# hegdepashupati/zero-inflated-gp

Hardware: AMD Instinct MI355X
Metric: elbo_steps_per_sec (higher is better)
Workload: dtype f64; 1 GPU; dense zero-inflated GP ELBO step (value+gradient), N=1000000 rows per GPU, D=3, M=1024 per latent, full batch; rows_this_rank=1000000, rows_total=1000000, M=1024, D=3, chunk_rows=32768, parallelism=row-shard x1, 1 all-reduce/step

## Files before the change

zero-inflated-gp_amd/csrc/zigp_ctx.h:

```cpp
#pragma once
#include <hip/hip_runtime.h>
#include <stdint.h>
#include <stdio.h>
#include <string.h>
#include <string>
#include <vector>
#include <map>
#include <memory>
#include "../../include/zigp.h"
#include "../../include/zigp_diag.h"
#include "zigp_gemm.h"

namespace zigp {

struct DevBuf {
  double* p = nullptr;
  size_t cap = 0;
  bool owned = true;
  DevBuf() = default;
  DevBuf(const DevBuf&) = delete;
  DevBuf& operator=(const DevBuf&) = delete;
  DevBuf(DevBuf&& o) noexcept : p(o.p), cap(o.cap), owned(o.owned) { o.p = nullptr; o.cap = 0; o.owned = true; }
  DevBuf& operator=(DevBuf&& o) noexcept {
    if (this != &o) { release(); p = o.p; cap = o.cap; owned = o.owned; o.p = nullptr; o.cap = 0; o.owned = true; }
    return *this;
  }
  ~DevBuf() { release(); }
  int ensure(size_t n) {
    if (!owned) { p = nullptr; cap = 0; owned = true; }
    if (n <= cap) return 0;
    if (p) (void)hipFree(p);
    p = nullptr; cap = 0;
    hipError_t e = hipMalloc((void**)&p, n * sizeof(double));
    if (e != hipSuccess) return -1;
    cap = n;
    return 0;
  }
  void alias(double* q, size_t n) { release(); p = q; cap = n; owned = false; }
  void release() { if (p && owned) (void)hipFree(p); p = nullptr; cap = 0; owned = true; }
};

enum ProfClass { PC_GEMM_A1 = 0, PC_GEMM_A2 = 1, PC_GEMM_H = 2, PC_GEMM_J = 3, PC_SYR2K = 4, PC_KUF = 5, PC_POINT = 6, PC_RED = 7, PC_MXM = 8, PC_OTHER = 9 };

struct TileList {
  GemmTile* d = nullptr;
  int n = 0;
  int per = 1;
};
struct HipFree { void operator()(void* q) const { (void)hipFree(q); } };
struct CachedTiles {
  std::unique_ptr<GemmTile, HipFree> d;
  int n = 0, per = 1;
  TileList view() const { return TileList{d.get(), n, per}; }
};

struct Latent {
  int M = 0, Mp = 0;
  DevBuf Z, ell, u, s, s2;
  double zc[64] = {0};
  bool kg_exact = false;
  DevBuf Zs;
  double var = 1.0;
  DevBuf Kuu, L, W;
  DevBuf K, A1, Jp;
  DevBuf Kd;
  DevBuf Wp, a1gm;
  DevBuf Wt;
  DevBuf P, Qt, Rt;
  bool P_ready = false;
  DevBuf part;
  DevBuf gm, gv;
  DevBuf du, dsq, krow;
  DevBuf xm, mom, ks0;
  DevBuf dLpart;
  DevBuf T1, T2, T3, G;
  DevBuf sk;
  DevBuf vec;
  DevBuf wh;
  DevBuf Lraw, Lq, lqssq, dLq;
};

struct KronState;
struct KfState;

struct PinnedArena {
  struct Block { char* p; size_t cap, used; };
  std::vector<Block> blocks;
  PinnedArena() = default;
  PinnedArena(const PinnedArena&) = delete;
  PinnedArena& operator=(const PinnedArena&) = delete;
  ~PinnedArena() { for (auto& b : blocks) (void)hipHostFree(b.p); }
  void reset() { for (auto& b : blocks) b.used = 0; }
  void* alloc(size_t bytes) {
    bytes = (bytes + 63) & ~(size_t)63;
    for (auto& b : blocks)
      if (b.cap - b.used >= bytes) { void* r = b.p + b.used; b.used += bytes; return r; }
    Block nb; nb.cap = bytes > ((size_t)1 << 20) ? bytes : ((size_t)1 << 20); nb.used = bytes; nb.p = nullptr;
    if (hipHostMalloc((void**)&nb.p, nb.cap, hipHostMallocDefault) != hipSuccess) return nullptr;
    blocks.push_back(nb);
    return nb.p;
  }
};

struct CtxHandles {
  hipStream_t stream = nullptr;
  hipStream_t stream_main = nullptr, stream2 = nullptr;
  hipStream_t stream3 = nullptr;
  hipEvent_t ev_fork = nullptr, ev_join = nullptr;
  hipEvent_t ev_prep_fork = nullptr, ev_prep = nullptr;
  int* d_info = nullptr;
  struct PendingEv { hipEvent_t a, b; int cls; };
  std::vector<PendingEv> pending;
  std::vector<hipEvent_t> ev_pool;
  CtxHandles() = default;
  CtxHandles(const CtxHandles&) = delete;
  CtxHandles& operator=(const CtxHandles&) = delete;
  ~CtxHandles() {
    if (d_info) (void)hipFree(d_info);
    for (auto& e : pending) { (void)hipEventDestroy(e.a); (void)hipEventDestroy(e.b); }
    for (auto e : ev_pool) (void)hipEventDestroy(e);
    for (hipEvent_t e : {ev_fork, ev_join, ev_prep_fork, ev_prep})
      if (e) (void)hipEventDestroy(e);
    for (hipStream_t s : {stream3, stream2, stream_main})
      if (s) (void)hipStreamDestroy(s);
  }
};

}

struct zigp_ctx : zigp::CtxHandles {
  ~zigp_ctx();
  int device = 0;
  std::string err;
  int info = 0;
  int64_t fit_steps_applied = 0;
  int64_t chunk = 32768;
  bool chunk_auto = true;
  const double* dX = nullptr; const double* dY = nullptr;
  zigp::DevBuf ownX, ownY;
  int64_t N = 0; int D = 0;
  const double* fullX = nullptr; const double* fullY = nullptr; int64_t fullN = 0;
  zigp::DevBuf selX, selY, selIdx;
  zigp::DevBuf fitX, fitY, fitIdx, fit;
  int64_t dense_fit_steps_applied = 0;
  zigp::Latent lat[2];
  zigp::DevBuf pw_part;
  bool fwd_kuf_side = true;
  bool trmm_tail = true;
  int overlap = 1;
  bool mean_on = false;
  bool whiten = false;
  int kern[2] = {0, 0};
  bool q_full = false;
  double mean_a[8] = {0}, mean_b = 0.0, mean_da[8] = {0}, mean_db = 0.0;
  zigp::DevBuf out9;
  zigp::DevBuf scratch, scratch2;
  zigp::DevBuf path_tab, path_out;
  zigp::PinnedArena pinned;
  std::unique_ptr<zigp::KronState> kron;
  std::unique_ptr<zigp::KfState> kronf;
  bool kron_panels = false;
  int kron_kern[2][2] = {{0, 0}, {0, 0}};
  bool kron_matern_fused = false;
  int kron_range_tiles = 1024;
  std::map<std::string, zigp::CachedTiles> tiles;
  void* comm = nullptr; int comm_rank = 0, comm_nranks = 1; int64_t comm_calls = 0;
  double comm_timeout_s = 120.0;
  zigp::DevBuf packed;
  zigp::DevBuf parm;
  double pivot_rtol = 8.0;
  bool prof_on = false;
  int prof_every = 8;
  bool prof_skip = false;
  int64_t prof_total[ZIGP_NCLASS] = {0};
  double prof_ms[ZIGP_NCLASS] = {0};
  int64_t prof_n[ZIGP_NCLASS] = {0};
  double prof_flops[ZIGP_NCLASS] = {0};
};

namespace zigp {

#define ZIGP_HIP(ctx, expr)                                                              \
  do {                                                                                   \
    hipError_t _e = (expr);                                                              \
    if (_e != hipSuccess) {                                                              \
      char _b[512];                                                                      \
      snprintf(_b, sizeof(_b), "HIP error '%s' at %s:%d (%s)", hipGetErrorString(_e), __FILE__, __LINE__, #expr); \
      (ctx)->err = _b;                                                                   \
      return ZIGP_EHIP;                                                                  \
    }                                                                                    \
  } while (0)

#define ZIGP_TRY(expr)            \
  do {                            \
    int _rc = (expr);             \
    if (_rc != 0) return _rc;     \
  } while (0)

#define ZIGP_ENSURE(ctx, buf, n)                                        \
  do {                                                                  \
    if ((buf).ensure((size_t)(n)) != 0) {                               \
      (ctx)->err = "hipMalloc failed for " #buf;                        \
      return ZIGP_EHIP;                                                 \
    }                                                                   \
  } while (0)

inline int fail_arg(zigp_ctx* c, const char* msg) { c->err = msg; return ZIGP_EARG; }

struct OnStream {
  zigp_ctx* c;
  hipStream_t saved;
  OnStream(zigp_ctx* c_, hipStream_t s) : c(c_), saved(c_->stream) { c->stream = s; }
  ~OnStream() { c->stream = saved; }
  OnStream(const OnStream&) = delete;
  OnStream& operator=(const OnStream&) = delete;
};

inline int fork_side(zigp_ctx* c, hipEvent_t ev, hipStream_t side) {
  ZIGP_HIP(c, hipEventRecord(ev, c->stream_main));
  ZIGP_HIP(c, hipStreamWaitEvent(side, ev, 0));
  return 0;
}
inline int join_side(zigp_ctx* c, hipEvent_t ev, hipStream_t side) {
  ZIGP_HIP(c, hipEventRecord(ev, side));
  ZIGP_HIP(c, hipStreamWaitEvent(c->stream_main, ev, 0));
  return 0;
}

struct ProfScope {
  zigp_ctx* c; hipEvent_t a = nullptr, b = nullptr; int cls; bool on;
  static hipEvent_t get_ev(zigp_ctx* c) {
    if (!c->ev_pool.empty()) { hipEvent_t e = c->ev_pool.back(); c->ev_pool.pop_back(); return e; }
    hipEvent_t e; if (hipEventCreate(&e) != hipSuccess) return nullptr; return e;
  }
  ProfScope(zigp_ctx* c_, int cls_, double flops = 0.0) : c(c_), cls(cls_), on(c_->prof_on) {
    if (!on) return;
    c->prof_total[cls] += 1;
    if (c->prof_skip) { on = false; return; }
    a = get_ev(c); b = get_ev(c);
    if (!a || !b) { on = false; return; }
    (void)hipEventRecord(a, c->stream);
    c->prof_flops[cls] += flops;
    c->prof_n[cls] += 1;
  }
  ~ProfScope() {
    if (!on) return;
    (void)hipEventRecord(b, c->stream);
    c->pending.push_back({a, b, cls});
  }
};

inline void prof_collect(zigp_ctx* c) {
  for (auto& p : c->pending) {
    float ms = 0.f;
    if (hipEventSynchronize(p.b) == hipSuccess && hipEventElapsedTime(&ms, p.a, p.b) == hipSuccess) c->prof_ms[p.cls] += ms;
    c->ev_pool.push_back(p.a); c->ev_pool.push_back(p.b);
  }
  c->pending.clear();
}

}
```

zero-inflated-gp_amd/csrc/zigp_dense.hip:

```cpp
#include "zigp_ctx.h"
#include "zigp_kernels.h"
#include "zigp_host.h"
#include "zigp_rows.h"
#include "zigp_comm.h"
#include <algorithm>
#include <cmath>
#include <functional>

using namespace zigp;

static_assert(WIDE_MAXD == ZIGP_MAX_D, "the wide kernels' hyperparameter structs hold ZIGP_MAX_D entries");
#define ZIGP_STR2(x) #x
#define ZIGP_STR(x) ZIGP_STR2(x)
#define ZIGP_MAX_D_STR ZIGP_STR(ZIGP_MAX_D)

namespace {

enum class Param : int { Diag = 0, White = 1, WhiteFull = 2 };
constexpr bool is_white(Param p) { return p != Param::Diag; }
constexpr bool is_full(Param p) { return p == Param::WhiteFull; }
static_assert((int)Param::Diag == ZIGP_FIT_DIAG && (int)Param::White == ZIGP_FIT_WHITE && (int)Param::WhiteFull == ZIGP_FIT_WHITE_FULL,
              "Param values are the ZIGP_FIT_* modes of include/zigp.h");
Param param_of(const zigp_ctx* c) { return !c->whiten ? Param::Diag : c->q_full ? Param::WhiteFull : Param::White; }

struct HostLatent {
  int M; const double *Z, *u, *s, *ell; double var;
  int kind = ZIGP_KERN_RBF;
};
static_assert(KERN_RBF == ZIGP_KERN_RBF && KERN_M32 == ZIGP_KERN_MATERN32 && KERN_M52 == ZIGP_KERN_MATERN52,
              "the kernels' kind values are the ZIGP_KERN_* constants of include/zigp.h");
constexpr bool is_matern(int kind) { return kind != ZIGP_KERN_RBF; }
const char* kern_name(int kind) { return kind == ZIGP_KERN_MATERN32 ? "Matern32" : kind == ZIGP_KERN_MATERN52 ? "Matern52" : "RBF"; }
const char* matern_latent(const zigp_ctx* c, std::string& who) {
  for (int h = 0; h < 2; ++h)
    if (is_matern(c->kern[h])) { who = std::string(kern_name(c->kern[h])) + " kernel on latent " + (h ? "g" : "f"); return who.c_str(); }
  return nullptr;
}

void kgrad_centre(Latent& lt, const double* Z, const double* ell, int M, int D) {
  double spread = 0.0;
  for (int d = 0; d < WIDE_MAXD; ++d) {
    double sum = 0.0;
    if (d < D) for (int m = 0; m < M; ++m) sum += Z[(size_t)m * D + d];
    lt.zc[d] = M > 0 ? sum / M : 0.0;
    if (d < D) for (int m = 0; m < M; ++m) spread = std::max(spread, std::fabs(Z[(size_t)m * D + d] - lt.zc[d]) / ell[d]);
  }
  lt.kg_exact = !(spread <= KG_EXACT_SPREAD);
}

int latents_layout(zigp_ctx* c, const int (&M)[2], int D, size_t (&off)[2][6], size_t& total) {
  total = 0;
  for (int h = 0; h < 2; ++h) {
    Latent& lt = c->lat[h];
    lt.M = M[h];
    lt.Mp = (int)round_up(M[h], BM);
    const size_t Mp = lt.Mp;
    off[h][0] = total; total += Mp * D;
    off[h][1] = total; total += std::max(D, MAXD);
    off[h][2] = total; total += Mp;
    off[h][3] = total; total += Mp;
    off[h][4] = total; total += Mp * D;
    off[h][5] = total;
  }
  ZIGP_ENSURE(c, c->parm, total);
  return 0;
}
int latents_views(zigp_ctx* c, const size_t (&off)[2][6], int D) {
  for (int h = 0; h < 2; ++h) {
    Latent& lt = c->lat[h];
    const size_t Mp = lt.Mp;
    lt.Z.alias(c->parm.p + off[h][0], Mp * D); lt.ell.alias(c->parm.p + off[h][1], std::max(D, MAXD));
    lt.u.alias(c->parm.p + off[h][2], Mp); lt.s.alias(c->parm.p + off[h][3], Mp); lt.Zs.alias(c->parm.p + off[h][4], Mp * D);
    ZIGP_ENSURE(c, lt.s2, Mp);
    ZIGP_ENSURE(c, lt.Kuu, Mp * Mp);
    ZIGP_ENSURE(c, lt.L, Mp * Mp);
    ZIGP_ENSURE(c, lt.W, Mp * Mp);
    ZIGP_ENSURE(c, lt.T1, Mp * Mp);
    ZIGP_ENSURE(c, lt.vec, 4 * Mp + 8);
    ZIGP_ENSURE(c, lt.wh, 4 * Mp + 8);
    ZIGP_ENSURE(c, lt.Wp, Mp * Mp);
    ZIGP_ENSURE(c, lt.Wt, Mp * Mp);
    ZIGP_ENSURE(c, lt.P, Mp * Mp); ZIGP_ENSURE(c, lt.Qt, Mp * Mp); ZIGP_ENSURE(c, lt.Rt, Mp * Mp);
  }
  return 0;
}
int latents_upload(zigp_ctx* c, const HostLatent (&hl)[2], int D, Param par) {
  size_t off[2][6], total = 0;
  const int M[2] = {hl[0].M, hl[1].M};
  ZIGP_TRY(latents_layout(c, M, D, off, total));
  for (int h = 0; h < 2; ++h) c->lat[h].var = hl[h].var;
  ZIGP_PINNED(c, img, total);
  memset(img, 0, sizeof(double) * total);
  for (int h = 0; h < 2; ++h) {
    const HostLatent& q = hl[h];
    memcpy(img + off[h][0], q.Z, sizeof(double) * q.M * D);
    memcpy(img + off[h][1], q.ell, sizeof(double) * D);
    memcpy(img + off[h][2], q.u, sizeof(double) * q.M);
    if (is_full(par)) for (int m = 0; m < q.M; ++m) img[off[h][3] + m] = q.s[(size_t)m * q.M + m];
    else memcpy(img + off[h][3], q.s, sizeof(double) * q.M);
    const KufHypWide kh = make_kuf_hyp_wide(q.ell, q.var, D);
    kgrad_centre(c->lat[h], q.Z, q.ell, q.M, D);
    for (int m = 0; m < q.M; ++m)
      for (int d = 0; d < D; ++d) img[off[h][4] + (size_t)m * D + d] = q.Z[(size_t)m * D + d] * kh.scale[d];
  }
  ZIGP_HIP(c, hipMemcpyAsync(c->parm.p, img, sizeof(double) * total, hipMemcpyHostToDevice, c->stream));
  if (is_full(par))
    for (int h = 0; h < 2; ++h) {
      Latent& lt = c->lat[h];
      const size_t mm = (size_t)hl[h].M * hl[h].M, mmp = (size_t)lt.Mp * lt.Mp;
      ZIGP_ENSURE(c, lt.Lraw, mm); ZIGP_ENSURE(c, lt.Lq, mmp); ZIGP_ENSURE(c, lt.lqssq, mmp / 256);
      ZIGP_PINNED(c, raw, mm);
      memcpy(raw, hl[h].s, sizeof(double) * mm);
      ZIGP_HIP(c, hipMemcpyAsync(lt.Lraw.p, raw, sizeof(double) * mm, hipMemcpyHostToDevice, c->stream));
    }
  return latents_views(c, off, D);
}

int latent_qfull_stage(zigp_ctx* c, Latent& lt) {
  const int Mp = lt.Mp, nblk = (int)((size_t)Mp * Mp / 256);
  hipLaunchKernelGGL(k_lq_stage, dim3(nblk), dim3(256), 0, c->stream, lt.Lraw.p, lt.M, (int64_t)Mp, lt.Lq.p, lt.lqssq.p);
  hipLaunchKernelGGL(k_kl_white_full, dim3(1), dim3(256), 0, c->stream, lt.u.p, lt.Lq.p, lt.lqssq.p, nblk, lt.M, (int64_t)Mp, lt.wh.p);
  ZIGP_HIP(c, hipGetLastError());
  return 0;
}
int latent_qfull_factors(zigp_ctx* c, Latent& lt) {
  const int Mp = lt.Mp, nb = Mp / BM;
  ZIGP_TRY((run_gemm_sk<LAY_KCONTIG, LAY_KCONTIG>(c, lt.sk, SkRule::TT, nb, lt.Lq.p, lt.Lq.p, lt.P.p, Mp, SK_STORE, 1.0)));
  hipLaunchKernelGGL(k_sub_eye, dim3(ceil_div(Mp, 256)), dim3(256), 0, c->stream, lt.P.p, lt.M, (int64_t)Mp);
  ZIGP_HIP(c, hipGetLastError());
  return run_gemm_sk<LAY_KCONTIG, LAY_MNCONTIG>(c, lt.sk, SkRule::Y, nb, lt.P.p, lt.W.p, lt.Rt.p, Mp, SK_STORE, 1.0);
}
int latent_qfull_dlq(zigp_ctx* c, Latent& lt, bool with_data, bool with_kl) {
  const int Mp = lt.Mp, nb = Mp / BM;
  const size_t mm = (size_t)Mp * Mp;
  ZIGP_ENSURE(c, lt.T3, mm); ZIGP_ENSURE(c, lt.dLq, mm);
  if (with_data)
    ZIGP_TRY((run_gemm_sk<LAY_KCONTIG, LAY_MNCONTIG>(c, lt.sk, SkRule::Y, nb, lt.T1.p, lt.Lq.p, lt.T3.p, Mp, SK_STORE, 1.0)));
  hipLaunchKernelGGL(k_dlq_assemble, dim3(ceil_div((int64_t)mm, 256)), dim3(256), 0, c->stream, lt.T3.p, lt.Lq.p, with_data ? 1 : 0, with_kl ? 1 : 0,
                     lt.M, (int64_t)Mp, lt.dLq.p);
  ZIGP_HIP(c, hipGetLastError());
  return 0;
}

int latents_forward(zigp_ctx* c, const HostLatent (&hl)[2], int D, double jitter, Param par, bool with_kl, bool need_grad, const double* d_hyp,
                    int* d_info2) {
  const hipStream_t st[2] = {c->stream_main, c->stream2};
  for (int h = 0; h < 2; ++h) {
    Latent& lt = c->lat[h];
    const int Mp = lt.Mp;
    OnStream on(c, st[h]);
    const dim3 grid(ceil_div((int64_t)Mp * Mp, 256));
    if (is_matern(hl[h].kind))
      hipLaunchKernelGGL(k_kuu_setup_matern, grid, dim3(256), 0, c->stream, lt.Z.p, (int64_t)hl[h].M, make_hyp(hl[h].ell, hl[h].var, D), hl[h].kind, jitter,
                         lt.Kuu.p, lt.L.p, lt.W.p, lt.s.p, lt.s2.p, (int64_t)Mp);
    else if (d_hyp)
      hipLaunchKernelGGL(k_kuu_setup<LatHypDev>, grid, dim3(256), 0, c->stream, lt.Z.p, (int64_t)hl[h].M, LatHypDev{d_hyp + h * DH_LAT, D}, jitter, lt.Kuu.p,
                         lt.L.p, lt.W.p, lt.s.p, lt.s2.p, (int64_t)Mp);
    else if (D > MAXD)
      hipLaunchKernelGGL(k_kuu_setup<KernHypWide>, grid, dim3(256), 0, c->stream, lt.Z.p, (int64_t)hl[h].M, make_hyp_wide(hl[h].ell, hl[h].var, D), jitter,
                         lt.Kuu.p, lt.L.p, lt.W.p, lt.s.p, lt.s2.p, (int64_t)Mp);
    else {
      KernHyp hyp = make_hyp(hl[h].ell, hl[h].var, D);
      hipLaunchKernelGGL(k_kuu_setup<KernHyp>, grid, dim3(256), 0, c->stream, lt.Z.p, (int64_t)hl[h].M, hyp, jitter, lt.Kuu.p,
                         lt.L.p, lt.W.p, lt.s.p, lt.s2.p, (int64_t)Mp);
    }
    ZIGP_HIP(c, hipGetLastError());
  }
  {
    PotrfJob jobs[2];
    for (int h = 0; h < 2; ++h) {
      Latent& lt = c->lat[h];
      jobs[h] = PotrfJob{lt.L.p, lt.W.p, lt.T1.p, lt.Mp, true, lt.M, d_hyp ? 0.0 : pivot_tol(hl[h].var, jitter, c->pivot_rtol), true, &lt.sk};
      if (d_hyp) { jobs[h].tol_dev = d_hyp + h * DH_LAT + DH_PIVTOL; jobs[h].info = d_info2 + h; }
    }
    ZIGP_TRY(potrf_trtri_jobs(c, 2, jobs, st));
  }
  for (int step = 0; step < 8; ++step)
    for (int h = 0; h < 2; ++h) {
      Latent& lt = c->lat[h];
      const int Mp = lt.Mp;
      OnStream on(c, st[h]);
      if (step == 0) lt.P_ready = false;
      double* v = lt.vec.p; double* alpha = v + Mp; double* dkinv = v + 2 * Mp; double* klv = v + 3 * Mp;
      if (is_white(par)) {
        switch (step) {
          case 0: hipLaunchKernelGGL(k_transpose, dim3(Mp / 32, Mp / 32), dim3(32, 8), 0, c->stream, lt.W.p, (int64_t)Mp, lt.Wt.p); break;
          case 1:
            if (is_full(par)) ZIGP_TRY(latent_qfull_stage(c, lt));
            else hipLaunchKernelGGL(k_kl_white, dim3(1), dim3(256), 0, c->stream, lt.u.p, lt.s.p, lt.M, (int64_t)Mp, lt.wh.p);
            break;
          case 2: if (need_grad) hipLaunchKernelGGL(k_gemv_cols, dim3(Mp / 64), dim3(64, COL_LANES), 0, c->stream, lt.W.p, lt.u.p, (int64_t)Mp, alpha); break;
          case 3:
            if (need_grad && is_full(par)) ZIGP_TRY(latent_qfull_factors(c, lt));
            else if (need_grad) hipLaunchKernelGGL(k_rowscale, dim3(ceil_div((int64_t)Mp * Mp, 256)), dim3(256), 0, c->stream, lt.W.p, lt.wh.p, (int64_t)Mp, lt.Wp.p);
            break;
          default: break;
        }
        ZIGP_HIP(c, hipGetLastError());
        continue;
      }
      switch (step) {
        case 0:
          hipLaunchKernelGGL(k_transpose, dim3(Mp / 32, Mp / 32), dim3(32, 8), 0, c->stream, lt.W.p, (int64_t)Mp, lt.Wt.p);
          break;
        case 1: if (with_kl) hipLaunchKernelGGL(k_gemv_rows, dim3(Mp), dim3(256), 0, c->stream, lt.W.p, lt.u.p, (int64_t)Mp, v); break;
        case 2: if (with_kl) hipLaunchKernelGGL(k_kl_cols, dim3(Mp / 64), dim3(64, COL_LANES), 0, c->stream, lt.W.p, v, (int64_t)Mp, alpha, dkinv); break;
        case 3: if (with_kl) hipLaunchKernelGGL(k_kl_value, dim3(1), dim3(256), 0, c->stream, v, lt.L.p, lt.s.p, dkinv, lt.M, (int64_t)Mp, klv); break;
        case 4:
          if (need_grad) hipLaunchKernelGGL(k_colscale, dim3(ceil_div((int64_t)Mp * Mp, 256)), dim3(256), 0, c->stream, lt.W.p, lt.s2.p, (int64_t)Mp, lt.Wp.p);
          break;
        case 5:
          if (need_grad) {
            ZIGP_TRY((run_gemm_sk<LAY_MNCONTIG, LAY_MNCONTIG>(c, lt.sk, SkRule::S, Mp / BM, lt.W.p, lt.W.p, lt.P.p, Mp, SK_STORE, 1.0)));
            lt.P_ready = true;
          }
          break;
        case 6:
          if (need_grad) hipLaunchKernelGGL(k_rowscale_minus_eye, dim3(ceil_div((int64_t)Mp * Mp, 256)), dim3(256), 0, c->stream, lt.P.p, lt.s2.p, (int64_t)Mp, lt.Qt.p);
          break;
        case 7:
          if (need_grad) ZIGP_TRY((run_gemm_sk<LAY_KCONTIG, LAY_MNCONTIG>(c, lt.sk, SkRule::RT, Mp / BM, lt.W.p, lt.Qt.p, lt.Rt.p, Mp, SK_STORE, 1.0)));
          break;
        default: break;
      }
      ZIGP_HIP(c, hipGetLastError());
    }
  return 0;
}

int latent_chunk_kuf_matern(zigp_ctx* c, Latent& lt, const double* dX, int64_t Nrows, int64_t n0, int64_t Nc, int D, const double* ell_host, int kind,
                            bool with_kd) {
  if (D < 1 || D > MAXD || !ell_host) return fail_arg(c, "a Matern Kuf panel needs 1 <= D <= 8 and host lengthscales");
  if (with_kd && lt.Kd.cap < (size_t)lt.Mp * Nc) return fail_arg(c, "a Matern gradient step's K' panel was not sized for this chunk");
  const KufHyp kh = make_kuf_hyp(ell_host, lt.var, D);
  ProfScope ps(c, PC_KUF);
  const dim3 grid((unsigned)(Nc / 512), lt.Mp / 16), block(256);
#define ZIGP_KUF_M(DD, KK, GG) \
  hipLaunchKernelGGL((k_kuf_build_matern<DD, KK, GG>), grid, block, 0, c->stream, dX, Nrows, n0, lt.Zs.p, lt.M, kh, lt.K.p, GG ? lt.Kd.p : nullptr, Nc)
#define ZIGP_KUF_MD(DD)                                                                    \
  case DD:                                                                                 \
    if (kind == ZIGP_KERN_MATERN32) { if (with_kd) ZIGP_KUF_M(DD, KERN_M32, true); else ZIGP_KUF_M(DD, KERN_M32, false); } \
    else { if (with_kd) ZIGP_KUF_M(DD, KERN_M52, true); else ZIGP_KUF_M(DD, KERN_M52, false); }                            \
    break;
  switch (D) { ZIGP_KUF_MD(1) ZIGP_KUF_MD(2) ZIGP_KUF_MD(3) ZIGP_KUF_MD(4) ZIGP_KUF_MD(5) ZIGP_KUF_MD(6) ZIGP_KUF_MD(7) ZIGP_KUF_MD(8) }
#undef ZIGP_KUF_MD
#undef ZIGP_KUF_M
  ZIGP_HIP(c, hipGetLastError());
  return 0;
}
int latent_chunk_kuf(zigp_ctx* c, Latent& lt, const double* dX, int64_t Nrows, int64_t n0, int64_t Nc, int D, const double* ell_host,
                     const double* R = nullptr, int kind = ZIGP_KERN_RBF, bool with_kd = false) {
  if (is_matern(kind)) return latent_chunk_kuf_matern(c, lt, dX, Nrows, n0, Nc, D, ell_host, kind, with_kd);
  const int Mp = lt.Mp;
  const KufHyp kh = (R || D > MAXD) ? KufHyp() : make_kuf_hyp(ell_host, lt.var, D);
  ProfScope ps(c, PC_KUF);
  const dim3 grid((unsigned)(Nc / 512), Mp / 16), block(256);
#define ZIGP_KUF(DD)                                                                                                                   \
  case DD:                                                                                                                             \
    if (R) hipLaunchKernelGGL((k_kuf_build<DD, LatHypDev>), grid, block, 0, c->stream, dX, Nrows, n0, lt.Zs.p, lt.M, LatHypDev{R, DD}, lt.K.p, Nc); \
    else hipLaunchKernelGGL((k_kuf_build<DD, KufHyp>), grid, block, 0, c->stream, dX, Nrows, n0, lt.Zs.p, lt.M, kh, lt.K.p, Nc);               \
    break;
  switch (D) {
    ZIGP_KUF(1) ZIGP_KUF(2) ZIGP_KUF(3) ZIGP_KUF(4) ZIGP_KUF(5) ZIGP_KUF(6) ZIGP_KUF(7) ZIGP_KUF(8)
    default:
      if (D < 1 || D > WIDE_MAXD || R) return fail_arg(c, "D out of range");
      hipLaunchKernelGGL(k_kuf_build_wide, grid, block, 0, c->stream, dX, Nrows, n0, lt.Zs.p, lt.M, D, make_kuf_hyp_wide(ell_host, lt.var, D), lt.K.p, Nc);
      break;
  }
#undef ZIGP_KUF
  ZIGP_HIP(c, hipGetLastError());
  return 0;
}

struct ChunkPlan {
  int64_t Nc = 0;
  bool paired = false;
  TrmmTail tail = {{0, 0}, {64, 64}};
  struct Lat { TileSpec a1_spec, a2j_spec, syr_spec, mom_spec; TileList a1, a2j, syr, mom; double fl = 0.0; } lat[2];
};
ChunkPlan chunk_plan(const int (&M)[2], int64_t Nc, Param par, bool need_grad, bool tail_on, bool wide) {
  ChunkPlan pl;
  const int nbm[2] = {ceil_div(M[0], BM), ceil_div(M[1], BM)}, nbn = (int)(Nc / BN);
  pl.Nc = Nc;
  pl.paired = trmm_paired_pays(nbn * ((nbm[0] + 1) / 2 + (nbm[1] + 1) / 2));
  if (pl.paired && tail_on)
    pl.tail = trmm_tail_plan((nbn + 7) / 8 * 8 * ((nbm[0] + 1) / 2), nbm[0], (nbn + 7) / 8 * 8 * ((nbm[1] + 1) / 2), nbm[1]);
  for (int h = 0; h < 2; ++h) {
    ChunkPlan::Lat& L = pl.lat[h];
    auto tri = [&](bool lower) { return trmm_tiles(lower, nbm[h], nbn, pl.paired, pl.tail.units[h], pl.tail.bins[h]); };
    auto full_product = [&] { return full_xcd_tiles(nbm[h], nbn, nbm[h] * (BM / BK)); };
    L.a1_spec = tri(true);
    switch (par) {
      case Param::Diag: L.a2j_spec = need_grad ? full_product() : tri(false); break;
      case Param::White: if (need_grad) L.a2j_spec = tri(false); break;
      case Param::WhiteFull: L.a2j_spec = need_grad ? full_product() : tri(false); break;
    }
    if (need_grad) L.syr_spec = syr2k_tiles(nbm[h], (int)(Nc / BK), syr_plan(nbm[h]));
    if (need_grad && wide) L.mom_spec = kgmom_tiles(nbm[h], Nc);
    L.fl = (double)M[h] * M[h] * (double)Nc;
  }
  return pl;
}
int upload_plan(zigp_ctx* c, ChunkPlan& pl) {
  for (ChunkPlan::Lat& L : pl.lat) {
    ZIGP_TRY(get_tiles(c, L.a1_spec, L.a1));
    if (L.a2j_spec.build) ZIGP_TRY(get_tiles(c, L.a2j_spec, L.a2j));
    if (L.syr_spec.build) ZIGP_TRY(get_tiles(c, L.syr_spec, L.syr));
    if (L.mom_spec.build) ZIGP_TRY(get_tiles(c, L.mom_spec, L.mom));
  }
  return 0;
}

int chunk_forward(zigp_ctx* c, const ChunkPlan& pl, Param par, bool need_grad, const std::function<int()>& after_a1 = nullptr) {
  const int64_t Nc = pl.Nc;
  struct Set { TileList t1, t2; double fl; GemmArgs a1, a2j; EpiStoreColsum e1; EpiColsum e2; EpiStorePanelKColsum ej; } q[3] = {};
  for (int h = 0; h < 2; ++h) {
    Latent& lt = c->lat[h];
    const int Mp = lt.Mp, np = Mp / 32;
    q[h].t1 = pl.lat[h].a1; q[h].t2 = pl.lat[h].a2j; q[h].fl = pl.lat[h].fl;
    q[h].a1 = mk_args(lt.Wt.p, Mp, lt.K.p, Nc, lt.A1.p, Nc);
    q[h].e1 = EpiStoreColsum{is_full(par) ? lt.wh.p + Mp : lt.vec.p, nullptr, lt.part.p, lt.part.p + (size_t)np * Nc};
    if (need_grad) {
      q[h].a2j = mk_args(lt.Rt.p, Mp, lt.A1.p, Nc, lt.Jp.p, Nc);
      q[h].ej = EpiStorePanelKColsum{lt.K.p, lt.part.p + (size_t)2 * np * Nc};
    } else {
      q[h].a2j = mk_args(is_full(par) ? lt.Lq.p : lt.W.p, Mp, lt.A1.p, Nc, nullptr, Nc);
      q[h].e2 = EpiColsum{nullptr, is_full(par) ? nullptr : lt.s2.p, nullptr, lt.part.p + (size_t)2 * np * Nc};
    }
  }
  const int groups = pl.paired ? 1 : 2;
  for (int gi = 0; gi < groups; ++gi) {
    const Set& x = q[gi];
    const Set& y = q[pl.paired ? 1 : 2];
    {
      ProfScope ps(c, PC_GEMM_A1, x.fl + y.fl);
      ZIGP_TRY((run_gemm<LAY_MNCONTIG, LAY_MNCONTIG, false, TRI_A_LOWER>(c, x.t1, x.a1, x.e1, y.t1, y.a1, y.e1)));
    }
    if (gi == groups - 1 && after_a1) ZIGP_TRY(after_a1());
    if (need_grad) {
      ProfScope ps(c, PC_GEMM_J, 2.0 * (x.fl + y.fl));
      ZIGP_TRY((run_gemm<LAY_MNCONTIG, LAY_MNCONTIG, false>(c, x.t2, x.a2j, x.ej, y.t2, y.a2j, y.ej)));
    } else {
      ProfScope ps(c, PC_GEMM_A2, x.fl + y.fl);
      ZIGP_TRY((run_gemm<LAY_MNCONTIG, LAY_MNCONTIG, false, TRI_A_UPPER>(c, x.t2, x.a2j, x.e2, y.t2, y.a2j, y.e2)));
    }
  }
  return 0;
}

int chunk_forward_white(zigp_ctx* c, const ChunkPlan& pl, bool need_grad, bool part_j, const std::function<int()>& after_a = nullptr) {
  const int64_t Nc = pl.Nc;
  struct Set { TileList t; double fl; GemmArgs g; EpiStoreColsum es; EpiColsum ec; } q[3] = {};
  for (int h = 0; h < 2; ++h) {
    Latent& lt = c->lat[h];
    const int Mp = lt.Mp, np = Mp / 32;
    double* p0 = lt.part.p; double* p2 = lt.part.p + (size_t)2 * np * Nc;
    q[h].fl = pl.lat[h].fl;
    if (part_j) { q[h].t = pl.lat[h].a2j; q[h].g = mk_args(lt.Wp.p, Mp, lt.A1.p, Nc, lt.Jp.p, Nc); continue; }
    q[h].t = pl.lat[h].a1;
    q[h].g = mk_args(lt.Wt.p, Mp, lt.K.p, Nc, need_grad ? lt.A1.p : nullptr, Nc);
    q[h].es = EpiStoreColsum{lt.wh.p + Mp, lt.wh.p, p0, p2};
    q[h].ec = EpiColsum{lt.wh.p + Mp, lt.wh.p, p0, p2};
  }
  const int groups = pl.paired ? 1 : 2;
  for (int gi = 0; gi < groups; ++gi) {
    const Set& x = q[gi];
    const Set& y = q[pl.paired ? 1 : 2];
    if (part_j) {
      ProfScope ps(c, PC_GEMM_J, x.fl + y.fl);
      ZIGP_TRY((run_gemm<LAY_MNCONTIG, LAY_MNCONTIG, false, TRI_A_UPPER>(c, x.t, x.g, EpiStore(), y.t, y.g, EpiStore())));
      continue;
    }
    {
      ProfScope ps(c, PC_GEMM_A1, x.fl + y.fl);
      if (need_grad) ZIGP_TRY((run_gemm<LAY_MNCONTIG, LAY_MNCONTIG, false, TRI_A_LOWER>(c, x.t, x.g, x.es, y.t, y.g, y.es)));
      else ZIGP_TRY((run_gemm<LAY_MNCONTIG, LAY_MNCONTIG, false, TRI_A_LOWER>(c, x.t, x.g, x.ec, y.t, y.g, y.ec)));
    }
    if (gi == groups - 1 && after_a) ZIGP_TRY(after_a());
  }
  return 0;
}

int latent_chunk_kgrad_wide(zigp_ctx* c, Latent& lt, const double* dX, int64_t Nrows, int64_t n0, int64_t Nc, int D, const TileList& mom) {
  const int Mp = lt.Mp, S = kgmom_slices(Mp / BM, Nc);
  if (mom.n != S * (Mp / BM)) return fail_arg(c, "wide Kuf gradient: the moments product's tile list was not planned for this chunk shape");
  KgCentreWide ctr;
  for (int d = 0; d < WIDE_MAXD; ++d) ctr.c[d] = lt.zc[d];
  hipLaunchKernelGGL(k_kgrad_wide_prep, dim3(Mp / KG_ROWS, KG_SPLIT), dim3(256), 0, c->stream, lt.Jp.p, lt.K.p, lt.vec.p + Mp, lt.gm.p, lt.gv.p, dX, Nrows,
                     n0, lt.M, Mp, D, Nc, (int64_t)Mp * (2 + 2 * D), ctr, lt.krow.p, lt.ks0.p, lt.xm.p);
  ZIGP_HIP(c, hipGetLastError());
  GemmArgs g = mk_args(lt.Jp.p, Nc, lt.xm.p, WIDE_MOM_COLS, lt.mom.p, WIDE_MOM_COLS);
  g.slice_stride = (int64_t)Mp * WIDE_MOM_COLS;
  ZIGP_TRY((run_gemm<LAY_KCONTIG, LAY_MNCONTIG, false>(c, mom, g, EpiStore())));
  hipLaunchKernelGGL(k_kgrad_wide_finish, dim3(Mp / 4), dim3(256), 0, c->stream, lt.mom.p, S, lt.ks0.p, lt.Z.p, lt.M, Mp, D, ctr, lt.krow.p);
  ZIGP_HIP(c, hipGetLastError());
  return 0;
}
int ensure_kgrad_wide(zigp_ctx* c, Latent& lt, int64_t Nc) {
  const int Mp = lt.Mp;
  ZIGP_ENSURE(c, lt.xm, (size_t)Nc * WIDE_MOM_COLS);
  ZIGP_ENSURE(c, lt.mom, (size_t)kgmom_slices(Mp / BM, Nc) * Mp * WIDE_MOM_COLS);
  ZIGP_ENSURE(c, lt.ks0, (size_t)KG_SPLIT * Mp);
  return 0;
}

int latent_chunk_kgrad_matern(zigp_ctx* c, Latent& lt, const double* dX, int64_t Nrows, int64_t n0, int64_t Nc, int D) {
  const int Mp = lt.Mp;
  if (D < 1 || D > MAXD) return fail_arg(c, "a Matern Kuf gradient needs 1 <= D <= 8");
  if (lt.Kd.cap < (size_t)Mp * Nc) return fail_arg(c, "a Matern gradient step's K' panel was not sized for this chunk");
  ProfScope ps(c, PC_RED);
  const dim3 gk((unsigned)ceil_div(lt.M, KG_ROWS), KG_SPLIT), bk(256);
  const int64_t slab = (int64_t)Mp * (2 + 2 * D);
#define ZIGP_KGRAD_M(DD)                                                                                                                         \
  case DD:                                                                                                                                       \
    hipLaunchKernelGGL((k_kgrad_matern<DD>), gk, bk, 0, c->stream, lt.Jp.p, lt.K.p, lt.Kd.p, lt.vec.p + Mp, lt.gm.p, lt.gv.p, dX, Nrows, n0, lt.Z.p, \
                       lt.M, Nc, slab, lt.krow.p);                                                                                               \
    break;
  switch (D) { ZIGP_KGRAD_M(1) ZIGP_KGRAD_M(2) ZIGP_KGRAD_M(3) ZIGP_KGRAD_M(4) ZIGP_KGRAD_M(5) ZIGP_KGRAD_M(6) ZIGP_KGRAD_M(7) ZIGP_KGRAD_M(8) }
#undef ZIGP_KGRAD_M
  ZIGP_HIP(c, hipGetLastError());
  return 0;
}
int latent_chunk_kgrad(zigp_ctx* c, Latent& lt, const double* dX, int64_t Nrows, int64_t n0, int64_t Nc, int D, const double* ell_host,
                       const TileList& mom = TileList(), int kind = ZIGP_KERN_RBF) {
  if (is_matern(kind)) return latent_chunk_kgrad_matern(c, lt, dX, Nrows, n0, Nc, D);
  const int Mp = lt.Mp;
  KgCentre hyp;
  for (int d = 0; d < MAXD; ++d) hyp.c[d] = lt.zc[d];
  double* alpha = lt.vec.p + Mp;
  {
    ProfScope ps(c, PC_RED);
    const dim3 gk((unsigned)ceil_div(lt.M, KG_ROWS), KG_SPLIT), bk(256);
    const int64_t slab = (int64_t)Mp * (2 + 2 * D);
#define ZIGP_KGRAD(DD)                                                                                                            \
  case DD:                                                                                                                        \
    if (lt.kg_exact)                                                                                                              \
      hipLaunchKernelGGL((k_kgrad<DD, true>), gk, bk, 0, c->stream, lt.Jp.p, lt.K.p, alpha, lt.gm.p, lt.gv.p, dX, Nrows, n0, lt.Z.p, lt.M, Nc, \
                         slab, hyp, lt.krow.p);                                                                                   \
    else                                                                                                                          \
      hipLaunchKernelGGL((k_kgrad<DD, false>), gk, bk, 0, c->stream, lt.Jp.p, lt.K.p, alpha, lt.gm.p, lt.gv.p, dX, Nrows, n0, lt.Z.p, lt.M, Nc, \
                         slab, hyp, lt.krow.p);                                                                                   \
    break;
    switch (D) {
      ZIGP_KGRAD(1) ZIGP_KGRAD(2) ZIGP_KGRAD(3) ZIGP_KGRAD(4) ZIGP_KGRAD(5) ZIGP_KGRAD(6) ZIGP_KGRAD(7) ZIGP_KGRAD(8)
      default:
        if (D < 1 || D > WIDE_MAXD) return fail_arg(c, "D out of range");
        if (!lt.kg_exact) { ZIGP_TRY(latent_chunk_kgrad_wide(c, lt, dX, Nrows, n0, Nc, D, mom)); break; }
        for (int d0 = 0; d0 < D; d0 += WIDE_SLICE)
          hipLaunchKernelGGL(k_kgrad_slice, gk, bk, 0, c->stream, lt.Jp.p, lt.K.p, alpha, lt.gm.p, lt.gv.p, dX, Nrows, n0, lt.Z.p, lt.M, D, d0, Nc,
                             slab, lt.krow.p);
        break;
    }
#undef ZIGP_KGRAD
    ZIGP_HIP(c, hipGetLastError());
  }
  return 0;
}

int latent_chunk_syrk(zigp_ctx* c, const ChunkPlan& pl, int h) {
  Latent& lt = c->lat[h];
  const int Mp = lt.Mp;
  const int64_t Nc = pl.Nc;
  ProfScope ps(c, PC_SYR2K, pl.lat[h].fl);
  GemmArgs g = mk_args(lt.A1.p, Nc, lt.A1.p, Nc, lt.dLpart.p, Mp);
  g.slice_stride = (int64_t)Mp * Mp; g.kscale = lt.gv.p;
  return run_gemm<LAY_KCONTIG, LAY_KCONTIG, true, TRI_C_LOWER>(c, pl.lat[h].syr, g, EpiAccum());
}

void latent_sym_from_planes(zigp_ctx* c, Latent& lt) {
  const int Mp = lt.Mp;
  const SyrPlan sp = syr_plan(Mp / BM);
  const int nt = Mp / 32;
  hipLaunchKernelGGL(k_sym_from_planes, dim3(nt * (nt + 1) / 2), dim3(256), 0, c->stream, lt.dLpart.p, sp.So, sp.Sd, (int64_t)Mp, lt.T1.p);
}

void launch_kuu_grad(zigp_ctx* c, Latent& lt, int D, double jitter, const HostLatent* hk = nullptr) {
  const int Mp = lt.Mp;
  if (hk && is_matern(hk->kind))
    hipLaunchKernelGGL(k_kuu_grad_matern, dim3(Mp), dim3(256), 0, c->stream, lt.T3.p, lt.Kuu.p, jitter, lt.Z.p, lt.M, make_hyp(hk->ell, hk->var, D), hk->kind,
                       (int64_t)Mp, lt.krow.p);
  else if (D > MAXD)
    hipLaunchKernelGGL(k_kuu_grad_wide, dim3(Mp, ceil_div(D, WIDE_SLICE)), dim3(256), 0, c->stream, lt.T3.p, lt.Kuu.p, jitter, lt.Z.p, lt.M, D, (int64_t)Mp,
                       lt.krow.p);
  else hipLaunchKernelGGL(k_kuu_grad, dim3(Mp), dim3(256), 0, c->stream, lt.T3.p, lt.Kuu.p, jitter, lt.Z.p, lt.M, D, (int64_t)Mp, lt.krow.p);
}

using MxmTap = std::function<int(int, const double*)>;
#define ZIGP_TAP(id, buf) do { if (tap) ZIGP_TRY(tap(id, buf)); } while (0)

int mxm_backward_head(zigp_ctx* c, Latent& lt, int D, Param par, const MxmTap& tap) {
  const int Mp = lt.Mp;
  double* kgm = lt.vec.p + 3 * Mp + 8;
  hipLaunchKernelGGL(k_gather, dim3(ceil_div(Mp, 256)), dim3(256), 0, c->stream, lt.krow.p, 2 + 2 * D, 1 + 2 * D, Mp, KG_SPLIT,
                     (int64_t)Mp * (2 + 2 * D), kgm);
  hipLaunchKernelGGL(k_gemv_rows, dim3(Mp), dim3(256), 0, c->stream, lt.W.p, kgm, (int64_t)Mp, lt.a1gm.p);
  if (!is_white(par)) hipLaunchKernelGGL(k_gemv_cols, dim3(Mp / 64), dim3(64, COL_LANES), 0, c->stream, lt.W.p, lt.a1gm.p, (int64_t)Mp, lt.du.p);
  latent_sym_from_planes(c, lt);
  ZIGP_TAP(ZIGP_MXM_TAP_C1, lt.T1.p);
  return 0;
}
int mxm_backward_r_diag(zigp_ctx* c, Latent& lt, const MxmTap& tap) {
  const int Mp = lt.Mp, nb = Mp / BM, gridmm = ceil_div((int64_t)Mp * Mp, 256);
  ZIGP_TRY((run_gemm_sk<LAY_KCONTIG, LAY_MNCONTIG>(c, lt.sk, SkRule::Y, nb, lt.T1.p, lt.W.p, lt.T3.p, Mp, SK_STORE, 1.0)));
  ZIGP_TAP(ZIGP_MXM_TAP_Y, lt.T3.p);
  hipLaunchKernelGGL(k_coldot, dim3(Mp / 64), dim3(64, COL_LANES), 0, c->stream, lt.W.p, lt.T3.p, (int64_t)Mp, lt.dsq.p);
  ZIGP_TRY((run_gemm_sk<LAY_KCONTIG, LAY_KCONTIG>(c, lt.sk, SkRule::TT, nb, lt.Wp.p, lt.W.p, lt.T2.p, Mp, SK_STORE, 1.0)));
  ZIGP_TAP(ZIGP_MXM_TAP_T, lt.T2.p);
  ZIGP_TRY((run_gemm_sk<LAY_KCONTIG, LAY_MNCONTIG>(c, lt.sk, SkRule::FULL, nb, lt.T2.p, lt.T1.p, lt.T3.p, Mp, SK_STORE, 1.0)));
  ZIGP_TAP(ZIGP_MXM_TAP_U, lt.T3.p);
  hipLaunchKernelGGL(k_uut_minus, dim3(gridmm), dim3(256), 0, c->stream, lt.T3.p, lt.T1.p, (int64_t)Mp, lt.G.p);
  ZIGP_TAP(ZIGP_MXM_TAP_V, lt.G.p);
  ZIGP_TRY((run_gemm_sk<LAY_MNCONTIG, LAY_MNCONTIG>(c, lt.sk, SkRule::R, nb, lt.W.p, lt.G.p, lt.T2.p, Mp, SK_STORE, 1.0)));
  ZIGP_TAP(ZIGP_MXM_TAP_R, lt.T2.p);
  return 0;
}
int mxm_backward_r_white(zigp_ctx* c, Latent& lt, Param par, bool with_kl, const MxmTap& tap) {
  const int Mp = lt.Mp, nb = Mp / BM;
  if (is_full(par)) {
    ZIGP_TRY(latent_qfull_dlq(c, lt, true, with_kl));
    ZIGP_TAP(ZIGP_MXM_TAP_Y, lt.T3.p);
    ZIGP_TRY((run_gemm_sk<LAY_MNCONTIG, LAY_MNCONTIG>(c, lt.sk, SkRule::RFULL, nb, lt.Rt.p, lt.T1.p, lt.T2.p, Mp, SK_STORE, 1.0)));
  } else {
    hipLaunchKernelGGL(k_diag, dim3(ceil_div(Mp, 256)), dim3(256), 0, c->stream, lt.T1.p, (int64_t)Mp, lt.dsq.p);
    ZIGP_TRY((run_gemm_sk<LAY_MNCONTIG, LAY_MNCONTIG>(c, lt.sk, SkRule::R, nb, lt.Wp.p, lt.T1.p, lt.T2.p, Mp, SK_STORE, 1.0)));
  }
  ZIGP_TAP(ZIGP_MXM_TAP_R, lt.T2.p);
  return 0;
}
int mxm_backward_tail(zigp_ctx* c, Latent& lt, const double* r1, const double* r2, const MxmTap& tap) {
  const int Mp = lt.Mp, nb = Mp / BM;
  hipLaunchKernelGGL(k_dl_assemble, dim3(ceil_div((int64_t)Mp * Mp, 256)), dim3(256), 0, c->stream, lt.T2.p, (int64_t)Mp, lt.vec.p + Mp, lt.a1gm.p, r1,
                     r2, lt.T1.p);
  ZIGP_TAP(ZIGP_MXM_TAP_DL, lt.T1.p);
  ZIGP_TRY((run_gemm_sk<LAY_MNCONTIG, LAY_MNCONTIG>(c, lt.sk, SkRule::R, nb, lt.L.p, lt.T1.p, lt.T2.p, Mp, SK_PHI, 1.0)));
  ZIGP_TAP(ZIGP_MXM_TAP_Q, lt.T2.p);
  ZIGP_TRY((run_gemm_sk<LAY_KCONTIG, LAY_MNCONTIG>(c, lt.sk, SkRule::T, nb, lt.T2.p, lt.W.p, lt.T3.p, Mp, SK_STORE, 1.0)));
  ZIGP_TAP(ZIGP_MXM_TAP_QW, lt.T3.p);
  ZIGP_TRY((run_gemm_sk<LAY_MNCONTIG, LAY_MNCONTIG>(c, lt.sk, SkRule::S, nb, lt.W.p, lt.T3.p, lt.T1.p, Mp, SK_STORE, 1.0)));
  ZIGP_TAP(ZIGP_MXM_TAP_S, lt.T1.p);
  return 0;
}
int latent_mxm_backward(zigp_ctx* c, Latent& lt, int D, double jitter, Param par, bool with_data, bool with_kl, const MxmTap& tap,
                        const HostLatent* hk = nullptr) {
  const int Mp = lt.Mp, nb = Mp / BM;
  const size_t mm = (size_t)Mp * Mp;
  ZIGP_ENSURE(c, lt.T1, mm); ZIGP_ENSURE(c, lt.T2, mm); ZIGP_ENSURE(c, lt.T3, mm);
  if (!is_white(par)) ZIGP_ENSURE(c, lt.G, mm);
  const int gridmm = ceil_div((int64_t)mm, 256);
  if (with_data) {
    ZIGP_TRY(mxm_backward_head(c, lt, D, par, tap));
    if (is_white(par)) ZIGP_TRY(mxm_backward_r_white(c, lt, par, with_kl, tap));
    else ZIGP_TRY(mxm_backward_r_diag(c, lt, tap));
    ZIGP_TRY(mxm_backward_tail(c, lt, lt.du.p, is_white(par) ? lt.du.p : lt.vec.p, tap));
  } else if (is_full(par)) ZIGP_TRY(latent_qfull_dlq(c, lt, false, with_kl));
  if (is_white(par)) {
    hipLaunchKernelGGL(k_sym_combine, dim3(gridmm), dim3(256), 0, c->stream, lt.T1.p, lt.T1.p, lt.T1.p, lt.vec.p + Mp, with_data ? 1 : 0, 0,
                       (int64_t)Mp, lt.T3.p);
  } else {
    double* P = lt.P_ready ? lt.P.p : lt.T2.p; double* PSP = lt.G.p;
    if (with_kl) {
      if (!lt.P_ready) {
        ZIGP_TRY((run_gemm_sk<LAY_MNCONTIG, LAY_MNCONTIG>(c, lt.sk, SkRule::S, nb, lt.W.p, lt.W.p, lt.T2.p, Mp, SK_STORE, 1.0)));
        ZIGP_TAP(ZIGP_MXM_TAP_P, lt.T2.p);
      }
      hipLaunchKernelGGL(k_rowscale, dim3(gridmm), dim3(256), 0, c->stream, P, lt.s2.p, (int64_t)Mp, lt.T3.p);
      ZIGP_TRY((run_gemm_sk<LAY_KCONTIG, LAY_MNCONTIG>(c, lt.sk, SkRule::FULL, nb, P, lt.T3.p, lt.G.p, Mp, SK_STORE, 1.0)));
      ZIGP_TAP(ZIGP_MXM_TAP_PSP, lt.G.p);
    }
    hipLaunchKernelGGL(k_sym_combine, dim3(gridmm), dim3(256), 0, c->stream, lt.T1.p, P, PSP, lt.vec.p + Mp, with_data ? 1 : 0, with_kl ? 1 : 0,
                       (int64_t)Mp, lt.T3.p);
  }
  launch_kuu_grad(c, lt, D, jitter, hk);
  ZIGP_HIP(c, hipGetLastError());
  return 0;
}

int validate_params(zigp_ctx* c, const zigp_params* p) {
  if (!p) return fail_arg(c, "params is NULL");
  if (p->Mf <= 0 || p->Mg <= 0) return fail_arg(c, "Mf and Mg must be positive");
  if (p->D <= 0 || p->D > ZIGP_MAX_D) return fail_arg(c, "D must be in [1, " ZIGP_MAX_D_STR "] (ZIGP_MAX_D)");
  if (p->D > MAXD) {
    std::string who;
    if (matern_latent(c, who))
      return fail_arg(c, ("a " + who + " (zigp_set_kernel) and D = " + std::to_string(p->D) + ": the Matern kernels cover D in [1, 8] (the wide kernels are RBF only)").c_str());
  }
  if (p->D > MAXD && c->mean_on)
    for (int d = 0; d < MAXD; ++d)
      if (c->mean_a[d] != 0.0) return fail_arg(c, "a Linear mean function is set and D > 8: Linear covers D in [1, 8] (Zero and Constant work at every D)");
  if (!p->Zf || !p->Zg || !p->u_fm || !p->u_gm || !p->u_fs_sqrt || !p->u_gs_sqrt || !p->ell_f || !p->ell_g)
    return fail_arg(c, "NULL pointer in params");
  if (!(p->var_f > 0) || !(p->var_g > 0) || !(p->noise > 0)) return fail_arg(c, "variances must be positive");
  for (int d = 0; d < p->D; ++d)
    if (!(p->ell_f[d] > 0) || !(p->ell_g[d] > 0)) return fail_arg(c, "lengthscales must be positive");
  if (c->q_full) {
    if (!c->whiten) return fail_arg(c, "zigp_set_q_full is on while whitening is off: the full-covariance q(u) exists for the whitened model only (zigp_set_whiten)");
    for (int m = 0; m < p->Mf; ++m)
      if (!(p->u_fs_sqrt[(size_t)m * p->Mf + m] != 0)) return fail_arg(c, "u_fs_sqrt has a zero (or NaN) diagonal entry (full q_sqrt, zigp_set_q_full)");
    for (int m = 0; m < p->Mg; ++m)
      if (!(p->u_gs_sqrt[(size_t)m * p->Mg + m] != 0)) return fail_arg(c, "u_gs_sqrt has a zero (or NaN) diagonal entry (full q_sqrt, zigp_set_q_full)");
    return 0;
  }
  for (int m = 0; m < p->Mf; ++m)
    if (!(p->u_fs_sqrt[m] > 0)) return fail_arg(c, "u_fs_sqrt must be positive (diagonal q_sqrt, transforms.positive)");
  for (int m = 0; m < p->Mg; ++m)
    if (!(p->u_gs_sqrt[m] > 0)) return fail_arg(c, "u_gs_sqrt must be positive (diagonal q_sqrt, transforms.positive)");
  return 0;
}

struct DenseCall {
  const zigp_params* p; const double* dX; const double* dY; int64_t Nrows; int D;
  double jitter, scale, g_offset; int64_t row_begin, row_end; int include_kl; bool predict; double* d_out9;
  bool need_grad, has_rows;
  Param par = Param::Diag;
  bool dlq_as_triangle = false;
  HostLatent hl[2]; const double* ell_h[2];
  int64_t Nc = 0;
  ChunkPlan plan[2];
  int pw_blocks = 0;
  int* hinfo = nullptr;
  bool prep_side = false;
  const double* d_hyp = nullptr; int* d_info2 = nullptr;
  int lik = 0;
  const double* hyp_rec(int h) const { return d_hyp ? d_hyp + h * DH_LAT : nullptr; }
};

int dense_prepare_buffers(zigp_ctx* c, DenseCall& k);
int64_t dense_first_chunk_rows(const DenseCall& k) { return std::min<int64_t>(k.Nc, round_up(k.row_end - k.row_begin, 1024)); }
int dense_mxm_forward(zigp_ctx* c, DenseCall& k) {
  if (k.d_hyp) ZIGP_HIP(c, hipMemsetAsync(k.d_info2, 0, 2 * sizeof(int), c->stream));
  else {
    ZIGP_TRY(begin_staged_call(c));
    ZIGP_HIP(c, hipMemsetAsync(c->d_info, 0, sizeof(int), c->stream));
    ZIGP_TRY(latents_upload(c, k.hl, k.D, k.par));
  }
  k.prep_side = c->overlap == 1 && !c->prof_on;
  if (k.prep_side) {
    ZIGP_TRY(fork_side(c, c->ev_prep_fork, c->stream3));
    OnStream on(c, c->stream3);
    ZIGP_TRY(dense_prepare_buffers(c, k));
    if (k.has_rows)
      for (int h = 0; h < 2; ++h)
        ZIGP_TRY(latent_chunk_kuf(c, c->lat[h], k.dX, k.Nrows, k.row_begin, dense_first_chunk_rows(k), k.D, k.ell_h[h], k.hyp_rec(h), k.hl[h].kind,
                                  k.need_grad));
    ZIGP_HIP(c, hipEventRecord(c->ev_prep, c->stream3));
  }
  {
    ProfScope ps(c, PC_MXM);
    ZIGP_TRY(fork_side(c, c->ev_fork, c->stream2));
    ZIGP_TRY(latents_forward(c, k.hl, k.D, k.jitter, k.par, true, k.need_grad, k.d_hyp, k.d_info2));
    ZIGP_TRY(join_side(c, c->ev_join, c->stream2));
  }
  return k.d_hyp ? 0 : request_info(c, &k.hinfo);
}

int64_t auto_chunk_for(bool chunk_auto, int64_t chunk_set, int64_t Mp) {
  if (!chunk_auto) return chunk_set;
  return std::min<int64_t>(131072, std::max<int64_t>(32768, round_up(32768 * 1024 / std::max<int64_t>(Mp, 128), 1024)));
}
int64_t chunk_rows_for(bool chunk_auto, int64_t chunk_set, int64_t Mp, int64_t span) {
  int64_t chunk = auto_chunk_for(chunk_auto, chunk_set, Mp);
  if (chunk_auto && span > 0 && span <= 131072 && 4 * 2 * 8 * Mp * round_up(span, 1024) <= ((int64_t)9 << 30)) chunk = 131072;
  if (span <= 0) return 1024;
  const int64_t nchunks = (span + chunk - 1) / chunk;
  return std::max<int64_t>(1024, round_up((span + nchunks - 1) / nchunks, 1024));
}
int dense_prepare_buffers(zigp_ctx* c, DenseCall& k) {
  const int64_t Nc = k.Nc;
  const int D = k.D;
  k.pw_blocks = (int)(Nc / PW_PTS);
  ZIGP_ENSURE(c, c->pw_part, (size_t)k.pw_blocks * PW_ACC);
  ZeroRanges zr;
  zr.count = 0;
  static_assert(1 + 2 * 4 <= ZERO_RANGES_MAX, "one launch zeroes every small accumulator of a call");
  auto zero = [&](double* ptr, int64_t n) { zr.p[zr.count] = ptr; zr.n[zr.count] = n; ++zr.count; };
  zero(c->pw_part.p, (int64_t)k.pw_blocks * PW_ACC);
  for (int h = 0; h < 2; ++h) {
    Latent& lt = c->lat[h];
    const int Mp = lt.Mp;
    ZIGP_ENSURE(c, lt.gm, Nc); ZIGP_ENSURE(c, lt.gv, Nc);
    if (k.has_rows) {
      ZIGP_ENSURE(c, lt.K, (size_t)Mp * Nc);
      if (k.par != Param::White || k.need_grad) ZIGP_ENSURE(c, lt.A1, (size_t)Mp * Nc);
      ZIGP_ENSURE(c, lt.part, (size_t)3 * (Mp / 32) * Nc);
      if (k.need_grad) ZIGP_ENSURE(c, lt.Jp, (size_t)Mp * Nc);
      if (k.need_grad && is_matern(k.hl[h].kind)) ZIGP_ENSURE(c, lt.Kd, (size_t)Mp * Nc);
      if (k.need_grad && D > MAXD && !lt.kg_exact) ZIGP_TRY(ensure_kgrad_wide(c, lt, Nc));
    }
    if (k.need_grad) {
      ZIGP_ENSURE(c, lt.du, Mp); ZIGP_ENSURE(c, lt.dsq, Mp); ZIGP_ENSURE(c, lt.krow, (size_t)KG_SPLIT * Mp * (2 + 2 * D));
      const int S = syr_plan(Mp / BM).planes();
      ZIGP_ENSURE(c, lt.dLpart, (size_t)S * Mp * Mp);
      ZIGP_ENSURE(c, lt.a1gm, Mp);
      zero(lt.a1gm.p, Mp); zero(lt.du.p, Mp); zero(lt.dsq.p, Mp); zero(lt.krow.p, (int64_t)KG_SPLIT * Mp * (2 + 2 * D));
      if (k.has_rows) ZIGP_HIP(c, hipMemsetAsync(lt.dLpart.p, 0, sizeof(double) * S * Mp * Mp, c->stream));
    }
  }
  hipLaunchKernelGGL(k_zero_ranges, dim3(64), dim3(256), 0, c->stream, zr);
  ZIGP_HIP(c, hipGetLastError());
  return 0;
}

PwArgs dense_pointwise_args(zigp_ctx* c, const DenseCall& k, int64_t n0, int64_t Nc) {
  PwArgs a;
  a.part_f = c->lat[0].part.p; a.part_g = c->lat[1].part.p; a.np_f = c->lat[0].Mp / 32; a.np_g = c->lat[1].Mp / 32;
  {
    constexpr int RW2 = Shape<WavesFor<LAY_MNCONTIG, LAY_MNCONTIG, false>::value>::RW, RW1 = RW2;
    static_assert(RW1 >= 32 && RW2 >= 32, "partial-row planes are allocated for 32-row wave tiles");
    a.np1_f = c->lat[0].Mp / RW1; a.np2_f = c->lat[0].Mp / RW2; a.np1_g = c->lat[1].Mp / RW1; a.np2_g = c->lat[1].Mp / RW2;
  }
  a.Y = k.dY; a.n0 = n0; a.row_end = k.row_end; a.Nc = Nc;
  a.var_f = k.p->var_f; a.var_g = k.p->var_g; a.noise = k.p->noise; a.g_offset = k.g_offset; a.scale = k.scale;
  a.gm_f = k.need_grad ? c->lat[0].gm.p : nullptr; a.gv_f = c->lat[0].gv.p; a.gm_g = c->lat[1].gm.p; a.gv_g = c->lat[1].gv.p;
  a.X = k.dX; a.D = k.D; a.mean_on = c->mean_on ? 1 : 0; a.mean_b = c->mean_b;
  for (int d = 0; d < MAXD; ++d) a.mean_a[d] = (d < k.D) ? c->mean_a[d] : 0.0;
  a.acc = c->pw_part.p; a.out9 = k.d_out9 ? k.d_out9 - k.row_begin : nullptr; a.ld9 = k.row_end - k.row_begin;
  return a;
}
static_assert(PWH_GAUSSIAN == ZIGP_LIK_GAUSSIAN && PWH_BERNOULLI == ZIGP_LIK_BERNOULLI, "the head kernel's LIK values are the ZIGP_LIK_* constants");
template <int LIK>
void pointwise_head_launch(zigp_ctx* c, const dim3& grid, const dim3& block, bool predict, bool plane2, const PwArgs& a) {
  if (predict && plane2) hipLaunchKernelGGL((k_pointwise_head<LIK, true, true>), grid, block, 0, c->stream, a);
  else if (predict) hipLaunchKernelGGL((k_pointwise_head<LIK, true, false>), grid, block, 0, c->stream, a);
  else if (plane2) hipLaunchKernelGGL((k_pointwise_head<LIK, false, true>), grid, block, 0, c->stream, a);
  else hipLaunchKernelGGL((k_pointwise_head<LIK, false, false>), grid, block, 0, c->stream, a);
}
int dense_pointwise_launch(zigp_ctx* c, Param par, bool predict, bool need_grad, const PwArgs& a, const double* d_hyp, int lik = 0) {
  ProfScope ps(c, PC_POINT);
  const dim3 grid((unsigned)(a.Nc / PW_PTS)), block(PW_THREADS);
  const bool plane2 = need_grad || d_hyp || par == Param::White;
  if (lik == ZIGP_LIK_GAUSSIAN) pointwise_head_launch<PWH_GAUSSIAN>(c, grid, block, predict, plane2, a);
  else if (lik == ZIGP_LIK_BERNOULLI) pointwise_head_launch<PWH_BERNOULLI>(c, grid, block, predict, plane2, a);
  else if (d_hyp) hipLaunchKernelGGL((k_pointwise<false, true>), grid, block, 0, c->stream, a, d_hyp);
  else if (predict && plane2) hipLaunchKernelGGL((k_pointwise<true, true>), grid, block, 0, c->stream, a);
  else if (predict) hipLaunchKernelGGL((k_pointwise<true, false>), grid, block, 0, c->stream, a);
  else if (plane2) hipLaunchKernelGGL((k_pointwise<false, true>), grid, block, 0, c->stream, a);
  else hipLaunchKernelGGL((k_pointwise<false, false>), grid, block, 0, c->stream, a);
  ZIGP_HIP(c, hipGetLastError());
  return 0;
}
int dense_pointwise(zigp_ctx* c, const DenseCall& k, int64_t n0, int64_t Nc) {
  return dense_pointwise_launch(c, k.par, k.predict, k.need_grad, dense_pointwise_args(c, k, n0, Nc), k.d_hyp, k.lik);
}

int dense_chunk_loop(zigp_ctx* c, const DenseCall& k) {
  if (!k.has_rows) return 0;
  const int64_t Nc_full = k.Nc, row_begin = k.row_begin, row_end = k.row_end;
  const int D = k.D;
  auto chunk_rows = [&](int64_t n0) { return std::min<int64_t>(Nc_full, round_up(row_end - n0, 1024)); };
  auto sampled = [&](int64_t n0) {
    if (!c->prof_on) return false;
    if (c->prof_every <= 1 || row_end - row_begin <= Nc_full) return true;
    return chunk_rows(n0) == Nc_full && (((n0 - row_begin) / Nc_full) % c->prof_every) == 0;
  };
  auto kuf = [&](int64_t n0) -> int {
    for (int h = 0; h < 2; ++h)
      ZIGP_TRY(latent_chunk_kuf(c, c->lat[h], k.dX, k.Nrows, n0, chunk_rows(n0), D, k.ell_h[h], k.hyp_rec(h), k.hl[h].kind, k.need_grad));
    return 0;
  };
  auto kgrad = [&](int64_t n0, int64_t Nc) -> int {
    const ChunkPlan& pl = k.plan[Nc == k.plan[0].Nc ? 0 : 1];
    for (int h = 0; h < 2; ++h) ZIGP_TRY(latent_chunk_kgrad(c, c->lat[h], k.dX, k.Nrows, n0, Nc, D, k.ell_h[h], pl.lat[h].mom, k.hl[h].kind));
    return 0;
  };
  bool side_busy = false;
  auto on_side = [&](auto work) -> int {
    ZIGP_TRY(fork_side(c, c->ev_fork, c->stream2));
    OnStream on(c, c->stream2);
    ZIGP_TRY(work());
    ZIGP_HIP(c, hipEventRecord(c->ev_join, c->stream2));
    side_busy = true;
    return 0;
  };
  auto wait_side = [&]() -> int {
    if (side_busy) ZIGP_HIP(c, hipStreamWaitEvent(c->stream_main, c->ev_join, 0));
    side_busy = false;
    return 0;
  };
  c->prof_skip = c->prof_on && !sampled(row_begin);
  if (!k.prep_side) ZIGP_TRY(kuf(row_begin));
  for (int64_t n0 = row_begin; n0 < row_end; n0 += Nc_full) {
    const int64_t Nc = chunk_rows(n0);
    const int64_t n1 = n0 + Nc_full;
    const bool has_next = n1 < row_end;
    const bool timed = sampled(n0), timed_next = has_next && sampled(n1);
    c->prof_skip = c->prof_on && !timed;
    ZIGP_TRY(wait_side());
    const bool kuf_fwd_side = c->overlap == 1 && c->fwd_kuf_side && !k.need_grad && has_next && !timed && !timed_next;
    std::function<int()> after_a1;
    if (kuf_fwd_side) after_a1 = [&] { return on_side([&] { return kuf(n1); }); };
    const ChunkPlan& pl = k.plan[Nc == k.plan[0].Nc ? 0 : 1];
    if (k.par == Param::White) {
      ZIGP_TRY(chunk_forward_white(c, pl, k.need_grad, false, after_a1));
      ZIGP_TRY(dense_pointwise(c, k, n0, Nc));
      if (k.need_grad) ZIGP_TRY(chunk_forward_white(c, pl, true, true));
    } else {
      ZIGP_TRY(chunk_forward(c, pl, k.par, k.need_grad, after_a1));
      ZIGP_TRY(dense_pointwise(c, k, n0, Nc));
    }
    const bool kgrad_side = c->overlap == 1 && k.need_grad && !timed;
    const bool kuf_side = kgrad_side && has_next && !timed_next;
    if (kgrad_side)
      ZIGP_TRY(on_side([&]() -> int {
        ZIGP_TRY(kgrad(n0, Nc));
        return kuf_side ? kuf(n1) : 0;
      }));
    if (k.need_grad) {
      if (!kgrad_side) ZIGP_TRY(kgrad(n0, Nc));
      for (int h = 0; h < 2; ++h) ZIGP_TRY(latent_chunk_syrk(c, pl, h));
    }
    if (has_next && !kuf_side && !kuf_fwd_side) {
      ZIGP_TRY(wait_side());
      c->prof_skip = c->prof_on && !timed_next;
      ZIGP_TRY(kuf(n1));
    }
  }
  return wait_side();
}

int dense_pack(zigp_ctx* c, const DenseCall& k, DensePackArgs& a, size_t& n) {
  const int D = k.D;
  n = DP_HDR;
  memset(&a, 0, sizeof(a));
  for (int h = 0; h < 2; ++h) {
    Latent& lt = c->lat[h];
    DensePackLat& L = a.lat[h];
    L.krow = lt.krow.p; L.du = lt.du.p; L.dsq = lt.dsq.p; L.vec = lt.vec.p; L.s = lt.s.p; L.ell = lt.ell.p;
    if (is_white(k.par)) { L.du = lt.a1gm.p; L.vec = lt.wh.p; }
    L.M = lt.M; L.Mp = lt.Mp; L.var = lt.var; L.out_off = (int64_t)n; L.q_full = is_full(k.par) ? 1 : 0;
    L.ns = !is_full(k.par) ? (int64_t)lt.M : k.dlq_as_triangle ? (int64_t)lt.M * (lt.M + 1) / 2 : (int64_t)lt.M * lt.M;
    if (k.need_grad) n += (size_t)lt.M * D + (size_t)lt.M + (size_t)L.ns + D;
  }
  a.pw = c->pw_part.p; a.pw_blocks = k.pw_blocks; a.D = D; a.need_grad = k.need_grad ? 1 : 0; a.include_kl = k.include_kl ? 1 : 0;
  a.mean_on = c->mean_on ? 1 : 0;
  ZIGP_ENSURE(c, c->packed, n);
  a.out = c->packed.p;
  if (k.d_hyp) hipLaunchKernelGGL(k_dense_pack<const double*>, dim3(2), dim3(256), 0, c->stream, a, k.d_hyp);
  else hipLaunchKernelGGL(k_dense_pack<>, dim3(2), dim3(256), 0, c->stream, a);
  if (k.need_grad && is_full(k.par))
    for (int h = 0; h < 2; ++h) {
      const Latent& lt = c->lat[h];
      double* os = a.out + a.lat[h].out_off + (int64_t)lt.M * D + lt.M;
      const dim3 grid(ceil_div((int64_t)lt.M * lt.M, 256));
      if (k.dlq_as_triangle) hipLaunchKernelGGL(k_pack_tril, grid, dim3(256), 0, c->stream, lt.dLq.p, lt.M, (int64_t)lt.Mp, os);
      else hipLaunchKernelGGL(k_pack_square, grid, dim3(256), 0, c->stream, lt.dLq.p, lt.M, (int64_t)lt.Mp, os);
    }
  ZIGP_HIP(c, hipGetLastError());
  return 0;
}
int dense_gather(zigp_ctx* c, DenseCall& k, double* elbo_data, double* kl, zigp_grads* grads) {
  const int D = k.D;
  size_t n = 0;
  DensePackArgs a;
  ZIGP_TRY(dense_pack(c, k, a, n));
  ZIGP_TRY(comm_allreduce(c, c->packed.p, n));
  double* hv = nullptr;
  ZIGP_TRY(download(c, c->packed.p, n, &hv));
  double* hkl_f = nullptr;
  if (k.lik) ZIGP_TRY(download(c, (is_white(k.par) ? c->lat[0].wh.p : c->lat[0].vec.p) + 3 * c->lat[0].Mp, 1, &hkl_f));
  ZIGP_HIP(c, hipStreamSynchronize(c->stream));
  prof_collect(c);
  ZIGP_TRY(info_result(c, k.hinfo, "Kuu"));
  if (elbo_data) *elbo_data = hv[0];
  if (kl) *kl = !k.lik ? hv[1] : k.include_kl ? *hkl_f : 0.0;
  c->mean_db = hv[5];
  for (int d = 0; d < MAXD; ++d) c->mean_da[d] = hv[6 + d];
  if (k.need_grad) {
    double* gZ[2] = {grads->Zf, grads->Zg};
    double* gu[2] = {grads->u_fm, grads->u_gm};
    double* gs[2] = {grads->u_fs_sqrt, grads->u_gs_sqrt};
    double* gl[2] = {grads->ell_f, grads->ell_g};
    for (int h = 0; h < (k.lik ? 1 : 2); ++h) {
      const size_t M = (size_t)c->lat[h].M;
      const double* o = hv + a.lat[h].out_off;
      if (gZ[h]) memcpy(gZ[h], o, sizeof(double) * M * D);
      if (gu[h]) memcpy(gu[h], o + M * D, sizeof(double) * M);
      const size_t ns = is_full(k.par) ? M * M : M;
      if (gs[h]) memcpy(gs[h], o + M * D + M, sizeof(double) * ns);
      if (gl[h]) memcpy(gl[h], o + M * D + M + ns, sizeof(double) * D);
    }
    grads->var_f = hv[2]; grads->noise = hv[4];
    if (!k.lik) grads->var_g = hv[3];
  }
  return 0;
}

int dense_plan(zigp_ctx* c, DenseCall& k) {
  const int M[2] = {k.hl[0].M, k.hl[1].M};
  const int64_t span = k.has_rows ? k.row_end - k.row_begin : 0;
  k.Nc = chunk_rows_for(c->chunk_auto, c->chunk, round_up(std::max(M[0], M[1]), BM), span);
  if (k.has_rows) {
    const int64_t last = std::min<int64_t>(k.Nc, round_up(span - (span - 1) / k.Nc * k.Nc, 1024));
    k.plan[0] = chunk_plan(M, k.Nc, k.par, k.need_grad, c->trmm_tail, k.D > MAXD);
    ZIGP_TRY(upload_plan(c, k.plan[0]));
    if (last != k.Nc) { k.plan[1] = chunk_plan(M, last, k.par, k.need_grad, c->trmm_tail, k.D > MAXD); ZIGP_TRY(upload_plan(c, k.plan[1])); }
  }
  return 0;
}
int dense_step(zigp_ctx* c, DenseCall& k) {
  ZIGP_TRY(dense_mxm_forward(c, k));
  if (k.prep_side) ZIGP_HIP(c, hipStreamWaitEvent(c->stream_main, c->ev_prep, 0));
  else ZIGP_TRY(dense_prepare_buffers(c, k));
  const int rc = dense_chunk_loop(c, k);
  c->prof_skip = false;
  ZIGP_TRY(rc);
  if (k.need_grad) {
    ProfScope ps(c, PC_MXM);
    ZIGP_TRY(fork_side(c, c->ev_fork, c->stream2));
    for (int h = 0; h < 2; ++h) {
      OnStream on(c, h == 0 ? c->stream_main : c->stream2);
      ZIGP_TRY(latent_mxm_backward(c, c->lat[h], k.D, k.jitter, k.par, k.has_rows, k.include_kl != 0, nullptr, &k.hl[h]));
    }
    ZIGP_TRY(join_side(c, c->ev_join, c->stream2));
  }
  return 0;
}

struct HeadPlaceholder {
  double Z[ZIGP_MAX_D], ell[ZIGP_MAX_D], u[1], s[1];
  HeadPlaceholder() { for (int d = 0; d < ZIGP_MAX_D; ++d) { Z[d] = 0.0; ell[d] = 1.0; } u[0] = 0.0; s[0] = 1.0; }
};
const HeadPlaceholder& head_placeholder() { static const HeadPlaceholder h; return h; }

int run_dense_lik(zigp_ctx* c, const zigp_params* p, int lik, const double* dX, const double* dY, int64_t Nrows, int D, double jitter,
                  double scale, double g_offset, int64_t row_begin, int64_t row_end, int include_kl, bool predict, double* d_out9,
                  double* elbo_data, double* kl, zigp_grads* grads);
int run_dense(zigp_ctx* c, const zigp_params* p, const double* dX, const double* dY, int64_t Nrows, int D, double jitter,
              double scale, double g_offset, int64_t row_begin, int64_t row_end, int include_kl, bool predict, double* d_out9,
              double* elbo_data, double* kl, zigp_grads* grads) {
  return run_dense_lik(c, p, 0, dX, dY, Nrows, D, jitter, scale, g_offset, row_begin, row_end, include_kl, predict, d_out9, elbo_data, kl, grads);
}
int run_dense_lik(zigp_ctx* c, const zigp_params* p, int lik, const double* dX, const double* dY, int64_t Nrows, int D, double jitter,
                  double scale, double g_offset, int64_t row_begin, int64_t row_end, int include_kl, bool predict, double* d_out9,
                  double* elbo_data, double* kl, zigp_grads* grads) {
  DenseCall k;
  k.lik = lik;
  k.p = p; k.dX = dX; k.dY = dY; k.Nrows = Nrows; k.D = D; k.jitter = jitter; k.scale = scale; k.g_offset = g_offset;
  k.row_begin = row_begin; k.row_end = row_end; k.include_kl = include_kl; k.predict = predict; k.d_out9 = d_out9;
  k.need_grad = (grads != nullptr) && !predict;
  k.has_rows = row_end > row_begin;
  k.par = param_of(c);
  k.hl[0] = HostLatent{p->Mf, p->Zf, p->u_fm, p->u_fs_sqrt, p->ell_f, p->var_f, c->kern[0]};
  k.hl[1] = HostLatent{p->Mg, p->Zg, p->u_gm, p->u_gs_sqrt, p->ell_g, p->var_g, lik ? (int)ZIGP_KERN_RBF : c->kern[1]};
  k.ell_h[0] = p->ell_f; k.ell_h[1] = p->ell_g;
  ZIGP_TRY(dense_plan(c, k));
  ZIGP_TRY(dense_step(c, k));
  if (predict) { ZIGP_HIP(c, hipStreamSynchronize(c->stream)); prof_collect(c); return info_result(c, k.hinfo, "Kuu"); }
  return dense_gather(c, k, elbo_data, kl, grads);
}

}

extern "C" {

int zigp_create(zigp_ctx** out, int device_id) {
  if (!out) return ZIGP_EARG;
  *out = nullptr;
  int ndev = 0;
  if (hipGetDeviceCount(&ndev) != hipSuccess || ndev <= 0) return ZIGP_EHIP;
  if (device_id < 0 || device_id >= ndev) return ZIGP_EARG;
  if (hipSetDevice(device_id) != hipSuccess) return ZIGP_EHIP;
  zigp_ctx* c = new (std::nothrow) zigp_ctx();
  if (!c) return ZIGP_EHIP;
  c->device = device_id;
  if (hipStreamCreateWithFlags(&c->stream, hipStreamNonBlocking) != hipSuccess) { delete c; return ZIGP_EHIP; }
  c->stream_main = c->stream;
  if (hipStreamCreateWithFlags(&c->stream2, hipStreamNonBlocking) != hipSuccess) { delete c; return ZIGP_EHIP; }
  if (hipStreamCreateWithFlags(&c->stream3, hipStreamNonBlocking) != hipSuccess) { delete c; return ZIGP_EHIP; }
  if (hipEventCreateWithFlags(&c->ev_fork, hipEventDisableTiming) != hipSuccess ||
      hipEventCreateWithFlags(&c->ev_join, hipEventDisableTiming) != hipSuccess ||
      hipEventCreateWithFlags(&c->ev_prep_fork, hipEventDisableTiming) != hipSuccess ||
      hipEventCreateWithFlags(&c->ev_prep, hipEventDisableTiming) != hipSuccess) { delete c; return ZIGP_EHIP; }
  if (hipMalloc((void**)&c->d_info, sizeof(int)) != hipSuccess) { delete c; return ZIGP_EHIP; }
  if (hipFuncSetAttribute(reinterpret_cast<const void*>(&k_potrf_diag<double>), hipFuncAttributeMaxDynamicSharedMemorySize,
                          (int)(sizeof(double) * PB * PBLD)) != hipSuccess ||
      hipFuncSetAttribute(reinterpret_cast<const void*>(&k_potrf_diag<const double*>), hipFuncAttributeMaxDynamicSharedMemorySize,
                          (int)(sizeof(double) * PB * PBLD)) != hipSuccess) { delete c; return ZIGP_EHIP; }
  if (const char* e = getenv("ZIGP_FWD_KUF_SIDE")) c->fwd_kuf_side = atoi(e) != 0;
  if (const char* e = getenv("ZIGP_TRMM_TAIL")) c->trmm_tail = atoi(e) != 0;
  if (const char* e = getenv("ZIGP_COMM_TIMEOUT_S")) { const double v = atof(e); if (v > 0) c->comm_timeout_s = v; }
  *out = c;
  return ZIGP_OK;
}

int zigp_destroy(zigp_ctx* c) {
  if (!c) return ZIGP_EARG;
  (void)hipSetDevice(c->device);
  (void)hipStreamSynchronize(c->stream_main);
  (void)hipStreamSynchronize(c->stream2);
  if (c->stream3) (void)hipStreamSynchronize(c->stream3);
  if (c->comm) { RcclApi* api = rccl_api(nullptr); if (api) (void)api->CommDestroy(static_cast<ncclComm_t>(c->comm)); c->comm = nullptr; }
  delete c;
  return ZIGP_OK;
}

const char* zigp_last_error(zigp_ctx* c) { return c ? c->err.c_str() : "null context"; }
int zigp_last_info(zigp_ctx* c) { return c ? c->info : 0; }

int zigp_set_overlap(zigp_ctx* c, int32_t on) {
  if (!c) return ZIGP_EARG;
  if (on < 0 || on > 1) return fail_arg(c, "zigp_set_overlap: mode must be 0 or 1");
  c->overlap = on;
  return ZIGP_OK;
}

int zigp_set_chunk(zigp_ctx* c, int64_t chunk_rows) {
  if (!c) return ZIGP_EARG;
  if (chunk_rows == 0) { c->chunk_auto = true; c->chunk = 32768; return ZIGP_OK; }
  if (chunk_rows < 1024 || chunk_rows % 1024 != 0) return fail_arg(c, "chunk must be a positive multiple of 1024 (or 0: automatic)");
  if (chunk_rows > (1 << 20)) return fail_arg(c, "chunk must be <= 1048576 rows (32-bit staging offsets; 3 panels (K, A1, J') of 8*M*chunk bytes per latent)");
  c->chunk = chunk_rows;
  c->chunk_auto = false;
  return ZIGP_OK;
}

int zigp_set_pivot_rtol(zigp_ctx* c, double rtol) {
  if (!c) return ZIGP_EARG;
  if (!(rtol >= 0) || !std::isfinite(rtol)) return fail_arg(c, "zigp_set_pivot_rtol: rtol must be finite and >= 0");
  c->pivot_rtol = rtol;
  return ZIGP_OK;
}

int64_t zigp_get_chunk(zigp_ctx* c, int32_t M) {
  if (!c || M <= 0) return ZIGP_EARG;
  return auto_chunk_for(c->chunk_auto, c->chunk, round_up(M, BM));
}

int64_t zigp_get_chunk_rows(zigp_ctx* c, int32_t M, int64_t span) {
  if (!c || M <= 0 || span < 0) return ZIGP_EARG;
  return chunk_rows_for(c->chunk_auto, c->chunk, round_up(M, BM), span);
}

static_assert(MAXD == 8, "zigp_ctx::mean_a / mean_da hold MAXD entries");

int zigp_set_mean_function(zigp_ctx* c, const double* a, int32_t D, double b) {
  if (!c) return ZIGP_EARG;
  if (D < -1 || D > MAXD || (D > 0 && !a)) return fail_arg(c, "zigp_set_mean_function: need -1 <= D <= 8 and a[D] (a Linear mean function covers D in [1, 8]; Zero and Constant work at every D)");
  if (D < 0) {
    for (int d = 0; d < MAXD; ++d) c->mean_a[d] = 0.0;
    c->mean_b = 0.0; c->mean_on = false;
    return ZIGP_OK;
  }
  if (!std::isfinite(b)) return fail_arg(c, "zigp_set_mean_function: b must be finite");
  for (int d = 0; d < D; ++d)
    if (!std::isfinite(a[d])) return fail_arg(c, "zigp_set_mean_function: a must be finite");
  for (int d = 0; d < MAXD; ++d) c->mean_a[d] = (d < D) ? a[d] : 0.0;
  c->mean_b = b;
  c->mean_on = true;
  return ZIGP_OK;
}

int zigp_set_whiten(zigp_ctx* c, int32_t on) {
  if (!c) return ZIGP_EARG;
  if (on < 0 || on > 1) return fail_arg(c, "zigp_set_whiten: on must be 0 or 1");
  c->whiten = on != 0;
  return ZIGP_OK;
}
int zigp_get_whiten(zigp_ctx* c) { return c ? (c->whiten ? 1 : 0) : (int)ZIGP_EARG; }

int zigp_set_q_full(zigp_ctx* c, int32_t on) {
  if (!c) return ZIGP_EARG;
  if (on < 0 || on > 1) return fail_arg(c, "zigp_set_q_full: on must be 0 or 1");
  c->q_full = on != 0;
  return ZIGP_OK;
}
int zigp_get_q_full(zigp_ctx* c) { return c ? (c->q_full ? 1 : 0) : (int)ZIGP_EARG; }

int zigp_set_kernel(zigp_ctx* c, int32_t latent, int32_t kind) {
  if (!c) return ZIGP_EARG;
  if (latent < 0 || latent > 1) return fail_arg(c, "zigp_set_kernel: latent must be 0 (f) or 1 (g)");
  if (kind != ZIGP_KERN_RBF && kind != ZIGP_KERN_MATERN32 && kind != ZIGP_KERN_MATERN52)
    return fail_arg(c, "zigp_set_kernel: unknown kernel kind (ZIGP_KERN_RBF, ZIGP_KERN_MATERN32, ZIGP_KERN_MATERN52)");
  c->kern[latent] = kind;
  if (!is_matern(kind)) {
    (void)hipSetDevice(c->device);
    c->lat[latent].Kd.release();
  }
  return ZIGP_OK;
}
int zigp_get_kernel(zigp_ctx* c, int32_t latent) { return (c && latent >= 0 && latent <= 1) ? c->kern[latent] : (int)ZIGP_EARG; }

int zigp_get_mean_function_grad(zigp_ctx* c, double* da, int32_t D, double* db) {
  if (!c) return ZIGP_EARG;
  if (D < 0 || D > MAXD || (D > 0 && !da)) return fail_arg(c, "zigp_get_mean_function_grad: need 0 <= D <= 8 and da[D]");
  for (int d = 0; d < D; ++d) da[d] = c->mean_da[d];
  if (db) *db = c->mean_db;
  return ZIGP_OK;
}

int zigp_set_data(zigp_ctx* c, const double* X, const double* Y, int64_t N, int32_t D) {
  if (!c) return ZIGP_EARG;
  if (!X || !Y || N <= 0 || D <= 0 || D > ZIGP_MAX_D) return fail_arg(c, "zigp_set_data: bad arguments (need X, Y, N>0, 1<=D<=" ZIGP_MAX_D_STR ")");
  ZIGP_HIP(c, hipSetDevice(c->device));
  ZIGP_ENSURE(c, c->ownX, (size_t)N * D);
  ZIGP_ENSURE(c, c->ownY, (size_t)N);
  ZIGP_HIP(c, hipMemcpyAsync(c->ownX.p, X, sizeof(double) * N * D, hipMemcpyHostToDevice, c->stream));
  ZIGP_HIP(c, hipMemcpyAsync(c->ownY.p, Y, sizeof(double) * N, hipMemcpyHostToDevice, c->stream));
  ZIGP_HIP(c, hipStreamSynchronize(c->stream));
  c->dX = c->ownX.p; c->dY = c->ownY.p; c->N = N; c->D = D;
  c->fullX = c->dX; c->fullY = c->dY; c->fullN = N;
  return ZIGP_OK;
}

int zigp_set_data_device(zigp_ctx* c, const double* dX, const double* dY, int64_t N, int32_t D) {
  if (!c) return ZIGP_EARG;
  if (!dX || !dY || N <= 0 || D <= 0 || D > ZIGP_MAX_D) return fail_arg(c, "zigp_set_data_device: bad arguments (need dX, dY, N>0, 1<=D<=" ZIGP_MAX_D_STR ")");
  c->dX = dX; c->dY = dY; c->N = N; c->D = D;
  c->fullX = dX; c->fullY = dY; c->fullN = N;
  return ZIGP_OK;
}

int zigp_select_rows(zigp_ctx* c, const int64_t* rows, int64_t n) {
  if (!c) return ZIGP_EARG;
  if (!c->fullX) return fail_arg(c, "zigp_select_rows: no data set (call zigp_set_data first)");
  if (n < 0 || (n > 0 && !rows)) return fail_arg(c, "zigp_select_rows: bad arguments");
  if (n == 0) { c->dX = c->fullX; c->dY = c->fullY; c->N = c->fullN; return ZIGP_OK; }
  for (int64_t i = 0; i < n; ++i)
    if (rows[i] < 0 || rows[i] >= c->fullN) return fail_arg(c, "zigp_select_rows: row index out of range");
  ZIGP_HIP(c, hipSetDevice(c->device));
  ZIGP_TRY(begin_staged_call(c));
  const int D = c->D;
  ZIGP_ENSURE(c, c->selX, (size_t)n * D); ZIGP_ENSURE(c, c->selY, (size_t)n); ZIGP_ENSURE(c, c->selIdx, (size_t)n);
  int64_t* h = (int64_t*)c->pinned.alloc(sizeof(int64_t) * n);
  if (!h) { c->err = "hipHostMalloc failed for the staging arena"; return ZIGP_EHIP; }
  memcpy(h, rows, sizeof(int64_t) * n);
// ... 1239 lines not shown
```

zero-inflated-gp_amd/csrc/zigp_host.h:

```cpp
#pragma once
#include "zigp_ctx.h"
#include "zigp_kernels.h"
#include <algorithm>
#include <cmath>
#include <functional>
#include <initializer_list>

namespace zigp {

static inline int ceil_div(int64_t a, int64_t b) { return (int)((a + b - 1) / b); }
static inline int64_t round_up(int64_t a, int64_t b) { return (a + b - 1) / b * b; }

struct TileSpec { std::string key; std::function<int(std::vector<GemmTile>&)> build; };
static int get_tiles(zigp_ctx* c, const TileSpec& s, TileList& out) {
  auto it = c->tiles.find(s.key);
  if (it != c->tiles.end()) { out = it->second.view(); return 0; }
  std::vector<GemmTile> v;
  CachedTiles t;
  t.per = s.build(v); t.n = (int)v.size();
  if (t.n > 0) {
    GemmTile* d = nullptr;
    ZIGP_HIP(c, hipMalloc((void**)&d, sizeof(GemmTile) * v.size()));
    t.d.reset(d);
    ZIGP_HIP(c, hipMemcpy(d, v.data(), sizeof(GemmTile) * v.size(), hipMemcpyHostToDevice));
  }
  out = c->tiles.emplace(s.key, std::move(t)).first->second.view();
  return 0;
}
template <class F>
static int get_tiles(zigp_ctx* c, const std::string& key, F build, TileList& out) {
  return get_tiles(c, TileSpec{key, [&](std::vector<GemmTile>& v) { build(v); return 1; }}, out);
}

static inline GemmTile mk_tile(int bi, int bj, int kbeg, int kend, int slice = 0) {
  GemmTile t; t.bi = bi; t.bj = bj; t.kbeg = kbeg; t.kend = kend; t.slice = slice; t.kdir = 1; t.pad1 = t.pad2 = 0; return t;
}

constexpr int NST = 2;

template <int AL, int BL, bool KS> struct WavesFor { static constexpr int value = 4; };
template <> struct WavesFor<LAY_MNCONTIG, LAY_MNCONTIG, false> { static constexpr int value = 8; };

template <int AL, int BL, bool KS, int TRI = TRI_NONE, class EP>
static int run_gemm(zigp_ctx* c, TileList tl0, GemmArgs g0, EP ep0, TileList tl1 = {}, GemmArgs g1 = {}, EP ep1 = {}) {
  if (tl0.n == 0) { tl0 = tl1; g0 = g1; ep0 = ep1; tl1 = TileList(); }
  if (tl0.n == 0) return 0;
  if (EP::writes_c && (!g0.C || (tl1.n > 0 && !g1.C))) return fail_arg(c, "run_gemm: the epilogue stores C, and C is NULL");
  constexpr int WV = WavesFor<AL, BL, KS>::value;
  constexpr size_t shm = sizeof(double) * NST * STAGE_DOUBLES;
  static bool attr_set = false;
  if (!attr_set) {
    ZIGP_HIP(c, hipFuncSetAttribute(reinterpret_cast<const void*>(&gemm_f64_kernel<AL, BL, NST, KS, TRI, WV, EP>),
                                    hipFuncAttributeMaxDynamicSharedMemorySize, (int)shm));
    attr_set = true;
  }
  g0.tiles = tl0.d; g0.per = tl0.per;
  const int n0 = tl0.n / tl0.per;
  int64_t nwg = n0;
  if (tl1.n > 0) { g1.tiles = tl1.d; g1.per = tl1.per; nwg = round_up(n0, 8) + tl1.n / tl1.per; }
  else { g1 = g0; ep1 = ep0; }
  hipLaunchKernelGGL((gemm_f64_kernel<AL, BL, NST, KS, TRI, WV, EP>), dim3((unsigned)nwg), dim3(64 * WV), shm, c->stream, g0, ep0, g1, ep1, n0);
  ZIGP_HIP(c, hipGetLastError());
  return 0;
}

static inline GemmArgs mk_args(const double* A, int64_t lda, const double* B, int64_t ldb, double* C, int64_t ldc, double alpha = 1.0) {
  GemmArgs g;
  g.seg[0].A = A; g.seg[0].B = B; g.seg[0].lda = lda; g.seg[0].ldb = ldb;
  g.tiles = nullptr; g.per = 1; g.C = C; g.ldc = ldc; g.slice_stride = 0; g.alpha = alpha; g.kscale = nullptr;
  return g;
}

static inline int trmm_tail_makespan(int nbm, int tail_units_per_xcd, int bins) {
  std::vector<int> len;
  const int U = (nbm + 1) / 2;
  for (int i = 0; i < tail_units_per_xcd; ++i) {
    const int u = i % U, lo = u + 1, hi = nbm - u;
    len.push_back(hi);
    if (lo != hi) len.push_back(lo);
  }
  std::sort(len.begin(), len.end(), [](int a, int b) { return a > b; });
  std::vector<int> load(bins, 0);
  for (int l : len) *std::min_element(load.begin(), load.end()) += l;
  return *std::max_element(load.begin(), load.end());
}
static int build_trmm_list(bool lower, int nbm, int nbn, bool paired, int tail_units, int tail_bins, std::vector<GemmTile>& v) {
  const int kb = BM / BK;
  if (!paired) {
    if (lower) { for (int bi = nbm - 1; bi >= 0; --bi) for (int bj = 0; bj < nbn; ++bj) v.push_back(mk_tile(bi, bj, 0, (bi + 1) * kb)); }
    else { for (int bi = 0; bi < nbm; ++bi) for (int bj = 0; bj < nbn; ++bj) v.push_back(mk_tile(bi, bj, bi * kb, nbm * kb)); }
    return 1;
  }
  const int U = (nbm + 1) / 2;
  auto tile = [&](int bi, int bj, int dir) {
    GemmTile t = lower ? mk_tile(bi, bj, 0, (bi + 1) * kb) : mk_tile(bi, bj, bi * kb, nbm * kb);
    t.kdir = dir;
    return t;
  };
  std::vector<GemmTile> q[8];
  for (int bj = 0; bj < nbn; ++bj)
    for (int u = 0; u < U; ++u) {
      const int lo = u, hi = nbm - 1 - u;
      std::vector<GemmTile>& dst = q[bj % 8];
      if (lo == hi) { dst.push_back(tile(lo, bj, lower ? -1 : 1)); dst.push_back(mk_tile(0, 0, 0, 0)); continue; }
      if (lower) { dst.push_back(tile(lo, bj, 1)); dst.push_back(tile(hi, bj, -1)); }
      else { dst.push_back(tile(hi, bj, -1)); dst.push_back(tile(lo, bj, 1)); }
    }
  size_t longest = 0;
  for (int x = 0; x < 8; ++x) longest = std::max(longest, q[x].size());
  int per = 2;
  std::vector<std::vector<GemmTile>> bins[8];
  const int tu = std::min<int>(tail_units / 8, (int)(longest / 2));
  if (tu > 0) {
    const int BINS = std::max(1, std::min(64, tail_bins));
    for (int x = 0; x < 8; ++x) {
      const size_t first = std::min(q[x].size(), (longest / 2 - (size_t)tu) * 2);
      std::vector<GemmTile> t(q[x].begin() + first, q[x].end());
      q[x].resize(first);
      t.erase(std::remove_if(t.begin(), t.end(), [](const GemmTile& a) { return a.kend <= a.kbeg; }), t.end());
      std::stable_sort(t.begin(), t.end(), [](const GemmTile& a, const GemmTile& b) { return a.kend - a.kbeg > b.kend - b.kbeg; });
      bins[x].assign(std::min<size_t>((size_t)BINS, t.size()), std::vector<GemmTile>());
      std::vector<int> load(bins[x].size(), 0);
      for (const GemmTile& a : t) {
        const size_t b = std::min_element(load.begin(), load.end()) - load.begin();
        bins[x][b].push_back(a);
        load[b] += a.kend - a.kbeg;
      }
      std::vector<size_t> order(bins[x].size());
      for (size_t i = 0; i < order.size(); ++i) order[i] = i;
      std::stable_sort(order.begin(), order.end(), [&](size_t a, size_t b) { return load[a] > load[b]; });
      std::vector<std::vector<GemmTile>> sorted;
      for (size_t i : order) sorted.push_back(bins[x][i]);
      bins[x] = sorted;
      for (const auto& b : bins[x]) per = std::max(per, (int)b.size());
    }
  }
  {
    size_t reg = 0, nb = 0;
    for (int x = 0; x < 8; ++x) { reg = std::max(reg, q[x].size() / 2); nb = std::max(nb, bins[x].size()); }
    for (size_t i = 0; i < reg; ++i)
      for (int x = 0; x < 8; ++x)
        for (int e = 0; e < per; ++e) v.push_back(e < 2 && 2 * i + e < q[x].size() ? q[x][2 * i + e] : mk_tile(0, 0, 0, 0));
    for (size_t i = 0; i < nb; ++i)
      for (int x = 0; x < 8; ++x)
        for (int e = 0; e < per; ++e) v.push_back(i < bins[x].size() && e < (int)bins[x][i].size() ? bins[x][i][e] : mk_tile(0, 0, 0, 0));
  }
  return per;
}
static TileSpec trmm_tiles(bool lower, int nbm, int nbn, bool paired, int tail_units, int tail_bins) {
  return {std::string(lower ? "trl:" : "tru:") + std::to_string(nbm) + ":" + std::to_string(nbn) + (paired ? ":p" : ":l") +
              (tail_units > 0 ? ":t" + std::to_string(tail_units) + ":" + std::to_string(tail_bins) : std::string()),
          [=](std::vector<GemmTile>& v) { return build_trmm_list(lower, nbm, nbn, paired, tail_units, tail_bins, v); }};
}
static inline bool trmm_paired_pays(int units_both_latents) {
  const int slots = 512, waves = (units_both_latents + slots - 1) / slots;
  return units_both_latents >= slots && (double)units_both_latents / ((double)waves * slots) >= 0.85;
}
struct TrmmTail { int units[2], bins[2]; };
static inline TrmmTail trmm_tail_plan(int units0, int nbm0, int units1, int nbm1) {
// ... 93 lines not shown
  int h = 0;
  ZIGP_HIP(c, hipMemcpyAsync(&h, c->d_info, sizeof(int), hipMemcpyDeviceToHost, c->stream));
  ZIGP_HIP(c, hipStreamSynchronize(c->stream));
  if (h != 0) {
    c->info = h;
    char b[256];
    snprintf(b, sizeof(b), "Cholesky decomposition was not successful for %s: the input might not be positive definite (pivot %d)", what, h);
    c->err = b;
    return ZIGP_ENOTPD;
  }
  return 0;
}

static inline double pivot_tol(double var, double jitter, double rtol = 8.0) { return rtol * 2.220446049250313e-16 * (var + jitter); }

__global__ void __launch_bounds__(256)
k_sk_finish_tiles(const double* __restrict__ planes, const GemmTile* __restrict__ tiles, int S, int64_t Mp, double alpha, int accum, double* __restrict__ out) {
  const GemmTile tl = tiles[blockIdx.x >> 6];
  const int e = ((blockIdx.x & 63) << 8) + threadIdx.x;
  const int64_t idx = ((int64_t)tl.bi * BM + (e >> 7)) * Mp + (int64_t)tl.bj * BN + (e & 127);
  double v = 0.0;
  for (int s = 0; s < S; ++s) v += planes[(int64_t)s * Mp * Mp + idx];
  out[idx] = accum ? fma(alpha, v, out[idx]) : alpha * v;
}
template <int AL, int BL, class Gen>
static int run_gemm_sk_tiles(zigp_ctx* c, DevBuf& planes, const std::string& key, Gen gen, const double* A, const double* B, double* C, int64_t Mp, double alpha,
                             bool accum = false) {
  std::vector<GemmTile> base;
  gen(base);
  if (base.empty()) return 0;
  int minlen = 1 << 30;
  for (const GemmTile& t : base) minlen = std::min(minlen, t.kend - t.kbeg);
  const int count = (int)base.size(), S = std::max(1, std::min(std::min(8, minlen), 512 / count));
  TileList tl;
  ZIGP_TRY(get_tiles(c, "skt:" + key + ":" + std::to_string(S), [&](std::vector<GemmTile>& v) {
    for (int s = 0; s < S; ++s)
      for (const GemmTile& t : base) {
        const int len = t.kend - t.kbeg;
        v.push_back(mk_tile(t.bi, t.bj, t.kbeg + (int)((int64_t)len * s / S), t.kbeg + (int)((int64_t)len * (s + 1) / S), s));
      }
  }, tl));
  ZIGP_ENSURE(c, planes, (size_t)S * Mp * Mp);
  GemmArgs g = mk_args(A, Mp, B, Mp, planes.p, Mp);
  g.slice_stride = Mp * Mp;
  ZIGP_TRY((run_gemm<AL, BL, false>(c, tl, g, EpiStore())));
  hipLaunchKernelGGL(k_sk_finish_tiles, dim3(64 * count), dim3(256), 0, c->stream, planes.p, tl.d, S, Mp, alpha, accum ? 1 : 0, C);
  ZIGP_HIP(c, hipGetLastError());
  return 0;
}

struct PotrfJob { double* L; double* W; double* T; int Mp; bool want_W; int Mreal; double piv_tol; bool prepared; DevBuf* planes;
                  const double* tol_dev = nullptr; int* info = nullptr; };
static int potrf_trtri_jobs(zigp_ctx* c, int njobs, const PotrfJob* jobs, const hipStream_t* streams) {
  const int kb = BM / BK;
  const size_t shm = sizeof(double) * PB * PBLD;
  int nbmax = 0;
  for (int q = 0; q < njobs; ++q) nbmax = std::max(nbmax, jobs[q].Mp / BM);
  for (int q = 0; q < njobs; ++q) {
    if (jobs[q].prepared) continue;
    OnStream on(c, streams[q]);
    ZIGP_HIP(c, hipMemsetAsync(jobs[q].W, 0, sizeof(double) * jobs[q].Mp * jobs[q].Mp, c->stream));
  }
  for (int j = 0; j < nbmax; ++j) {
    for (int step = 0; step < 3; ++step)
      for (int q = 0; q < njobs; ++q) {
        const PotrfJob& J = jobs[q];
        const int Mp = J.Mp, nb = Mp / BM, Mreal = (J.Mreal < 0 || J.Mreal > Mp) ? Mp : J.Mreal;
        if (j >= nb) continue;
        OnStream on(c, streams[q]);
        double* Lb = J.L; double* Wb = J.W;
        if (step == 0) {
          double* Ajj = Lb + (int64_t)j * BM * Mp + (int64_t)j * BM;
          double* Wjj = Wb + (int64_t)j * BM * Mp + (int64_t)j * BM;
          const int nreal_j = std::max(0, std::min(BM, Mreal - j * BM));
          int* info = J.info ? J.info : c->d_info;
          if (J.tol_dev) hipLaunchKernelGGL(k_potrf_diag<const double*>, dim3(1), dim3(1024), shm, c->stream, Ajj, Ajj, Wjj, (int64_t)Mp, j * BM, info, (nreal_j + PNB - 1) / PNB, J.tol_dev);
          else hipLaunchKernelGGL(k_potrf_diag<double>, dim3(1), dim3(1024), shm, c->stream, Ajj, Ajj, Wjj, (int64_t)Mp, j * BM, info, (nreal_j + PNB - 1) / PNB, J.piv_tol);
          ZIGP_HIP(c, hipGetLastError());
        } else if (j + 1 < nb && step == 1) {
          auto genp = [&](std::vector<GemmTile>& v) {
            for (int bi = j + 1; bi < nb; ++bi) v.push_back(mk_tile(bi, j, j * kb, (j + 1) * kb));
          };
          const std::string tag = "po_p:" + std::to_string(nb) + ":" + std::to_string(j);
          if (J.planes) { ZIGP_TRY((run_gemm_sk_tiles<LAY_KCONTIG, LAY_KCONTIG>(c, *J.planes, tag, genp, Lb, Wb, Lb, Mp, 1.0))); continue; }
          TileList tp;
          ZIGP_TRY(get_tiles(c, tag, genp, tp));
          ZIGP_TRY((run_gemm<LAY_KCONTIG, LAY_KCONTIG, false>(c, tp, mk_args(Lb, Mp, Wb, Mp, Lb, Mp), EpiStore())));
        } else if (j + 1 < nb && step == 2) {
          auto gens = [&](std::vector<GemmTile>& v) {
            for (int bi = j + 1; bi < nb; ++bi)
              for (int bj = j + 1; bj <= bi; ++bj) v.push_back(mk_tile(bi, bj, j * kb, (j + 1) * kb));
          };
          const std::string tag = "po_s:" + std::to_string(nb) + ":" + std::to_string(j);
          if (J.planes) { ZIGP_TRY((run_gemm_sk_tiles<LAY_KCONTIG, LAY_KCONTIG>(c, *J.planes, tag, gens, Lb, Lb, Lb, Mp, -1.0, true))); continue; }
          TileList ts;
          ZIGP_TRY(get_tiles(c, tag, gens, ts));
          ZIGP_TRY((run_gemm<LAY_KCONTIG, LAY_KCONTIG, false>(c, ts, mk_args(Lb, Mp, Lb, Mp, Lb, Mp, -1.0), EpiAccum())));
        }
      }
  }
  for (int bi = 0; bi + 1 < nbmax; ++bi)
    for (int q = 0; q < njobs; ++q) {
      const int Mp = jobs[q].Mp, nb = Mp / BM;
      if (bi + 1 >= nb || jobs[q].prepared) continue;
      OnStream on(c, streams[q]);
      ZIGP_HIP(c, hipMemset2DAsync(jobs[q].L + (int64_t)bi * BM * Mp + (int64_t)(bi + 1) * BM, sizeof(double) * Mp, 0,
                                   sizeof(double) * (size_t)(Mp - (bi + 1) * BM), BM, c->stream));
    }
  for (int b = 1; b < nbmax; b *= 2)
    for (int step = 0; step < 2; ++step)
      for (int q = 0; q < njobs; ++q) {
        const PotrfJob& J = jobs[q];
        const int Mp = J.Mp, nb = Mp / BM;
        if (!J.want_W || b >= nb) continue;
        OnStream on(c, streams[q]);
        auto gen1 = [&](std::vector<GemmTile>& v) {
          for (int lo = 0; lo < nb; lo += 2 * b) {
            const int mid = lo + b, hi = std::min(lo + 2 * b, nb);
            if (mid >= nb) continue;
            for (int bi = mid; bi < hi; ++bi)
              for (int bj = lo; bj < mid; ++bj) v.push_back(mk_tile(bi, bj, bj * kb, mid * kb));
          }
        };
        auto gen2 = [&](std::vector<GemmTile>& v) {
          for (int lo = 0; lo < nb; lo += 2 * b) {
            const int mid = lo + b, hi = std::min(lo + 2 * b, nb);
            if (mid >= nb) continue;
            for (int bi = mid; bi < hi; ++bi)
              for (int bj = lo; bj < mid; ++bj) v.push_back(mk_tile(bi, bj, mid * kb, (bi + 1) * kb));
          }
        };
        const std::string tag = std::to_string(nb) + ":" + std::to_string(b);
        if (step == 0) {
          if (J.planes) { ZIGP_TRY((run_gemm_sk_tiles<LAY_KCONTIG, LAY_MNCONTIG>(c, *J.planes, "tri1:" + tag, gen1, J.L, J.W, J.T, Mp, 1.0))); continue; }
          TileList t1;
          ZIGP_TRY(get_tiles(c, "tri1:" + tag, gen1, t1));
          ZIGP_TRY((run_gemm<LAY_KCONTIG, LAY_MNCONTIG, false>(c, t1, mk_args(J.L, Mp, J.W, Mp, J.T, Mp), EpiStore())));
        } else {
          if (J.planes) { ZIGP_TRY((run_gemm_sk_tiles<LAY_KCONTIG, LAY_MNCONTIG>(c, *J.planes, "tri2:" + tag, gen2, J.W, J.T, J.W, Mp, -1.0))); continue; }
          TileList t2;
          ZIGP_TRY(get_tiles(c, "tri2:" + tag, gen2, t2));
          ZIGP_TRY((run_gemm<LAY_KCONTIG, LAY_MNCONTIG, false>(c, t2, mk_args(J.W, Mp, J.T, Mp, J.W, Mp, -1.0), EpiStore())));
        }
      }
  return 0;
}
static int potrf_trtri(zigp_ctx* c, double* Lb, double* Wb, double* Tb, int Mp, bool want_W, int Mreal = -1, double piv_tol = 0.0) {
  const PotrfJob job = {Lb, Wb, Tb, Mp, want_W, Mreal, piv_tol, false, nullptr};
  const hipStream_t st = c->stream;
  return potrf_trtri_jobs(c, 1, &job, &st);
}

enum { SK_STORE = 0, SK_ACCUM = 1, SK_PHI = 2 };
template <int POST>
__global__ void __launch_bounds__(256)
k_sk_finish(const double* __restrict__ planes, int S, int64_t Mp, double alpha, int lower_only, double* __restrict__ out) {
  const int64_t idx = (int64_t)blockIdx.x * 256 + threadIdx.x;
  if (idx >= Mp * Mp) return;
  const int64_t i = idx / Mp, j = idx - i * Mp;
  if (lower_only && (j / BN > i / BM)) {
    if (POST != SK_ACCUM) out[idx] = 0.0;
    return;
  }
  double v = 0.0;
  for (int s = 0; s < S; ++s) v += planes[(int64_t)s * Mp * Mp + idx];
  v *= alpha;
  if (POST == SK_STORE) out[idx] = v;
  else if (POST == SK_ACCUM) out[idx] += v;
  else out[idx] = (j < i) ? v : ((j == i) ? 0.5 * v : 0.0);
}

enum class SkRule : int { S = 0, Y, R, TT, FULL, T, RT, RFULL, COUNT };
struct SkRuleInfo { const char* key; bool lower_only; };
constexpr SkRuleInfo SK_RULES[(int)SkRule::COUNT] = {
    {"s", false},
    {"y", false},
    {"r", true},
    {"tt", false},
    {"full", false},
    {"t", true},
    {"rt", false},
    {"rfull", true},
};
static inline void sk_range(SkRule r, int bi, int bj, int nb, int kb, int& k0, int& k1) {
  const bool lower = bj <= bi;
  k0 = 0; k1 = 0;
  switch (r) {
    case SkRule::S: k0 = std::max(bi, bj) * kb; k1 = nb * kb; break;
    case SkRule::Y: k0 = bj * kb; k1 = nb * kb; break;
    case SkRule::R: if (lower) { k0 = bi * kb; k1 = nb * kb; } break;
    case SkRule::TT: k1 = (std::min(bi, bj) + 1) * kb; break;
    case SkRule::FULL: k1 = nb * kb; break;
    case SkRule::T: if (lower) { k0 = bj * kb; k1 = (bi + 1) * kb; } break;
    case SkRule::RT: k1 = (bi + 1) * kb; break;
    case SkRule::RFULL: if (lower) k1 = nb * kb; break;
    case SkRule::COUNT: break;
  }
}
static inline int sk_slices(SkRule r, int nb) {
  int count = 0, minlen = 1 << 30;
  for (int bi = 0; bi < nb; ++bi)
    for (int bj = 0; bj < nb; ++bj) {
      int k0, k1; sk_range(r, bi, bj, nb, BM / BK, k0, k1);
      if (k1 > k0) { ++count; minlen = std::min(minlen, k1 - k0); }
    }
  return count == 0 ? 0 : std::max(1, std::min(std::min(8, minlen), 512 / count));
}
static inline void build_sk_list(SkRule r, int nb, std::vector<GemmTile>& v) {
  const int S = sk_slices(r, nb);
  for (int s = 0; s < S; ++s)
    for (int bi = 0; bi < nb; ++bi)
      for (int bj = 0; bj < nb; ++bj) {
        int k0, k1; sk_range(r, bi, bj, nb, BM / BK, k0, k1);
        if (k1 <= k0) continue;
        const int len = k1 - k0;
        v.push_back(mk_tile(bi, bj, k0 + (int)((int64_t)len * s / S), k0 + (int)((int64_t)len * (s + 1) / S), s));
      }
}
template <int AL, int BL>
static int run_gemm_sk(zigp_ctx* c, DevBuf& planes, SkRule r, int nb, const double* A, const double* B, double* C, int64_t Mp, int post, double alpha) {
  const SkRuleInfo& info = SK_RULES[(int)r];
  const int S = sk_slices(r, nb), lower_only = info.lower_only ? 1 : 0;
  if (S == 0) return 0;
  TileList tl;
  ZIGP_TRY(get_tiles(c, std::string("sk:") + info.key + ":" + std::to_string(nb) + ":" + std::to_string(S),
                     [&](std::vector<GemmTile>& v) { build_sk_list(r, nb, v); }, tl));
  ZIGP_ENSURE(c, planes, (size_t)S * Mp * Mp);
  GemmArgs g = mk_args(A, Mp, B, Mp, planes.p, Mp);
  g.slice_stride = Mp * Mp;
  ZIGP_TRY((run_gemm<AL, BL, false>(c, tl, g, EpiStore())));
  const dim3 grid((unsigned)((Mp * Mp + 255) / 256));
  if (post == SK_STORE) hipLaunchKernelGGL(k_sk_finish<SK_STORE>, grid, dim3(256), 0, c->stream, planes.p, S, Mp, alpha, lower_only, C);
  else if (post == SK_ACCUM) hipLaunchKernelGGL(k_sk_finish<SK_ACCUM>, grid, dim3(256), 0, c->stream, planes.p, S, Mp, alpha, lower_only, C);
  else hipLaunchKernelGGL(k_sk_finish<SK_PHI>, grid, dim3(256), 0, c->stream, planes.p, S, Mp, alpha, lower_only, C);
  ZIGP_HIP(c, hipGetLastError());
  return 0;
}

static inline KernHyp make_hyp(const double* ell, double var, int D) {
  KernHyp h;
  for (int d = 0; d < MAXD; ++d) h.inv_ell[d] = (d < D) ? 1.0 / ell[d] : 0.0;
  h.var = var; h.D = D;
  return h;
}

static inline KufHyp make_kuf_hyp(const double* ell, double var, int D) {
  KufHyp h;
  for (int d = 0; d < MAXD; ++d) h.scale[d] = (d < D) ? KUF_C * (1.0 / ell[d]) : 0.0;
  h.var = var;
  return h;
}

static inline int kgmom_slices(int nbm, int64_t Nc) {
  const int64_t ks = Nc / BK;
  return (int)std::max<int64_t>(1, std::min<int64_t>(std::min<int64_t>(64, ks / 16), 512 / std::max(nbm, 1)));
}
static inline int build_kgmom_list(int nbm, int64_t Nc, std::vector<GemmTile>& v) {
  const int S = kgmom_slices(nbm, Nc);
  const int64_t ks = Nc / BK;
  for (int s = 0; s < S; ++s)
    for (int bi = 0; bi < nbm; ++bi) v.push_back(mk_tile(bi, 0, (int)(ks * s / S), (int)(ks * (s + 1) / S), s));
  return 1;
}
static inline TileSpec kgmom_tiles(int nbm, int64_t Nc) {
  return TileSpec{"kgmom:" + std::to_string(nbm) + ":" + std::to_string(Nc), [=](std::vector<GemmTile>& v) { return build_kgmom_list(nbm, Nc, v); }};
}

static inline KernHypWide make_hyp_wide(const double* ell, double var, int D) {
  KernHypWide h;
  for (int d = 0; d < WIDE_MAXD; ++d) h.inv_ell[d] = (d < D) ? 1.0 / ell[d] : 0.0;
  h.var = var; h.D = D;
  return h;
}
static inline KufHypWide make_kuf_hyp_wide(const double* ell, double var, int D) {
  KufHypWide h;
  for (int d = 0; d < WIDE_MAXD; ++d) h.scale[d] = (d < D) ? KUF_C * (1.0 / ell[d]) : 0.0;
  h.var = var;
  return h;
}

static int begin_staged_call(zigp_ctx* c) {
  ZIGP_HIP(c, hipStreamSynchronize(c->stream_main));
  ZIGP_HIP(c, hipStreamSynchronize(c->stream2));
  ZIGP_HIP(c, hipStreamSynchronize(c->stream3));
  c->pinned.reset();
  return 0;
}
static inline double* pinned_doubles(zigp_ctx* c, size_t n) { return (double*)c->pinned.alloc(sizeof(double) * (n ? n : 1)); }
#define ZIGP_PINNED(ctx, ptr, n)                                                         \
  double* ptr = pinned_doubles((ctx), (n));                                              \
  if (!ptr) { (ctx)->err = "hipHostMalloc failed for the staging arena"; return ZIGP_EHIP; }
static int upload_padded(zigp_ctx* c, DevBuf& b, const double* src, size_t n, size_t npad) {
  ZIGP_ENSURE(c, b, npad);
  ZIGP_PINNED(c, h, npad);
  if (n) memcpy(h, src, sizeof(double) * n);
  if (npad > n) memset(h + n, 0, sizeof(double) * (npad - n));
  ZIGP_HIP(c, hipMemcpyAsync(b.p, h, sizeof(double) * npad, hipMemcpyHostToDevice, c->stream));
  return 0;
}
static int download(zigp_ctx* c, const double* dev, size_t n, double** out) {
  ZIGP_PINNED(c, h, n);
  ZIGP_HIP(c, hipMemcpyAsync(h, dev, sizeof(double) * n, hipMemcpyDeviceToHost, c->stream));
  *out = h;
  return 0;
}

static int require_device_ptrs(zigp_ctx* c, std::initializer_list<const void*> ptrs, const char* message) {
  for (const void* q : ptrs) {
    hipPointerAttribute_t at;
    if (!q) continue;
    if (hipPointerGetAttributes(&at, q) != hipSuccess || at.type != hipMemoryTypeDevice || at.device != c->device) {
      (void)hipGetLastError();
      return fail_arg(c, message);
    }
  }
  return 0;
}

}
```

zero-inflated-gp_amd/csrc/zigp_kernels.h:

```cpp
#pragma once
#include <hip/hip_runtime.h>
#include <stdint.h>
#include <math.h>

namespace zigp {

constexpr int MAXD = 8;

constexpr int KH_INV = 0, KH_ZC = MAXD, KH_ELL = 2 * MAXD, KH_VAR = 3 * MAXD, KH_FAC = 3 * MAXD + 2;
constexpr int KH_NOISE = 4 * KH_FAC, KH_FMU = KH_NOISE + 1, KH_SIZE = KH_NOISE + 4;
#define KF_CONST(p) ((const __attribute__((address_space(4))) double*)(p))
constexpr int PW_THREADS = 256;

struct KernHyp { double inv_ell[MAXD]; double var; int D; };

constexpr int DH_INV = 0, DH_ELL = MAXD, DH_SCALE = 2 * MAXD, DH_VAR = 3 * MAXD, DH_PIVTOL = 3 * MAXD + 1, DH_LAT = 3 * MAXD + 2;
constexpr int DH_NOISE = 2 * DH_LAT, DH_SIZE = DH_NOISE + 2;
struct LatHypDev { const double* R; int D; };
__device__ __forceinline__ int hyp_dim(const KernHyp& h) { return h.D; }
__device__ __forceinline__ double hyp_inv_ell(const KernHyp& h, int d) { return h.inv_ell[d]; }
__device__ __forceinline__ double hyp_var(const KernHyp& h) { return h.var; }
__device__ __forceinline__ int hyp_dim(const LatHypDev& h) { return h.D; }
__device__ __forceinline__ double hyp_inv_ell(const LatHypDev& h, int d) { return KF_CONST(h.R)[DH_INV + d]; }
__device__ __forceinline__ double hyp_scale(const LatHypDev& h, int d) { return KF_CONST(h.R)[DH_SCALE + d]; }
// ... 814 lines not shown
  g = fma(g, r, g);
  h = fma(h, r, h);
  return fma(fma(-g, g, s), h, g);
}
template <int KIND, bool GRAD>
__device__ __forceinline__ void kuf_matern(double w, const double* T, double& k, double& kd) {
  const double g = kuf_sqrt(fmin(fma(-w, KufMatern<KIND>::A, KufMatern<KIND>::B), 0x1p+996));
  const double t = g * (KUF_LN2 / 32.0);
  const double e = kuf_exp2_32(-g, T);
  if (KIND == KERN_M32) {
    k = fma(e, t, e);
    if (GRAD) kd = 3.0 * e;
  } else {
    k = e * fma(t, fma(t, 1.0 / 3.0, 1.0), 1.0);
    if (GRAD) kd = (5.0 / 3.0) * fma(e, t, e);
  }
}
template <int D, int KIND, bool GRAD>
__global__ void __launch_bounds__(256)
k_kuf_build_matern(const double* __restrict__ X, int64_t N, int64_t n0, const double* __restrict__ Zs, int M, KufHyp h,
                   double* __restrict__ K, double* __restrict__ Kd, int64_t Nc) {
  __shared__ double T[32];
  if (threadIdx.x < 32) T[threadIdx.x] = hyp_var(h) * KUF_T[threadIdx.x];
  const int64_t n = ((int64_t)blockIdx.x * 256 + threadIdx.x) * 2;
  const int m0 = blockIdx.y * 16;
  double xs[2][D];
#pragma unroll
  for (int e = 0; e < 2; ++e) {
    const bool valid = (n0 + n + e) < N;
#pragma unroll
    for (int d = 0; d < D; ++d) xs[e][d] = valid ? X[(n0 + n + e) * D + d] * hyp_scale(h, d) : 0.0;
  }
  __syncthreads();
#pragma unroll 4
  for (int mm = 0; mm < 16; ++mm) {
    const int m = m0 + mm;
    double2* out = reinterpret_cast<double2*>(K + (int64_t)m * Nc + n);
    double2* outd = GRAD ? reinterpret_cast<double2*>(Kd + (int64_t)m * Nc + n) : nullptr;
    if (m >= M) {
      *out = make_double2(0.0, 0.0);
      if (GRAD) *outd = make_double2(0.0, 0.0);
      continue;
    }
    double w0, w1;
#pragma unroll
    for (int d = 0; d < D; ++d) {
      const double zs = Zs[m * D + d];
      const double t0 = zs - xs[0][d], t1 = zs - xs[1][d];
      w0 = d == 0 ? -t0 * t0 : fma(-t0, t0, w0); w1 = d == 0 ? -t1 * t1 : fma(-t1, t1, w1);
    }
    double k0, k1, kd0 = 0.0, kd1 = 0.0;
    kuf_matern<KIND, GRAD>(w0, T, k0, kd0);
    kuf_matern<KIND, GRAD>(w1, T, k1, kd1);
    *out = make_double2(k0, k1);
    if (GRAD) *outd = make_double2(kd0, kd1);
  }
}

template <int D>
__global__ void __launch_bounds__(256)
k_kgrad_matern(const double* __restrict__ Jp, const double* __restrict__ K, const double* __restrict__ Kd, const double* __restrict__ alpha,
               const double* __restrict__ gm, const double* __restrict__ gv, const double* __restrict__ X, int64_t N, int64_t n0,
               const double* __restrict__ Z, int M, int64_t Nc, int64_t slab, double* __restrict__ krow) {
  constexpr int W = 2 + 2 * D;
  __shared__ double sh[4][KG_ROWS * W];
  krow += (int64_t)blockIdx.y * slab;
  const int m0 = blockIdx.x * KG_ROWS;
  if (m0 >= M) return;
  double am[KG_ROWS], acc[KG_ROWS][W], zr[KG_ROWS][D];
#pragma unroll
  for (int r = 0; r < KG_ROWS; ++r) {
    am[r] = alpha[min(m0 + r, M - 1)];
#pragma unroll
    for (int d = 0; d < D; ++d) zr[r][d] = Z[min(m0 + r, M - 1) * D + d];
#pragma unroll
    for (int q = 0; q < W; ++q) acc[r][q] = 0.0;
  }
  const int64_t nspan = Nc / KG_SPLIT, nbeg = (int64_t)blockIdx.y * nspan;
  const int64_t nmax = min(nbeg + nspan, N - n0);
  for (int64_t n = nbeg + threadIdx.x; n < nmax; n += 256) {
    const double gmn = gm[n], gv2 = 2.0 * gv[n];
    double xc[D];
#pragma unroll
    for (int d = 0; d < D; ++d) xc[d] = X[(n0 + n) * D + d];
#pragma unroll
    for (int r = 0; r < KG_ROWS; ++r) {
      const int64_t o = (int64_t)(m0 + r) * Nc + n;
      const double kk = K[o];
      const double f = fma(gv2, Jp[o], am[r] * gmn);
      const double t = f * Kd[o];
      acc[r][0] = fma(f, kk, acc[r][0]);
      acc[r][1 + 2 * D] = fma(kk, gmn, acc[r][1 + 2 * D]);
#pragma unroll
      for (int d = 0; d < D; ++d) {
        const double df = xc[d] - zr[r][d], td = t * df;
        acc[r][1 + d] += td;
        acc[r][1 + D + d] = fma(td, df, acc[r][1 + D + d]);
      }
    }
  }
#pragma unroll
  for (int r = 0; r < KG_ROWS; ++r)
#pragma unroll
    for (int q = 0; q < W; ++q) {
      const double v = wave_sum(acc[r][q]);
      if ((threadIdx.x & 63) == 0) sh[threadIdx.x >> 6][r * W + q] = v;
    }
  __syncthreads();
  if (threadIdx.x < KG_ROWS * W) {
    const int r = threadIdx.x / W, q = threadIdx.x - r * W;
    if (m0 + r < M)
      krow[(int64_t)(m0 + r) * W + q] += (sh[0][threadIdx.x] + sh[1][threadIdx.x]) + (sh[2][threadIdx.x] + sh[3][threadIdx.x]);
  }
}

__global__ void __launch_bounds__(256)
k_sym_from_planes(const double* __restrict__ part, int So, int Sd, int64_t Mp, double* __restrict__ out) {
  __shared__ double sh[32][33];
  const int t = blockIdx.x;
  int tr = (int)((sqrt(8.0 * t + 1.0) - 1.0) * 0.5);
  while (tr * (tr + 1) / 2 > t) --tr;
  while ((tr + 1) * (tr + 2) / 2 <= t) ++tr;
  const int tc = t - tr * (tr + 1) / 2;
  const int S = (tr * 32 / BM == tc * 32 / BM) ? Sd : So;
  const int tx = threadIdx.x & 31, ty = threadIdx.x >> 5;
  const int64_t plane = Mp * Mp;
  const double* __restrict__ src = part + (int64_t)(32 * tr + ty) * Mp + 32 * tc + tx;
  double a[4] = {0.0, 0.0, 0.0, 0.0};
  for (int s = 0; s < S; ++s) {
#pragma unroll
    for (int k = 0; k < 4; ++k) a[k] += src[(int64_t)s * plane + (int64_t)(8 * k) * Mp];
  }
#pragma unroll
  for (int k = 0; k < 4; ++k) sh[ty + 8 * k][tx] = a[k];
  __syncthreads();
#pragma unroll
  for (int k = 0; k < 4; ++k) {
    const int r = ty + 8 * k;
    if (tr != tc) {
      out[(int64_t)(32 * tr + r) * Mp + 32 * tc + tx] = sh[r][tx];
      out[(int64_t)(32 * tc + r) * Mp + 32 * tr + tx] = sh[tx][r];
    } else {
      out[(int64_t)(32 * tr + r) * Mp + 32 * tc + tx] = (tx <= r) ? sh[r][tx] : sh[tx][r];
    }
  }
}
constexpr int ZERO_RANGES_MAX = 12;
struct ZeroRanges { double* p[ZERO_RANGES_MAX]; int64_t n[ZERO_RANGES_MAX]; int count; };
__global__ void __launch_bounds__(256)
k_zero_ranges(ZeroRanges z) {
  for (int q = 0; q < z.count; ++q)
    for (int64_t i = (int64_t)blockIdx.x * 256 + threadIdx.x; i < z.n[q]; i += (int64_t)gridDim.x * 256) z.p[q][i] = 0.0;
}
__global__ void k_uut_minus(const double* __restrict__ U, const double* __restrict__ C, int64_t Mp, double* __restrict__ V) {
  int64_t idx = (int64_t)blockIdx.x * blockDim.x + threadIdx.x;
  if (idx >= Mp * Mp) return;
  int64_t i = idx / Mp, j = idx - i * Mp;
  V[idx] = U[idx] + U[j * Mp + i] - C[idx];
}
__global__ void k_dl_assemble(const double* __restrict__ R, int64_t Mp, const double* __restrict__ alpha,
                              const double* __restrict__ a1gm, const double* __restrict__ a2gm, const double* __restrict__ v,
                              double* __restrict__ out) {
  int64_t idx = (int64_t)blockIdx.x * blockDim.x + threadIdx.x;
  if (idx >= Mp * Mp) return;
  int64_t i = idx / Mp, j = idx - i * Mp;
  out[idx] = (j <= i) ? -(2.0 * R[idx] + alpha[i] * a1gm[j] + a2gm[i] * v[j]) : 0.0;
}

__global__ void k_sym_combine(const double* __restrict__ S, const double* __restrict__ P, const double* __restrict__ PSP,
                              const double* __restrict__ alpha, int with_data, int with_kl, int64_t Mp, double* __restrict__ G) {
  int64_t idx = (int64_t)blockIdx.x * blockDim.x + threadIdx.x;
  if (idx >= Mp * Mp) return;
  int64_t i = idx / Mp, j = idx - i * Mp;
  double v = 0.0;
  if (with_data) v = 0.5 * (S[i * Mp + j] + S[j * Mp + i]);
  if (with_kl) v -= 0.5 * (0.5 * (P[i * Mp + j] + P[j * Mp + i]) - alpha[i] * alpha[j] - 0.5 * (PSP[i * Mp + j] + PSP[j * Mp + i]));
  G[idx] = v;
}

__global__ void __launch_bounds__(256)
k_gemv_rows(const double* __restrict__ W, const double* __restrict__ u, int64_t Mp, double* __restrict__ v) {
  __shared__ double sh[4];
  const int i = blockIdx.x;
  double a = 0.0;
  for (int k = threadIdx.x; k <= i; k += 256) a = fma(W[(int64_t)i * Mp + k], u[k], a);
  a = block_sum<4>(a, sh);
  if (threadIdx.x == 0) v[i] = a;
}
__global__ void k_gather(const double* __restrict__ src, int stride, int off, int n, int nslab, int64_t slab, double* __restrict__ x) {
  int i = blockIdx.x * blockDim.x + threadIdx.x;
  if (i >= n) return;
  double a = 0.0;
  for (int sp = 0; sp < nslab; ++sp) a += src[(int64_t)sp * slab + (int64_t)i * stride + off];
  x[i] = a;
}
constexpr int COL_LANES = 16;
template <int NV>
__device__ __forceinline__ void col_lanes_reduce(double (&a)[NV], double (*sh)[COL_LANES][64]) {
#pragma unroll
  for (int q = 0; q < NV; ++q) sh[q][threadIdx.y][threadIdx.x] = a[q];
  __syncthreads();
  if (threadIdx.y == 0) {
#pragma unroll
    for (int q = 0; q < NV; ++q) {
      double t = 0.0;
      for (int l = 0; l < COL_LANES; ++l) t += sh[q][l][threadIdx.x];
      a[q] = t;
    }
  }
}
__global__ void __launch_bounds__(64 * COL_LANES)
k_gemv_cols(const double* __restrict__ W, const double* __restrict__ x, int64_t Mp, double* __restrict__ y) {
  __shared__ double sh[1][COL_LANES][64];
  const int i = blockIdx.x * 64 + threadIdx.x;
  double a[1] = {0.0};
  for (int k = blockIdx.x * 64 + threadIdx.y; k < Mp; k += COL_LANES)
    if (k >= i) a[0] = fma(W[(int64_t)k * Mp + i], x[k], a[0]);
  col_lanes_reduce<1>(a, sh);
  if (threadIdx.y == 0) y[i] = a[0];
}
__global__ void __launch_bounds__(64 * COL_LANES)
k_coldot(const double* __restrict__ W, const double* __restrict__ Y, int64_t Mp, double* __restrict__ d) {
  __shared__ double sh[1][COL_LANES][64];
  const int i = blockIdx.x * 64 + threadIdx.x;
  double a[1] = {0.0};
  for (int k = blockIdx.x * 64 + threadIdx.y; k < Mp; k += COL_LANES)
    if (k >= i) a[0] = fma(W[(int64_t)k * Mp + i], Y[(int64_t)k * Mp + i], a[0]);
  col_lanes_reduce<1>(a, sh);
  if (threadIdx.y == 0) d[i] = a[0];
}
__global__ void __launch_bounds__(64 * COL_LANES)
k_kl_cols(const double* __restrict__ W, const double* __restrict__ v, int64_t Mp,
          double* __restrict__ alpha, double* __restrict__ dkinv) {
  __shared__ double sh[2][COL_LANES][64];
  const int i = blockIdx.x * 64 + threadIdx.x;
  double a[2] = {0.0, 0.0};
  for (int k = blockIdx.x * 64 + threadIdx.y; k < Mp; k += COL_LANES)
    if (k >= i) {
      const double w = W[(int64_t)k * Mp + i];
      a[0] = fma(w, v[k], a[0]);
      a[1] = fma(w, w, a[1]);
    }
  col_lanes_reduce<2>(a, sh);
  if (threadIdx.y == 0) { alpha[i] = a[0]; dkinv[i] = a[1]; }
}
__global__ void __launch_bounds__(256)
k_kl_value(const double* __restrict__ v, const double* __restrict__ L, const double* __restrict__ s, const double* __restrict__ dkinv,
           int M, int64_t Mp, double* __restrict__ out) {
  __shared__ double sh[4];
  double mah = 0.0, lq = 0.0, tr = 0.0, lp = 0.0;
  for (int i = threadIdx.x; i < M; i += 256) {
    mah = fma(v[i], v[i], mah);
    const double si = s[i], li = L[(int64_t)i * Mp + i];
    lq += log(si * si);
    tr = fma(dkinv[i], si * si, tr);
    lp += log(li * li);
  }
  mah = block_sum<4>(mah, sh); lq = block_sum<4>(lq, sh); tr = block_sum<4>(tr, sh); lp = block_sum<4>(lp, sh);
  if (threadIdx.x == 0) out[0] = 0.5 * (mah - (double)M - lq + tr + lp);
}
__global__ void __launch_bounds__(256)
k_kl_white(const double* __restrict__ u, const double* __restrict__ s, int M, int64_t Mp, double* __restrict__ wh) {
  __shared__ double sh[4];
  double mah = 0.0, lq = 0.0, tr = 0.0;
  for (int i = threadIdx.x; i < Mp; i += 256) {
    const bool real = i < M;
    const double ui = real ? u[i] : 0.0, s2 = real ? s[i] * s[i] : 1.0;
    wh[i] = s2 - 1.0; wh[Mp + i] = ui; wh[2 * Mp + i] = 1.0;
    if (real) { mah = fma(ui, ui, mah); tr += s2; lq += log(s2); }
  }
  mah = block_sum<4>(mah, sh); lq = block_sum<4>(lq, sh); tr = block_sum<4>(tr, sh);
  if (threadIdx.x == 0) wh[3 * Mp] = 0.5 * (mah - (double)M - lq + tr);
}
__global__ void k_diag(const double* __restrict__ A, int64_t Mp, double* __restrict__ d) {
  const int64_t i = (int64_t)blockIdx.x * blockDim.x + threadIdx.x;
  if (i < Mp) d[i] = A[i * Mp + i];
}

__global__ void __launch_bounds__(256)
k_lq_stage(const double* __restrict__ raw, int M, int64_t Mp, double* __restrict__ Lq, double* __restrict__ ssq) {
  __shared__ double sh[4];
  const int64_t idx = (int64_t)blockIdx.x * 256 + threadIdx.x;
  const int64_t i = idx / Mp, j = idx - i * Mp;
  const double v = (i < M && j <= i) ? raw[i * M + j] : 0.0;
  Lq[idx] = v;
  const double s = block_sum<4>(v * v, sh);
  if (threadIdx.x == 0) ssq[blockIdx.x] = s;
}
__global__ void k_sub_eye(double* __restrict__ A, int M, int64_t Mp) {
  const int64_t i = (int64_t)blockIdx.x * blockDim.x + threadIdx.x;
  if (i < M) A[i * Mp + i] -= 1.0;
}
__global__ void __launch_bounds__(256)
k_kl_white_full(const double* __restrict__ u, const double* __restrict__ Lq, const double* __restrict__ ssq, int nssq, int M, int64_t Mp,
                double* __restrict__ wh) {
  __shared__ double sh[4];
  double mah = 0.0, lq = 0.0, tr = 0.0;
  for (int i = threadIdx.x; i < Mp; i += 256) {
    const bool real = i < M;
    const double ui = real ? u[i] : 0.0;
    wh[i] = 0.0; wh[Mp + i] = ui; wh[2 * Mp + i] = 0.0;
    if (real) { const double d = Lq[(int64_t)i * Mp + i]; mah = fma(ui, ui, mah); lq += log(d * d); }
  }
  for (int b = threadIdx.x; b < nssq; b += 256) tr += ssq[b];
  mah = block_sum<4>(mah, sh); lq = block_sum<4>(lq, sh); tr = block_sum<4>(tr, sh);
  if (threadIdx.x == 0) wh[3 * Mp] = 0.5 * (mah - (double)M - lq + tr);
}
__global__ void k_dlq_assemble(const double* __restrict__ Y, const double* __restrict__ Lq, int with_data, int with_kl, int M, int64_t Mp,
                               double* __restrict__ out) {
  const int64_t idx = (int64_t)blockIdx.x * blockDim.x + threadIdx.x;
  if (idx >= Mp * Mp) return;
  const int64_t i = idx / Mp, j = idx - i * Mp;
  double v = 0.0;
  if (i < M && j <= i) {
    if (with_data) v = 2.0 * Y[idx];
    if (with_kl) { const double l = Lq[idx]; v -= (i == j) ? l - 1.0 / l : l; }
  }
  out[idx] = v;
}
__global__ void k_pack_square(const double* __restrict__ src, int M, int64_t Mp, double* __restrict__ out) {
  const int64_t idx = (int64_t)blockIdx.x * blockDim.x + threadIdx.x;
// ... 78 lines not shown
  for (int m = t; m < M; m += 256) dv += ksum(m, 0);
  dv = block_sum<4>(dv, sh);
  for (int d = 0; d < D; ++d) {
    double v = 0.0;
    for (int m = t; m < M; m += 256) v += ksum(m, 1 + D + d);
    v = block_sum<4>(v, sh);
    if (t == 0) { const double e = L.ell[d]; ol[d] = v / (e * e * e); }
  }
  if (t == 0) a.out[2 + h] = dv / pack_var(a, h, hv...) + pws[2 + h];
}
__global__ void k_gather_rows(const double* __restrict__ X, const double* __restrict__ Y, const int64_t* __restrict__ idx, int64_t n, int D,
                              double* __restrict__ Xb, double* __restrict__ Yb) {
  const int64_t t = (int64_t)blockIdx.x * blockDim.x + threadIdx.x;
  if (t >= n * (D + 1)) return;
  const int64_t i = t / (D + 1); const int d = (int)(t - i * (D + 1));
  const int64_t r = idx[i];
  if (d < D) Xb[i * D + d] = X[r * D + d]; else Yb[i] = Y[r];
}

__device__ __forceinline__ double kfit_softplus(double x) {
#pragma clang fp contract(off)
  const double sp = x < 0.0 ? log1p(exp(x)) : (x == 0.0 ? 0.6931471805599453 : x + log1p(exp(-x)));
  return sp + 1e-6;
}
struct KfitAdam { double beta1, beta2, eps, lr_sq, lr_den; };
__device__ __forceinline__ void kfit_adam(double gc, bool positive, double lr, const KfitAdam& o, double& x, double& m, double& v) {
#pragma clang fp contract(off)
  const double g = -(positive ? gc * (0.5 * (1.0 + tanh(0.5 * x))) : gc);
  const double mnew = o.beta1 * m + (1.0 - o.beta1) * g;
  const double vnew = o.beta2 * v + (1.0 - o.beta2) * g * g;
  const double lr_t = lr * o.lr_sq / o.lr_den;
  x = x - lr_t * mnew / (sqrt(vnew) + o.eps);
  m = mnew; v = vnew;
}

constexpr int DFIT_BLOCKS = 11, DFIT_THREADS = 256;
struct DenseFitDesc {
  int off[DFIT_BLOCKS + 1], n[DFIT_BLOCKS], goff[DFIT_BLOCKS], gn[DFIT_BLOCKS], positive[DFIT_BLOCKS], trainable[DFIT_BLOCKS];
  double lr[DFIT_BLOCKS];
  int D, M[2];
  int tri;
  int img_Z[2], img_ell[2], img_u[2], img_s[2], img_Zs[2];
  double beta1, beta2, eps, jitter, rtol_eps;
};
__device__ __forceinline__ int dfit_block(const DenseFitDesc& d, int e) {
  int b = 0;
#pragma unroll
  for (int q = 1; q < DFIT_BLOCKS; ++q) b += (e >= d.off[q]) ? 1 : 0;
  return b;
}
__device__ __forceinline__ double dfit_value(const DenseFitDesc& d, int b, double x) { return d.positive[b] ? kfit_softplus(x) : x; }

__global__ void __launch_bounds__(DFIT_THREADS)
k_dense_fit_image(DenseFitDesc d, const double* __restrict__ x, double* __restrict__ img, double* __restrict__ H) {
#pragma clang fp contract(off)
  const int e = blockIdx.x * DFIT_THREADS + threadIdx.x;
  if (e >= d.off[DFIT_BLOCKS]) return;
  const int b = dfit_block(d, e), i = e - d.off[b];
  const double val = dfit_value(d, b, x[e]);
  const int h = b & 1, D = d.D;
  if (b <= 1) {
    const int dd = i % D, eb = 6 + h;
    const double ell = dfit_value(d, eb, x[d.off[eb] + (d.n[eb] == 1 ? 0 : dd)]);
    img[d.img_Z[h] + i] = val;
    img[d.img_Zs[h] + i] = val * (KUF_C * (1.0 / ell));
  } else if (b <= 3) img[d.img_u[h] + i] = val;
  else if (b <= 5) { if (!d.tri) img[d.img_s[h] + i] = val; }
  else if (b <= 7) {
    double* R = H + h * DH_LAT;
    for (int dd = (d.n[b] == 1 ? 0 : i); dd < (d.n[b] == 1 ? D : i + 1); ++dd) {
      img[d.img_ell[h] + dd] = val;
      R[DH_ELL + dd] = val; R[DH_INV + dd] = 1.0 / val; R[DH_SCALE + dd] = KUF_C * (1.0 / val);
    }
  } else if (b <= 9) {
    double* R = H + h * DH_LAT;
    R[DH_VAR] = val; R[DH_PIVTOL] = d.rtol_eps * (val + d.jitter);
  } else H[DH_NOISE] = val;
}

__global__ void __launch_bounds__(DFIT_THREADS)
k_dense_fit_image_tri(DenseFitDesc d, const double* __restrict__ x, double* __restrict__ img, double* __restrict__ Lraw_f,
                      double* __restrict__ Lraw_g) {
  const int h = blockIdx.y;
  const int64_t M = d.M[h], idx = (int64_t)blockIdx.x * DFIT_THREADS + threadIdx.x;
  if (idx >= M * M) return;
  const int64_t i = idx / M, j = idx - i * M;
  const double val = j <= i ? x[d.off[4 + h] + i * (i + 1) / 2 + j] : 0.0;
  (h == 0 ? Lraw_f : Lraw_g)[idx] = val;
  if (i == j) img[d.img_s[h] + i] = val;
}

struct DenseFitArgs {
  DenseFitDesc d;
  double *x, *m, *v;
  const double* packed;
  const int* info;
  double* hist;
  int* fail;
  int step;
  double lr_sq, lr_den;
};
__global__ void __launch_bounds__(DFIT_THREADS)
k_dense_fit_update(DenseFitArgs a) {
  const DenseFitDesc& d = a.d;
  __shared__ int s_fail;
  if (threadIdx.x == 0) {
    int f = a.fail[0];
    if (f == 0) {
      const int i0 = a.info[0], i1 = a.info[1];
      const int bad = i0 != 0 ? 0 : (i1 != 0 ? 1 : -1);
      if (bad >= 0) { f = 1 + a.step; if (blockIdx.x == 0) { a.fail[1] = bad; a.fail[2] = bad == 0 ? i0 : i1; a.fail[0] = f; } }
    }
    s_fail = f;
  }
  const int e = blockIdx.x * DFIT_THREADS + threadIdx.x;
  const bool live = e < d.off[DFIT_BLOCKS];
  const int b = live ? dfit_block(d, e) : 0, i = live ? e - d.off[b] : 0;
  double x = 0.0, m = 0.0, v = 0.0, gc = 0.0;
  if (live && d.trainable[b]) {
    x = a.x[e]; m = a.m[e]; v = a.v[e];
    const double* g = a.packed + d.goff[b] + i * d.gn[b];
    gc = g[0];
    for (int j = 1; j < d.gn[b]; ++j) gc += g[j];
  }
  __syncthreads();
  if (s_fail) return;
  if (e == 0) { a.hist[2 * a.step] = a.packed[0]; a.hist[2 * a.step + 1] = a.packed[1]; }
  if (!live || !d.trainable[b]) return;
  kfit_adam(gc, d.positive[b] != 0, d.lr[b], KfitAdam{d.beta1, d.beta2, d.eps, a.lr_sq, a.lr_den}, x, m, v);
  a.x[e] = x; a.m[e] = m; a.v[e] = v;
}

__global__ void k_square(const double* s, double* s2, int n) {
  int i = blockIdx.x * blockDim.x + threadIdx.x;
  if (i < n) s2[i] = s[i] * s[i];
}
__global__ void k_colscale(const double* __restrict__ W, const double* __restrict__ s2, int64_t Mp, double* __restrict__ out) {
  int64_t idx = (int64_t)blockIdx.x * blockDim.x + threadIdx.x;
  if (idx >= Mp * Mp) return;
  out[idx] = s2[idx % Mp] * W[idx];
}
__global__ void __launch_bounds__(256)
k_transpose(const double* __restrict__ W, int64_t Mp, double* __restrict__ Wt) {
  __shared__ double tile[32][33];
  const int bx = blockIdx.x * 32, by = blockIdx.y * 32;
  for (int j = threadIdx.y; j < 32; j += 8) tile[j][threadIdx.x] = W[(int64_t)(by + j) * Mp + bx + threadIdx.x];
  __syncthreads();
  for (int j = threadIdx.y; j < 32; j += 8) {
    const double v = tile[threadIdx.x][j];
    const int64_t o = (int64_t)(bx + j) * Mp + by + threadIdx.x;
    Wt[o] = v;
  }
}
__global__ void k_rowscale_minus_eye(const double* __restrict__ P, const double* __restrict__ s2, int64_t Mp, double* __restrict__ out) {
  int64_t idx = (int64_t)blockIdx.x * blockDim.x + threadIdx.x;
  if (idx >= Mp * Mp) return;
  const int64_t k = idx / Mp;
  out[idx] = fma(s2[k], P[idx], (idx - k * Mp == k) ? -1.0 : 0.0);
}
__global__ void k_rowscale(const double* __restrict__ P, const double* __restrict__ s2, int64_t Mp, double* __restrict__ out) {
  int64_t idx = (int64_t)blockIdx.x * blockDim.x + threadIdx.x;
  if (idx >= Mp * Mp) return;
  out[idx] = s2[idx / Mp] * P[idx];
}

constexpr int PB = 128, PBLD = 129, PNB = 32;
constexpr int PHB = 16;
__device__ __forceinline__ double readlane_f64(double v, int lane) {
  const int lo = __builtin_amdgcn_readlane(__double2loint(v), lane);
  const int hi = __builtin_amdgcn_readlane(__double2hiint(v), lane);
  return __hiloint2double(hi, lo);
}
struct PotrfShared { double dinv[PB]; double T[3][PNB][PNB + 1]; int fail; };
__device__ __forceinline__ double potrf_wget(const double* S, const double* dinv, int x, int y) {
  return x > y ? S[y * PBLD + x] : (x == y ? dinv[x] : 0.0);
}
typedef double potrf_d4 __attribute__((ext_vector_type(4)));
__device__ __forceinline__ void potrf_mfma16(double (&c)[4], double a, double b) {
  potrf_d4 v = {c[0], c[1], c[2], c[3]};
  v = __builtin_amdgcn_mfma_f64_16x16x4f64(a, b, v, 0, 0, 0);
  c[0] = v[0]; c[1] = v[1]; c[2] = v[2]; c[3] = v[3];
}
__device__ __forceinline__ double potrf_rsqrt(double d) {
  double y = __builtin_amdgcn_rsq(d);
  double e = fma(-d * y, y, 1.0);
  y = fma(0.5 * y, e, y);
  e = fma(-d * y, y, 1.0);
  y = fma(0.5 * y, e, y);
  return y;
}
__device__ __forceinline__ void potrf_tile_update(double* S, int i0, int k0, int c0) {
  const int lane = threadIdx.x & 63, g = lane >> 4, n = lane & 15;
  double acc[4] = {0.0, 0.0, 0.0, 0.0};
#pragma unroll
  for (int ks = 0; ks < PNB / 4; ++ks) {
    const int c = c0 + 4 * ks + g;
    potrf_mfma16(acc, S[(i0 + n) * PBLD + c], S[(k0 + n) * PBLD + c]);
  }
#pragma unroll
  for (int r = 0; r < 4; ++r) S[(i0 + 4 * r + g) * PBLD + k0 + n] -= acc[r];
}
__device__ __forceinline__ void potrf_tri_decode(int idx, int& ti, int& tk) {
  int r = 0;
  while (idx >= r + 1) { idx -= r + 1; ++r; }
  ti = r; tk = idx;
}
template <int J0, int J1>
__device__ __forceinline__ void potrf_factor_cols(double (&a)[PNB], int r, double tol, int& bad, double& rdv) {
#pragma unroll
  for (int j = J0; j < J1; ++j) {
    int rr = r;
    asm volatile("" : "+v"(rr));
    const double d = readlane_f64(a[j], j);
    if (!(d > tol)) { if (!bad) bad = j + 1; }
    const double rd = potrf_rsqrt(d);
    double sq = d * rd;
    sq = fma(0.5 * rd, fma(-sq, sq, d), sq);
    const double l = (rr == j) ? sq : a[j] * rd;
    rdv = (rr == j) ? rd : rdv;
    asm volatile("" : "+v"(rdv));
    a[j] = l;
#pragma unroll
    for (int k = j + 1; k < J1; ++k) {
      a[k] = fma(-l, readlane_f64(l, k), a[k]);
      asm volatile("" : "+v"(a[k]));
    }
    __builtin_amdgcn_sched_barrier(0);
  }
}
__device__ __forceinline__ void potrf_wave_sync() {
  __builtin_amdgcn_fence(__ATOMIC_RELEASE, "wavefront");
  __builtin_amdgcn_wave_barrier();
  __builtin_amdgcn_fence(__ATOMIC_ACQUIRE, "wavefront");
}
__device__ __forceinline__ int potrf_factor32(const double* S, PotrfShared& psh, int jb, double tol) {
  const int lane = threadIdx.x & 63, r = lane & 31;
  const int g = lane >> 4, n = lane & 15;
  double a[PNB];
#pragma unroll
  for (int k = 0; k < PNB; ++k) a[k] = S[(jb + r) * PBLD + jb + k];
  int bad = 0;
  double rdv = 1.0;
  potrf_factor_cols<0, PHB>(a, r, tol, bad, rdv);
  if (lane < 32) {
#pragma unroll
    for (int k = 0; k < PHB; ++k) psh.T[0][r][k] = a[k];
  }
  potrf_wave_sync();
  {
    double acc[4] = {0.0, 0.0, 0.0, 0.0};
#pragma unroll
    for (int ks = 0; ks < PHB / 4; ++ks) {
      const double bv = psh.T[0][PHB + n][4 * ks + g];
      potrf_mfma16(acc, bv, bv);
    }
#pragma unroll
    for (int q = 0; q < 4; ++q) psh.T[1][PHB + 4 * q + g][n] = acc[q];
  }
  potrf_wave_sync();
#pragma unroll
  for (int c = 0; c < PHB; ++c) a[PHB + c] -= psh.T[1][PHB + (r & 15)][c];
  potrf_factor_cols<PHB, PNB>(a, r, tol, bad, rdv);
  if (!bad && lane < 32) {
#pragma unroll
    for (int k = PHB; k < PNB; ++k) psh.T[0][r][k] = a[k];
    psh.T[1][0][r] = rdv;
    psh.dinv[jb + r] = rdv;
  }
  return bad;
}
__device__ __forceinline__ void potrf_invert16(double* S, PotrfShared& psh, int pb, int h) {
  const int lane = threadIdx.x & 63, r = lane & 15, p0 = pb + PHB * h;
  double a[PHB];
#pragma unroll
  for (int k = 0; k < PHB; ++k) a[k] = S[(p0 + r) * PBLD + p0 + k];
  {
    int rr = r;
    asm volatile("" : "+v"(rr));
#pragma unroll
    for (int k = 1; k < PHB; ++k) a[k] = (k <= rr) ? a[k] : 0.0;
  }
  const double dv = psh.dinv[p0 + r];
#pragma unroll
  for (int j = PHB - 1; j >= 0; --j) {
    int rr = r;
    asm volatile("" : "+v"(rr));
    const double wjj = readlane_f64(dv, j);
    double sum = 0.0;
#pragma unroll
    for (int k = j + 1; k < PHB; ++k) sum = fma(a[k], readlane_f64(a[j], k), sum);
    a[j] = (rr == j) ? wjj : ((rr > j) ? -wjj * sum : 0.0);
    asm volatile("" : "+v"(a[j]));
    __builtin_amdgcn_sched_barrier(0);
  }
  if (lane < PHB) {
#pragma unroll
    for (int k = 0; k < PHB; ++k) psh.T[2][PHB * h + r][k] = a[k];
  }
  __builtin_amdgcn_fence(__ATOMIC_RELEASE, "wavefront");
  __builtin_amdgcn_wave_barrier();
  __builtin_amdgcn_fence(__ATOMIC_ACQUIRE, "wavefront");
  for (int idx = lane; idx < PHB * PHB; idx += 64) {
    const int rr = idx >> 4, k = idx & 15;
    if (k < rr) S[(p0 + k) * PBLD + p0 + rr] = psh.T[2][PHB * h + rr][k];
  }
}
__device__ __forceinline__ void potrf_invert_couple(double* S, PotrfShared& psh, int pb) {
  const int lane = threadIdx.x & 63, g = lane >> 4, n = lane & 15;
  double x[4] = {0.0, 0.0, 0.0, 0.0}, w[4] = {0.0, 0.0, 0.0, 0.0};
  const double dn = psh.dinv[pb + n];
#pragma unroll
// ... 171 lines not shown
```

Baseline: 7.408 ELBO steps/s (value+gradient, 1e6-row steps, fp64).

## Fuse elementwise M×M passes into GEMM epilogues and overlap latent tail on side stream

```diff
diff --git a/zero-inflated-gp_amd/csrc/zigp_ctx.h b/zero-inflated-gp_amd/csrc/zigp_ctx.h
--- a/zero-inflated-gp_amd/csrc/zigp_ctx.h
+++ b/zero-inflated-gp_amd/csrc/zigp_ctx.h
@@ -108,6 +108,7 @@
   hipStream_t stream3 = nullptr;
   hipEvent_t ev_fork = nullptr, ev_join = nullptr;
   hipEvent_t ev_prep_fork = nullptr, ev_prep = nullptr;
+  hipEvent_t ev_tail_fork[2] = {nullptr, nullptr}, ev_tail = nullptr, ev_rev = nullptr;
   int* d_info = nullptr;
   struct PendingEv { hipEvent_t a, b; int cls; };
   std::vector<PendingEv> pending;
@@ -119,7 +120,7 @@
     if (d_info) (void)hipFree(d_info);
     for (auto& e : pending) { (void)hipEventDestroy(e.a); (void)hipEventDestroy(e.b); }
     for (auto e : ev_pool) (void)hipEventDestroy(e);
-    for (hipEvent_t e : {ev_fork, ev_join, ev_prep_fork, ev_prep})
+    for (hipEvent_t e : {ev_fork, ev_join, ev_prep_fork, ev_prep, ev_tail_fork[0], ev_tail_fork[1], ev_tail, ev_rev})
       if (e) (void)hipEventDestroy(e);
     for (hipStream_t s : {stream3, stream2, stream_main})
       if (s) (void)hipStreamDestroy(s);
diff --git a/zero-inflated-gp_amd/csrc/zigp_dense.hip b/zero-inflated-gp_amd/csrc/zigp_dense.hip
--- a/zero-inflated-gp_amd/csrc/zigp_dense.hip
+++ b/zero-inflated-gp_amd/csrc/zigp_dense.hip
@@ -143,7 +143,7 @@
 }
 
 int latents_forward(zigp_ctx* c, const HostLatent (&hl)[2], int D, double jitter, Param par, bool with_kl, bool need_grad, const double* d_hyp,
-                    int* d_info2) {
+                    int* d_info2, bool tail_side = false) {
   const hipStream_t st[2] = {c->stream_main, c->stream2};
   for (int h = 0; h < 2; ++h) {
     Latent& lt = c->lat[h];
@@ -175,11 +175,16 @@
     }
     ZIGP_TRY(potrf_trtri_jobs(c, 2, jobs, st));
   }
-  for (int step = 0; step < 8; ++step)
+  const bool diag_tail_side = tail_side && !is_white(par);
+  for (int step = 0; step < 6; ++step)
     for (int h = 0; h < 2; ++h) {
       Latent& lt = c->lat[h];
       const int Mp = lt.Mp;
-      OnStream on(c, st[h]);
+      if (diag_tail_side && step == 2) {
+        ZIGP_HIP(c, hipEventRecord(c->ev_tail_fork[h], st[h]));
+        ZIGP_HIP(c, hipStreamWaitEvent(c->stream3, c->ev_tail_fork[h], 0));
+      }
+      OnStream on(c, diag_tail_side && step >= 2 ? c->stream3 : st[h]);
       if (step == 0) lt.P_ready = false;
       double* v = lt.vec.p; double* alpha = v + Mp; double* dkinv = v + 2 * Mp; double* klv = v + 3 * Mp;
       if (is_white(par)) {
@@ -201,30 +206,28 @@
       }
       switch (step) {
         case 0:
-          hipLaunchKernelGGL(k_transpose, dim3(Mp / 32, Mp / 32), dim3(32, 8), 0, c->stream, lt.W.p, (int64_t)Mp, lt.Wt.p);
+          if (need_grad)
+            hipLaunchKernelGGL(k_transpose_colscale, dim3(Mp / 32, Mp / 32), dim3(32, 8), 0, c->stream, lt.W.p, lt.s2.p, (int64_t)Mp, lt.Wt.p, lt.Wp.p);
+          else hipLaunchKernelGGL(k_transpose, dim3(Mp / 32, Mp / 32), dim3(32, 8), 0, c->stream, lt.W.p, (int64_t)Mp, lt.Wt.p);
           break;
         case 1: if (with_kl) hipLaunchKernelGGL(k_gemv_rows, dim3(Mp), dim3(256), 0, c->stream, lt.W.p, lt.u.p, (int64_t)Mp, v); break;
         case 2: if (with_kl) hipLaunchKernelGGL(k_kl_cols, dim3(Mp / 64), dim3(64, COL_LANES), 0, c->stream, lt.W.p, v, (int64_t)Mp, alpha, dkinv); break;
         case 3: if (with_kl) hipLaunchKernelGGL(k_kl_value, dim3(1), dim3(256), 0, c->stream, v, lt.L.p, lt.s.p, dkinv, lt.M, (int64_t)Mp, klv); break;
         case 4:
-          if (need_grad) hipLaunchKernelGGL(k_colscale, dim3(ceil_div((int64_t)Mp * Mp, 256)), dim3(256), 0, c->stream, lt.W.p, lt.s2.p, (int64_t)Mp, lt.Wp.p);
-          break;
-        case 5:
           if (need_grad) {
-            ZIGP_TRY((run_gemm_sk<LAY_MNCONTIG, LAY_MNCONTIG>(c, lt.sk, SkRule::S, Mp / BM, lt.W.p, lt.W.p, lt.P.p, Mp, SK_STORE, 1.0)));
+            ZIGP_TRY((run_gemm_sk<LAY_MNCONTIG, LAY_MNCONTIG>(c, lt.sk, SkRule::S, Mp / BM, lt.W.p, lt.W.p, lt.P.p, Mp, SK_STORE, 1.0,
+                                                               FinQt{lt.s2.p, lt.Qt.p})));
             lt.P_ready = true;
           }
           break;
-        case 6:
-          if (need_grad) hipLaunchKernelGGL(k_rowscale_minus_eye, dim3(ceil_div((int64_t)Mp * Mp, 256)), dim3(256), 0, c->stream, lt.P.p, lt.s2.p, (int64_t)Mp, lt.Qt.p);
-          break;
-        case 7:
+        case 5:
           if (need_grad) ZIGP_TRY((run_gemm_sk<LAY_KCONTIG, LAY_MNCONTIG>(c, lt.sk, SkRule::RT, Mp / BM, lt.W.p, lt.Qt.p, lt.Rt.p, Mp, SK_STORE, 1.0)));
           break;
         default: break;
       }
       ZIGP_HIP(c, hipGetLastError());
     }
+  if (diag_tail_side) ZIGP_HIP(c, hipEventRecord(c->ev_tail, c->stream3));
   return 0;
 }
 
@@ -311,7 +314,8 @@
   return 0;
 }
 
-int chunk_forward(zigp_ctx* c, const ChunkPlan& pl, Param par, bool need_grad, const std::function<int()>& after_a1 = nullptr) {
+int chunk_forward(zigp_ctx* c, const ChunkPlan& pl, Param par, bool need_grad, const std::function<int()>& after_a1 = nullptr,
+                  const std::function<int()>& before_j = nullptr) {
   const int64_t Nc = pl.Nc;
   struct Set { TileList t1, t2; double fl; GemmArgs a1, a2j; EpiStoreColsum e1; EpiColsum e2; EpiStorePanelKColsum ej; } q[3] = {};
   for (int h = 0; h < 2; ++h) {
@@ -337,6 +341,7 @@
       ZIGP_TRY((run_gemm<LAY_MNCONTIG, LAY_MNCONTIG, false, TRI_A_LOWER>(c, x.t1, x.a1, x.e1, y.t1, y.a1, y.e1)));
     }
     if (gi == groups - 1 && after_a1) ZIGP_TRY(after_a1());
+    if (need_grad && gi == 0 && before_j) ZIGP_TRY(before_j());
     if (need_grad) {
       ProfScope ps(c, PC_GEMM_J, 2.0 * (x.fl + y.fl));
       ZIGP_TRY((run_gemm<LAY_MNCONTIG, LAY_MNCONTIG, false>(c, x.t2, x.a2j, x.ej, y.t2, y.a2j, y.ej)));
@@ -488,87 +493,94 @@
 using MxmTap = std::function<int(int, const double*)>;
 #define ZIGP_TAP(id, buf) do { if (tap) ZIGP_TRY(tap(id, buf)); } while (0)
 
-int mxm_backward_head(zigp_ctx* c, Latent& lt, int D, Param par, const MxmTap& tap) {
+int mxm_backward_seeds(zigp_ctx* c, Latent& lt, int D, Param par) {
   const int Mp = lt.Mp;
   double* kgm = lt.vec.p + 3 * Mp + 8;
   hipLaunchKernelGGL(k_gather, dim3(ceil_div(Mp, 256)), dim3(256), 0, c->stream, lt.krow.p, 2 + 2 * D, 1 + 2 * D, Mp, KG_SPLIT,
                      (int64_t)Mp * (2 + 2 * D), kgm);
   hipLaunchKernelGGL(k_gemv_rows, dim3(Mp), dim3(256), 0, c->stream, lt.W.p, kgm, (int64_t)Mp, lt.a1gm.p);
   if (!is_white(par)) hipLaunchKernelGGL(k_gemv_cols, dim3(Mp / 64), dim3(64, COL_LANES), 0, c->stream, lt.W.p, lt.a1gm.p, (int64_t)Mp, lt.du.p);
+  ZIGP_HIP(c, hipGetLastError());
+  return 0;
+}
+int mxm_backward_head(zigp_ctx* c, Latent& lt, int D, Param par, bool seeds_done, const MxmTap& tap) {
+  if (!seeds_done) ZIGP_TRY(mxm_backward_seeds(c, lt, D, par));
   latent_sym_from_planes(c, lt);
   ZIGP_TAP(ZIGP_MXM_TAP_C1, lt.T1.p);
   return 0;
 }
-int mxm_backward_r_diag(zigp_ctx* c, Latent& lt, const MxmTap& tap) {
-  const int Mp = lt.Mp, nb = Mp / BM, gridmm = ceil_div((int64_t)Mp * Mp, 256);
+int mxm_backward_r_diag(zigp_ctx* c, Latent& lt, const FinDl& dl, const MxmTap& tap) {
+  const int Mp = lt.Mp, nb = Mp / BM;
   ZIGP_TRY((run_gemm_sk<LAY_KCONTIG, LAY_MNCONTIG>(c, lt.sk, SkRule::Y, nb, lt.T1.p, lt.W.p, lt.T3.p, Mp, SK_STORE, 1.0)));
   ZIGP_TAP(ZIGP_MXM_TAP_Y, lt.T3.p);
   hipLaunchKernelGGL(k_coldot, dim3(Mp / 64), dim3(64, COL_LANES), 0, c->stream, lt.W.p, lt.T3.p, (int64_t)Mp, lt.dsq.p);
   ZIGP_TRY((run_gemm_sk<LAY_KCONTIG, LAY_KCONTIG>(c, lt.sk, SkRule::TT, nb, lt.Wp.p, lt.W.p, lt.T2.p, Mp, SK_STORE, 1.0)));
   ZIGP_TAP(ZIGP_MXM_TAP_T, lt.T2.p);
-  ZIGP_TRY((run_gemm_sk<LAY_KCONTIG, LAY_MNCONTIG>(c, lt.sk, SkRule::FULL, nb, lt.T2.p, lt.T1.p, lt.T3.p, Mp, SK_STORE, 1.0)));
+  ZIGP_TRY((run_gemm_sk_pair<LAY_KCONTIG, LAY_MNCONTIG>(c, lt.sk, SkRule::FULL, nb, lt.T2.p, lt.T1.p, lt.T3.p, Mp, 1.0, FinV{lt.T1.p, lt.G.p})));
   ZIGP_TAP(ZIGP_MXM_TAP_U, lt.T3.p);
-  hipLaunchKernelGGL(k_uut_minus, dim3(gridmm), dim3(256), 0, c->stream, lt.T3.p, lt.T1.p, (int64_t)Mp, lt.G.p);
   ZIGP_TAP(ZIGP_MXM_TAP_V, lt.G.p);
-  ZIGP_TRY((run_gemm_sk<LAY_MNCONTIG, LAY_MNCONTIG>(c, lt.sk, SkRule::R, nb, lt.W.p, lt.G.p, lt.T2.p, Mp, SK_STORE, 1.0)));
+  ZIGP_TRY((run_gemm_sk<LAY_MNCONTIG, LAY_MNCONTIG>(c, lt.sk, SkRule::R, nb, lt.W.p, lt.G.p, lt.T2.p, Mp, SK_STORE, 1.0, dl)));
   ZIGP_TAP(ZIGP_MXM_TAP_R, lt.T2.p);
   return 0;
 }
-int mxm_backward_r_white(zigp_ctx* c, Latent& lt, Param par, bool with_kl, const MxmTap& tap) {
+int mxm_backward_r_white(zigp_ctx* c, Latent& lt, Param par, bool with_kl, const FinDl& dl, const MxmTap& tap) {
   const int Mp = lt.Mp, nb = Mp / BM;
   if (is_full(par)) {
     ZIGP_TRY(latent_qfull_dlq(c, lt, true, with_kl));
     ZIGP_TAP(ZIGP_MXM_TAP_Y, lt.T3.p);
-    ZIGP_TRY((run_gemm_sk<LAY_MNCONTIG, LAY_MNCONTIG>(c, lt.sk, SkRule::RFULL, nb, lt.Rt.p, lt.T1.p, lt.T2.p, Mp, SK_STORE, 1.0)));
+    ZIGP_TRY((run_gemm_sk<LAY_MNCONTIG, LAY_MNCONTIG>(c, lt.sk, SkRule::RFULL, nb, lt.Rt.p, lt.T1.p, lt.T2.p, Mp, SK_STORE, 1.0, dl)));
   } else {
     hipLaunchKernelGGL(k_diag, dim3(ceil_div(Mp, 256)), dim3(256), 0, c->stream, lt.T1.p, (int64_t)Mp, lt.dsq.p);
-    ZIGP_TRY((run_gemm_sk<LAY_MNCONTIG, LAY_MNCONTIG>(c, lt.sk, SkRule::R, nb, lt.Wp.p, lt.T1.p, lt.T2.p, Mp, SK_STORE, 1.0)));
+    ZIGP_TRY((run_gemm_sk<LAY_MNCONTIG, LAY_MNCONTIG>(c, lt.sk, SkRule::R, nb, lt.Wp.p, lt.T1.p, lt.T2.p, Mp, SK_STORE, 1.0, dl)));
   }
   ZIGP_TAP(ZIGP_MXM_TAP_R, lt.T2.p);
   return 0;
 }
-int mxm_backward_tail(zigp_ctx* c, Latent& lt, const double* r1, const double* r2, const MxmTap& tap) {
+int mxm_backward_tail(zigp_ctx* c, Latent& lt, const FinG& fin, const MxmTap& tap) {
   const int Mp = lt.Mp, nb = Mp / BM;
-  hipLaunchKernelGGL(k_dl_assemble, dim3(ceil_div((int64_t)Mp * Mp, 256)), dim3(256), 0, c->stream, lt.T2.p, (int64_t)Mp, lt.vec.p + Mp, lt.a1gm.p, r1,
-                     r2, lt.T1.p);
   ZIGP_TAP(ZIGP_MXM_TAP_DL, lt.T1.p);
   ZIGP_TRY((run_gemm_sk<LAY_MNCONTIG, LAY_MNCONTIG>(c, lt.sk, SkRule::R, nb, lt.L.p, lt.T1.p, lt.T2.p, Mp, SK_PHI, 1.0)));
   ZIGP_TAP(ZIGP_MXM_TAP_Q, lt.T2.p);
   ZIGP_TRY((run_gemm_sk<LAY_KCONTIG, LAY_MNCONTIG>(c, lt.sk, SkRule::T, nb, lt.T2.p, lt.W.p, lt.T3.p, Mp, SK_STORE, 1.0)));
   ZIGP_TAP(ZIGP_MXM_TAP_QW, lt.T3.p);
-  ZIGP_TRY((run_gemm_sk<LAY_MNCONTIG, LAY_MNCONTIG>(c, lt.sk, SkRule::S, nb, lt.W.p, lt.T3.p, lt.T1.p, Mp, SK_STORE, 1.0)));
+  ZIGP_TRY((run_gemm_sk_pair<LAY_MNCONTIG, LAY_MNCONTIG>(c, lt.sk, SkRule::S, nb, lt.W.p, lt.T3.p, lt.T1.p, Mp, 1.0, fin)));
   ZIGP_TAP(ZIGP_MXM_TAP_S, lt.T1.p);
   return 0;
 }
 int latent_mxm_backward(zigp_ctx* c, Latent& lt, int D, double jitter, Param par, bool with_data, bool with_kl, const MxmTap& tap,
-                        const HostLatent* hk = nullptr) {
+                        const HostLatent* hk = nullptr, bool early_done = false) {
   const int Mp = lt.Mp, nb = Mp / BM;
   const size_t mm = (size_t)Mp * Mp;
   ZIGP_ENSURE(c, lt.T1, mm); ZIGP_ENSURE(c, lt.T2, mm); ZIGP_ENSURE(c, lt.T3, mm);
   if (!is_white(par)) ZIGP_ENSURE(c, lt.G, mm);
   const int gridmm = ceil_div((int64_t)mm, 256);
+  const bool kl_part = !is_white(par) && with_kl;
+  double* alpha = lt.vec.p + Mp;
+  auto kl_products = [&]() -> int {
+    if (!lt.P_ready) {
+      ZIGP_ENSURE(c, lt.P, mm);
+      ZIGP_TRY((run_gemm_sk<LAY_MNCONTIG, LAY_MNCONTIG>(c, lt.sk, SkRule::S, nb, lt.W.p, lt.W.p, lt.P.p, Mp, SK_STORE, 1.0)));
+      ZIGP_TAP(ZIGP_MXM_TAP_P, lt.P.p);
+    }
+    const double* Ps = lt.T3.p;
+    if (early_done && lt.P_ready) Ps = lt.Qt.p;
+    else hipLaunchKernelGGL(k_rowscale, dim3(gridmm), dim3(256), 0, c->stream, lt.P.p, lt.s2.p, (int64_t)Mp, lt.T3.p);
+    ZIGP_TRY((run_gemm_sk<LAY_KCONTIG, LAY_MNCONTIG>(c, lt.sk, SkRule::FULL, nb, lt.P.p, Ps, lt.G.p, Mp, SK_STORE, 1.0)));
+    ZIGP_TAP(ZIGP_MXM_TAP_PSP, lt.G.p);
+    return 0;
+  };
   if (with_data) {
-    ZIGP_TRY(mxm_backward_head(c, lt, D, par, tap));
-    if (is_white(par)) ZIGP_TRY(mxm_backward_r_white(c, lt, par, with_kl, tap));
-    else ZIGP_TRY(mxm_backward_r_diag(c, lt, tap));
-    ZIGP_TRY(mxm_backward_tail(c, lt, lt.du.p, is_white(par) ? lt.du.p : lt.vec.p, tap));
-  } else if (is_full(par)) ZIGP_TRY(latent_qfull_dlq(c, lt, false, with_kl));
-  if (is_white(par)) {
-    hipLaunchKernelGGL(k_sym_combine, dim3(gridmm), dim3(256), 0, c->stream, lt.T1.p, lt.T1.p, lt.T1.p, lt.vec.p + Mp, with_data ? 1 : 0, 0,
-                       (int64_t)Mp, lt.T3.p);
+    const FinDl dl{alpha, lt.a1gm.p, lt.du.p, is_white(par) ? lt.du.p : lt.vec.p, lt.T1.p};
+    ZIGP_TRY(mxm_backward_head(c, lt, D, par, early_done, tap));
+    if (is_white(par)) ZIGP_TRY(mxm_backward_r_white(c, lt, par, with_kl, dl, tap));
+    else ZIGP_TRY(mxm_backward_r_diag(c, lt, dl, tap));
+    if (kl_part) ZIGP_TRY(kl_products());
+    ZIGP_TRY(mxm_backward_tail(c, lt, FinG{lt.P.p, lt.G.p, alpha, kl_part ? 1 : 0, (int64_t)Mp, lt.T3.p}, tap));
   } else {
-    double* P = lt.P_ready ? lt.P.p : lt.T2.p; double* PSP = lt.G.p;
-    if (with_kl) {
-      if (!lt.P_ready) {
-        ZIGP_TRY((run_gemm_sk<LAY_MNCONTIG, LAY_MNCONTIG>(c, lt.sk, SkRule::S, nb, lt.W.p, lt.W.p, lt.T2.p, Mp, SK_STORE, 1.0)));
-        ZIGP_TAP(ZIGP_MXM_TAP_P, lt.T2.p);
-      }
-      hipLaunchKernelGGL(k_rowscale, dim3(gridmm), dim3(256), 0, c->stream, P, lt.s2.p, (int64_t)Mp, lt.T3.p);
-      ZIGP_TRY((run_gemm_sk<LAY_KCONTIG, LAY_MNCONTIG>(c, lt.sk, SkRule::FULL, nb, P, lt.T3.p, lt.G.p, Mp, SK_STORE, 1.0)));
-      ZIGP_TAP(ZIGP_MXM_TAP_PSP, lt.G.p);
-    }
-    hipLaunchKernelGGL(k_sym_combine, dim3(gridmm), dim3(256), 0, c->stream, lt.T1.p, P, PSP, lt.vec.p + Mp, with_data ? 1 : 0, with_kl ? 1 : 0,
-                       (int64_t)Mp, lt.T3.p);
+    if (is_full(par)) ZIGP_TRY(latent_qfull_dlq(c, lt, false, with_kl));
+    if (kl_part) ZIGP_TRY(kl_products());
+    hipLaunchKernelGGL(k_sym_combine, dim3(gridmm), dim3(256), 0, c->stream, lt.T1.p, kl_part ? lt.P.p : lt.T1.p, kl_part ? lt.G.p : lt.T1.p, alpha, 0,
+                       kl_part ? 1 : 0, (int64_t)Mp, lt.T3.p);
   }
   launch_kuu_grad(c, lt, D, jitter, hk);
   ZIGP_HIP(c, hipGetLastError());
@@ -619,6 +631,8 @@
   int pw_blocks = 0;
   int* hinfo = nullptr;
   bool prep_side = false;
+  bool tail_side = false;
+  bool rev_side = false;
   const double* d_hyp = nullptr; int* d_info2 = nullptr;
   int lik = 0;
   const double* hyp_rec(int h) const { return d_hyp ? d_hyp + h * DH_LAT : nullptr; }
@@ -627,6 +641,7 @@
 int dense_prepare_buffers(zigp_ctx* c, DenseCall& k);
 int64_t dense_first_chunk_rows(const DenseCall& k) { return std::min<int64_t>(k.Nc, round_up(k.row_end - k.row_begin, 1024)); }
 int dense_mxm_forward(zigp_ctx* c, DenseCall& k) {
+  k.tail_side = k.rev_side = false;
   if (k.d_hyp) ZIGP_HIP(c, hipMemsetAsync(k.d_info2, 0, 2 * sizeof(int), c->stream));
   else {
     ZIGP_TRY(begin_staged_call(c));
@@ -647,7 +662,8 @@
   {
     ProfScope ps(c, PC_MXM);
     ZIGP_TRY(fork_side(c, c->ev_fork, c->stream2));
-    ZIGP_TRY(latents_forward(c, k.hl, k.D, k.jitter, k.par, true, k.need_grad, k.d_hyp, k.d_info2));
+    k.tail_side = k.prep_side && k.need_grad && k.par == Param::Diag;
+    ZIGP_TRY(latents_forward(c, k.hl, k.D, k.jitter, k.par, true, k.need_grad, k.d_hyp, k.d_info2, k.tail_side));
     ZIGP_TRY(join_side(c, c->ev_join, c->stream2));
   }
   return k.d_hyp ? 0 : request_info(c, &k.hinfo);
@@ -742,7 +758,7 @@
   return dense_pointwise_launch(c, k.par, k.predict, k.need_grad, dense_pointwise_args(c, k, n0, Nc), k.d_hyp, k.lik);
 }
 
-int dense_chunk_loop(zigp_ctx* c, const DenseCall& k) {
+int dense_chunk_loop(zigp_ctx* c, DenseCall& k) {
   if (!k.has_rows) return 0;
   const int64_t Nc_full = k.Nc, row_begin = k.row_begin, row_end = k.row_end;
   const int D = k.D;
@@ -794,7 +810,9 @@
       ZIGP_TRY(dense_pointwise(c, k, n0, Nc));
       if (k.need_grad) ZIGP_TRY(chunk_forward_white(c, pl, true, true));
     } else {
-      ZIGP_TRY(chunk_forward(c, pl, k.par, k.need_grad, after_a1));
+      std::function<int()> before_j;
+      if (k.tail_side && n0 == row_begin) before_j = [&]() -> int { ZIGP_HIP(c, hipStreamWaitEvent(c->stream_main, c->ev_tail, 0)); return 0; };
+      ZIGP_TRY(chunk_forward(c, pl, k.par, k.need_grad, after_a1, before_j));
       ZIGP_TRY(dense_pointwise(c, k, n0, Nc));
     }
     const bool kgrad_side = c->overlap == 1 && k.need_grad && !timed;
@@ -804,6 +822,19 @@
         ZIGP_TRY(kgrad(n0, Nc));
         return kuf_side ? kuf(n1) : 0;
       }));
+    if (k.tail_side && kgrad_side && !has_next) {
+      ZIGP_HIP(c, hipStreamWaitEvent(c->stream3, c->ev_join, 0));
+      OnStream on(c, c->stream3);
+      for (int h = 0; h < 2; ++h) {
+        Latent& lt = c->lat[h];
+        ZIGP_TRY(mxm_backward_seeds(c, lt, D, k.par));
+        if (k.include_kl && lt.P_ready)
+          hipLaunchKernelGGL(k_rowscale, dim3(ceil_div((int64_t)lt.Mp * lt.Mp, 256)), dim3(256), 0, c->stream, lt.P.p, lt.s2.p, (int64_t)lt.Mp, lt.Qt.p);
+      }
+      ZIGP_HIP(c, hipGetLastError());
+      ZIGP_HIP(c, hipEventRecord(c->ev_rev, c->stream3));
+      k.rev_side = true;
+    }
     if (k.need_grad) {
       if (!kgrad_side) ZIGP_TRY(kgrad(n0, Nc));
       for (int h = 0; h < 2; ++h) ZIGP_TRY(latent_chunk_syrk(c, pl, h));
@@ -903,12 +934,14 @@
   const int rc = dense_chunk_loop(c, k);
   c->prof_skip = false;
   ZIGP_TRY(rc);
+  if (k.tail_side && !k.has_rows) ZIGP_HIP(c, hipStreamWaitEvent(c->stream_main, c->ev_tail, 0));
+  if (k.rev_side) ZIGP_HIP(c, hipStreamWaitEvent(c->stream_main, c->ev_rev, 0));
   if (k.need_grad) {
     ProfScope ps(c, PC_MXM);
     ZIGP_TRY(fork_side(c, c->ev_fork, c->stream2));
     for (int h = 0; h < 2; ++h) {
       OnStream on(c, h == 0 ? c->stream_main : c->stream2);
-      ZIGP_TRY(latent_mxm_backward(c, c->lat[h], k.D, k.jitter, k.par, k.has_rows, k.include_kl != 0, nullptr, &k.hl[h]));
+      ZIGP_TRY(latent_mxm_backward(c, c->lat[h], k.D, k.jitter, k.par, k.has_rows, k.include_kl != 0, nullptr, &k.hl[h], k.rev_side));
     }
     ZIGP_TRY(join_side(c, c->ev_join, c->stream2));
   }
@@ -969,7 +1002,11 @@
   if (hipEventCreateWithFlags(&c->ev_fork, hipEventDisableTiming) != hipSuccess ||
       hipEventCreateWithFlags(&c->ev_join, hipEventDisableTiming) != hipSuccess ||
       hipEventCreateWithFlags(&c->ev_prep_fork, hipEventDisableTiming) != hipSuccess ||
-      hipEventCreateWithFlags(&c->ev_prep, hipEventDisableTiming) != hipSuccess) { delete c; return ZIGP_EHIP; }
+      hipEventCreateWithFlags(&c->ev_prep, hipEventDisableTiming) != hipSuccess ||
+      hipEventCreateWithFlags(&c->ev_tail_fork[0], hipEventDisableTiming) != hipSuccess ||
+      hipEventCreateWithFlags(&c->ev_tail_fork[1], hipEventDisableTiming) != hipSuccess ||
+      hipEventCreateWithFlags(&c->ev_tail, hipEventDisableTiming) != hipSuccess ||
+      hipEventCreateWithFlags(&c->ev_rev, hipEventDisableTiming) != hipSuccess) { delete c; return ZIGP_EHIP; }
   if (hipMalloc((void**)&c->d_info, sizeof(int)) != hipSuccess) { delete c; return ZIGP_EHIP; }
   if (hipFuncSetAttribute(reinterpret_cast<const void*>(&k_potrf_diag<double>), hipFuncAttributeMaxDynamicSharedMemorySize,
                           (int)(sizeof(double) * PB * PBLD)) != hipSuccess ||
diff --git a/zero-inflated-gp_amd/csrc/zigp_host.h b/zero-inflated-gp_amd/csrc/zigp_host.h
--- a/zero-inflated-gp_amd/csrc/zigp_host.h
+++ b/zero-inflated-gp_amd/csrc/zigp_host.h
@@ -5,6 +5,7 @@
 #include <cmath>
 #include <functional>
 #include <initializer_list>
+#include <type_traits>
 
 namespace zigp {
 
@@ -404,23 +405,98 @@
 }
 
 enum { SK_STORE = 0, SK_ACCUM = 1, SK_PHI = 2 };
-template <int POST>
+struct FinNone {
+  __device__ __forceinline__ void operator()(int64_t, int64_t, int64_t, double) const {}
+  __device__ __forceinline__ void above(int64_t) const {}
+};
+struct FinQt {
+  const double* s2; double* Qt;
+  __device__ __forceinline__ void operator()(int64_t idx, int64_t i, int64_t j, double v) const { Qt[idx] = fma(s2[i], v, (j == i) ? -1.0 : 0.0); }
+  __device__ __forceinline__ void above(int64_t) const {}
+};
+struct FinDl {
+  const double *alpha, *a1gm, *a2gm, *v; double* dL;
+  __device__ __forceinline__ void operator()(int64_t idx, int64_t i, int64_t j, double r) const {
+#pragma clang fp contract(off)
+    const double t = alpha[i] * a1gm[j];
+    dL[idx] = (j <= i) ? -fma(a2gm[i], v[j], fma(2.0, r, t)) : 0.0;
+  }
+  __device__ __forceinline__ void above(int64_t idx) const { dL[idx] = 0.0; }
+};
+template <int POST, class F = FinNone>
 __global__ void __launch_bounds__(256)
-k_sk_finish(const double* __restrict__ planes, int S, int64_t Mp, double alpha, int lower_only, double* __restrict__ out) {
+k_sk_finish(const double* __restrict__ planes, int S, int64_t Mp, double alpha, int lower_only, double* __restrict__ out, F fin = F()) {
   const int64_t idx = (int64_t)blockIdx.x * 256 + threadIdx.x;
   if (idx >= Mp * Mp) return;
   const int64_t i = idx / Mp, j = idx - i * Mp;
   if (lower_only && (j / BN > i / BM)) {
     if (POST != SK_ACCUM) out[idx] = 0.0;
+    fin.above(idx);
     return;
   }
   double v = 0.0;
   for (int s = 0; s < S; ++s) v += planes[(int64_t)s * Mp * Mp + idx];
   v *= alpha;
-  if (POST == SK_STORE) out[idx] = v;
+  if (POST == SK_STORE) { out[idx] = v; fin(idx, i, j, v); }
   else if (POST == SK_ACCUM) out[idx] += v;
   else out[idx] = (j < i) ? v : ((j == i) ? 0.5 * v : 0.0);
 }
+template <class F>
+__global__ void __launch_bounds__(256)
+k_sk_finish_pair(const double* __restrict__ planes, int S, int64_t Mp, double alpha, double* __restrict__ out, F fin) {
+  __shared__ double sa[32][33], sb[32][33];
+  const int t = blockIdx.x;
+  int tr = (int)((sqrt(8.0 * t + 1.0) - 1.0) * 0.5);
+  while (tr * (tr + 1) / 2 > t) --tr;
+  while ((tr + 1) * (tr + 2) / 2 <= t) ++tr;
+  const int tc = t - tr * (tr + 1) / 2;
+  const int tx = threadIdx.x & 31, ty = threadIdx.x >> 5;
+  const int64_t plane = Mp * Mp;
+  const int64_t ia = (int64_t)(32 * tr + ty) * Mp + 32 * tc + tx, ib = (int64_t)(32 * tc + ty) * Mp + 32 * tr + tx;
+  double a[4] = {0.0, 0.0, 0.0, 0.0}, b[4] = {0.0, 0.0, 0.0, 0.0};
+  for (int s = 0; s < S; ++s) {
+#pragma unroll
+    for (int k = 0; k < 4; ++k) {
+      a[k] += planes[(int64_t)s * plane + ia + (int64_t)(8 * k) * Mp];
+      b[k] += planes[(int64_t)s * plane + ib + (int64_t)(8 * k) * Mp];
+    }
+  }
+#pragma unroll
+  for (int k = 0; k < 4; ++k) { a[k] *= alpha; b[k] *= alpha; sa[ty + 8 * k][tx] = a[k]; sb[ty + 8 * k][tx] = b[k]; }
+  __syncthreads();
+#pragma unroll
+  for (int k = 0; k < 4; ++k) {
+    const int r = ty + 8 * k;
+    const int64_t oa = ia + (int64_t)(8 * k) * Mp, ob = ib + (int64_t)(8 * k) * Mp;
+    out[oa] = a[k];
+    fin(oa, (int64_t)32 * tr + r, (int64_t)32 * tc + tx, a[k], sb[tx][r]);
+    if (tr != tc) {
+      out[ob] = b[k];
+      fin(ob, (int64_t)32 * tc + r, (int64_t)32 * tr + tx, b[k], sa[tx][r]);
+    }
+  }
+}
+struct FinV {
+  const double* C; double* V;
+  __device__ __forceinline__ void operator()(int64_t idx, int64_t, int64_t, double u, double ut) const {
+#pragma clang fp contract(off)
+    V[idx] = u + ut - C[idx];
+  }
+};
+struct FinG {
+  const double *P, *PSP, *alpha; int with_kl; int64_t Mp; double* G;
+  __device__ __forceinline__ void operator()(int64_t, int64_t i, int64_t j, double s, double st) const {
+#pragma clang fp contract(off)
+    double v = 0.5 * (s + st);
+    if (with_kl) {
+      const double aa = alpha[i] * alpha[j];
+      double kl = fma(P[i * Mp + j] + P[j * Mp + i], 0.5, -aa);
+      kl = fma(-0.5, PSP[i * Mp + j] + PSP[j * Mp + i], kl);
+      v = fma(-0.5, kl, v);
+    }
+    G[i * Mp + j] = v;
+  }
+};
 
 enum class SkRule : int { S = 0, Y, R, TT, FULL, T, RT, RFULL, COUNT };
 struct SkRuleInfo { const char* key; bool lower_only; };
@@ -470,9 +546,9 @@
       }
 }
 template <int AL, int BL>
-static int run_gemm_sk(zigp_ctx* c, DevBuf& planes, SkRule r, int nb, const double* A, const double* B, double* C, int64_t Mp, int post, double alpha) {
+static int run_gemm_sk_planes(zigp_ctx* c, DevBuf& planes, SkRule r, int nb, const double* A, const double* B, int64_t Mp, int& S) {
   const SkRuleInfo& info = SK_RULES[(int)r];
-  const int S = sk_slices(r, nb), lower_only = info.lower_only ? 1 : 0;
+  S = sk_slices(r, nb);
   if (S == 0) return 0;
   TileList tl;
   ZIGP_TRY(get_tiles(c, std::string("sk:") + info.key + ":" + std::to_string(nb) + ":" + std::to_string(S),
@@ -480,11 +556,31 @@
   ZIGP_ENSURE(c, planes, (size_t)S * Mp * Mp);
   GemmArgs g = mk_args(A, Mp, B, Mp, planes.p, Mp);
   g.slice_stride = Mp * Mp;
-  ZIGP_TRY((run_gemm<AL, BL, false>(c, tl, g, EpiStore())));
+  return run_gemm<AL, BL, false>(c, tl, g, EpiStore());
+}
+template <int AL, int BL, class F = FinNone>
+static int run_gemm_sk(zigp_ctx* c, DevBuf& planes, SkRule r, int nb, const double* A, const double* B, double* C, int64_t Mp, int post, double alpha,
+                       F fin = F()) {
+  if (!std::is_same<F, FinNone>::value && post != SK_STORE) return fail_arg(c, "run_gemm_sk: an epilogue functor rides behind SK_STORE only");
+  const int lower_only = SK_RULES[(int)r].lower_only ? 1 : 0;
+  int S = 0;
+  ZIGP_TRY((run_gemm_sk_planes<AL, BL>(c, planes, r, nb, A, B, Mp, S)));
+  if (S == 0) return 0;
   const dim3 grid((unsigned)((Mp * Mp + 255) / 256));
-  if (post == SK_STORE) hipLaunchKernelGGL(k_sk_finish<SK_STORE>, grid, dim3(256), 0, c->stream, planes.p, S, Mp, alpha, lower_only, C);
-  else if (post == SK_ACCUM) hipLaunchKernelGGL(k_sk_finish<SK_ACCUM>, grid, dim3(256), 0, c->stream, planes.p, S, Mp, alpha, lower_only, C);
-  else hipLaunchKernelGGL(k_sk_finish<SK_PHI>, grid, dim3(256), 0, c->stream, planes.p, S, Mp, alpha, lower_only, C);
+  if (post == SK_STORE) hipLaunchKernelGGL((k_sk_finish<SK_STORE, F>), grid, dim3(256), 0, c->stream, planes.p, S, Mp, alpha, lower_only, C, fin);
+  else if (post == SK_ACCUM) hipLaunchKernelGGL((k_sk_finish<SK_ACCUM, FinNone>), grid, dim3(256), 0, c->stream, planes.p, S, Mp, alpha, lower_only, C, FinNone());
+  else hipLaunchKernelGGL((k_sk_finish<SK_PHI, FinNone>), grid, dim3(256), 0, c->stream, planes.p, S, Mp, alpha, lower_only, C, FinNone());
+  ZIGP_HIP(c, hipGetLastError());
+  return 0;
+}
+template <int AL, int BL, class F>
+static int run_gemm_sk_pair(zigp_ctx* c, DevBuf& planes, SkRule r, int nb, const double* A, const double* B, double* C, int64_t Mp, double alpha, F fin) {
+  if (SK_RULES[(int)r].lower_only) return fail_arg(c, "run_gemm_sk_pair: the rule computes the lower tiles only");
+  int S = 0;
+  ZIGP_TRY((run_gemm_sk_planes<AL, BL>(c, planes, r, nb, A, B, Mp, S)));
+  if (S == 0) return 0;
+  const int nt = (int)(Mp / 32);
+  hipLaunchKernelGGL((k_sk_finish_pair<F>), dim3(nt * (nt + 1) / 2), dim3(256), 0, c->stream, planes.p, S, Mp, alpha, C, fin);
   ZIGP_HIP(c, hipGetLastError());
   return 0;
 }
diff --git a/zero-inflated-gp_amd/csrc/zigp_kernels.h b/zero-inflated-gp_amd/csrc/zigp_kernels.h
--- a/zero-inflated-gp_amd/csrc/zigp_kernels.h
+++ b/zero-inflated-gp_amd/csrc/zigp_kernels.h
@@ -990,21 +990,6 @@
   for (int q = 0; q < z.count; ++q)
     for (int64_t i = (int64_t)blockIdx.x * 256 + threadIdx.x; i < z.n[q]; i += (int64_t)gridDim.x * 256) z.p[q][i] = 0.0;
 }
-__global__ void k_uut_minus(const double* __restrict__ U, const double* __restrict__ C, int64_t Mp, double* __restrict__ V) {
-  int64_t idx = (int64_t)blockIdx.x * blockDim.x + threadIdx.x;
-  if (idx >= Mp * Mp) return;
-  int64_t i = idx / Mp, j = idx - i * Mp;
-  V[idx] = U[idx] + U[j * Mp + i] - C[idx];
-}
-__global__ void k_dl_assemble(const double* __restrict__ R, int64_t Mp, const double* __restrict__ alpha,
-                              const double* __restrict__ a1gm, const double* __restrict__ a2gm, const double* __restrict__ v,
-                              double* __restrict__ out) {
-  int64_t idx = (int64_t)blockIdx.x * blockDim.x + threadIdx.x;
-  if (idx >= Mp * Mp) return;
-  int64_t i = idx / Mp, j = idx - i * Mp;
-  out[idx] = (j <= i) ? -(2.0 * R[idx] + alpha[i] * a1gm[j] + a2gm[i] * v[j]) : 0.0;
-}
-
 __global__ void k_sym_combine(const double* __restrict__ S, const double* __restrict__ P, const double* __restrict__ PSP,
                               const double* __restrict__ alpha, int with_data, int with_kl, int64_t Mp, double* __restrict__ G) {
   int64_t idx = (int64_t)blockIdx.x * blockDim.x + threadIdx.x;
@@ -1389,11 +1374,19 @@
     Wt[o] = v;
   }
 }
-__global__ void k_rowscale_minus_eye(const double* __restrict__ P, const double* __restrict__ s2, int64_t Mp, double* __restrict__ out) {
-  int64_t idx = (int64_t)blockIdx.x * blockDim.x + threadIdx.x;
-  if (idx >= Mp * Mp) return;
-  const int64_t k = idx / Mp;
-  out[idx] = fma(s2[k], P[idx], (idx - k * Mp == k) ? -1.0 : 0.0);
+__global__ void __launch_bounds__(256)
+k_transpose_colscale(const double* __restrict__ W, const double* __restrict__ s2, int64_t Mp, double* __restrict__ Wt, double* __restrict__ Wp) {
+  __shared__ double tile[32][33];
+  const int bx = blockIdx.x * 32, by = blockIdx.y * 32;
+  const double sc = s2[bx + threadIdx.x];
+  for (int j = threadIdx.y; j < 32; j += 8) {
+    const int64_t idx = (int64_t)(by + j) * Mp + bx + threadIdx.x;
+    const double w = W[idx];
+    tile[j][threadIdx.x] = w;
+    Wp[idx] = sc * w;
+  }
+  __syncthreads();
+  for (int j = threadIdx.y; j < 32; j += 8) Wt[(int64_t)(bx + j) * Mp + by + threadIdx.x] = tile[threadIdx.x][j];
 }
 __global__ void k_rowscale(const double* __restrict__ P, const double* __restrict__ s2, int64_t Mp, double* __restrict__ out) {
   int64_t idx = (int64_t)blockIdx.x * blockDim.x + threadIdx.x;
```

After: 7.404 ELBO steps/s (value+gradient, 1e6-row steps, fp64). Within noise of the previous version (-0.1%).
